# mir-group/allegro

Hardware: NVIDIA H100
Metric: atom-steps/sec (energy+forces) (higher is better)
Workload: dtype f32

## Files before the change

allegro_b200/_lib.py:

```python
from __future__ import annotations

import ctypes as C
import os
from typing import Optional, Sequence, Tuple

import torch

from . import build as _build

AB2_F64, AB2_F32, AB2_BF16 = 0, 1, 2
ACT_NONE, ACT_SILU, ACT_MUL_DSILU = 0, 1, 2
EPI_NONE, EPI_MUL_DSILU = 0, 1
NL_SILU, NL_MISH, NL_GELU = 1, 2, 3
NOT_ELIGIBLE = -1
MAX_SEG = 4

DTYPE_ENUM = {torch.float64: AB2_F64, torch.float32: AB2_F32, torch.bfloat16: AB2_BF16}
ACC_DTYPE = {torch.float64: torch.float64, torch.float32: torch.float32, torch.bfloat16: torch.float32}

_LIB: Optional[C.CDLL] = None

_vp, _i64, _i32, _dbl = C.c_void_p, C.c_int64, C.c_int, C.c_double

_SIGNATURES = {
    "ab2_version": ([], C.c_int),
    "ab2_device_ok": ([], C.c_int),
    "ab2_last_error": ([], C.c_char_p),
    "ab2_set_option": ([C.c_char_p, _i32], C.c_int),
    "ab2_op_scatter_env": ([_i32, _i64, _i64, _dbl, _vp, _vp, _vp, _vp], C.c_int),
    "ab2_op_contract": ([_i32, _i32, _i64, _i32, _i32, _i32, _i32, _i32, _vp, _vp, _vp, _vp, _vp, _vp, _vp], C.c_int),
    "ab2_op_gather_rows": ([_i32, _i64, _i64, _dbl, _vp, _vp, _vp, _vp], C.c_int),
    "ab2_op_contract_wgrad": ([_i32, _i64, _i32, _i32, _i32, _i32, _i32, _vp, _vp, _vp, _vp, _vp, _vp, _vp], C.c_int),
    "ab2_sh_fwd": ([_i32, _i32, _i64, _vp, _vp, _vp], C.c_int),
    "ab2_sh_bwd": ([_i32, _i32, _i64, _vp, _vp, _vp, _i32, _vp], C.c_int),
    "ab2_linear": ([_i32, _i64, _i32, _i32, _i32, _vp, _vp, _vp, _vp, _vp, _i32, _vp, _vp, _i32, _vp, _vp, _vp, _vp, _i32, _vp, _i64, _vp], C.c_int),
    "ab2_linear_nl": ([_i32, _i64, _i32, _i32, _i32, _vp, _vp, _vp, _vp, _vp, _i32, _vp, _vp, _i32, _vp, _vp, _vp, _vp, _i32, _vp, _i64, _vp, _i32], C.c_int),
    "ab2_linear_packed_bytes": ([_i32, _i32, _i32], C.c_int64),
    "ab2_linear_pack": ([_i32, _i32, _i32, _vp, _vp, _vp], C.c_int),
    "ab2_mlp2_readout": ([_i32, _i32, _i64, _i32, _i32, _i32, _i32, _vp, _i64, _vp, _i64, _vp, _i64, _vp, _i64, _vp, _i64, _vp, _i64, _vp, _vp, _vp], C.c_int),
    "ab2_mlp2": ([_i32, _i32, _i64, _i32, _i32, _i32, _i32, _vp, _vp, _vp, _vp, _vp, _vp, _vp, _i64, _i32, _vp, _vp, _vp, _vp, _vp], C.c_int),
    "ab2_mlp2_nl": ([_i32, _i32, _i64, _i32, _i32, _i32, _i32, _vp, _vp, _vp, _vp, _vp, _vp, _vp, _i64, _i32, _vp, _vp, _vp, _vp, _vp, _i32], C.c_int),
    "ab2_mlp2_readout_nl": ([_i32, _i32, _i64, _i32, _i32, _i32, _i32, _vp, _i64, _vp, _i64, _vp, _i64, _vp, _i64, _vp, _i64, _vp, _i64, _vp, _vp, _vp, _i32],
                            C.c_int),
    "ab2_env_sum": ([_i32, _i32, _i64, _i32, _vp, _vp, _vp, _i64, _dbl, _vp, _vp], C.c_int),
    "ab2_env_bwd": ([_i32, _i32, _i64, _i64, _i32, _vp, _vp, _vp, _vp, _i64, _vp, _dbl, _vp, _i64, _vp, _vp], C.c_int),
    "ab2_tp_fwd": ([_i32, _i32, _i64, _i64, _i32, _i32, _i32, _i32, _vp, _vp, _vp, _vp, _vp, _vp, _i32, _vp, _vp, _i64, _vp, _vp], C.c_int),
    "ab2_tp_bwd": ([_i32, _i32, _i64, _i64, _i32, _i32, _i32, _i32, _vp, _vp, _vp, _vp, _vp, _vp, _i32, _vp, _vp, _i64, _vp, _vp, _vp, _i64, _vp, _vp, _vp], C.c_int),
    "ab2_tp_chain_fwd": ([_i32, _i32, _i64, _i64, _i32, _vp, _vp, _vp, _vp, _vp, _vp, _vp, _vp, _vp, _vp], C.c_int),
    "ab2_tp_chain_bwd": ([_i32, _i32, _i64, _i64, _i32, _vp, _vp, _vp, _vp, _vp, _vp, _vp, _vp, _vp, _vp, _vp, _vp, _vp, _vp], C.c_int),
    "ab2_edge_sum": ([_i32, _i64, _vp, _vp, _dbl, _vp, _vp], C.c_int),
    "ab2_edge_sum_bwd": ([_i32, _i64, _vp, _vp, _dbl, _vp, _vp], C.c_int),
    "ab2_force_scatter": ([_i32, _i64, _i64, _i64, _vp, _vp, _vp, _vp, _vp, _vp], C.c_int),
    "ab2_force_virial_scatter": ([_i32, _i64, _i64, _i64, _vp, _vp, _vp, _vp, _vp, _vp, _vp, _vp], C.c_int),
    "ab2_transpose_ui": ([_i32, _i64, _i32, _i32, _vp, _vp, _i32, _vp], C.c_int),
    "ab2_edge_vec": ([_i32, _i32, _i64, _vp, _vp, _vp, _vp, _vp, _vp], C.c_int),
    "ab2_radial_fwd": ([_i32, _i64, _i32, _i32, _dbl, _vp, _vp, _vp, _vp, _vp, _i32, _vp, _vp, _vp, _vp, _vp, _vp], C.c_int),
    "ab2_radial_pq_fwd": ([_i32, _i64, _i32, _i32, _dbl, _vp, _vp, _vp, _vp, _vp, _i32, _vp, _vp, _vp, _vp], C.c_int),
    "ab2_radial_pq_bwd": ([_i32, _i64, _i32, _i32, _dbl, _vp, _vp, _vp, _vp, _vp, _i32, _vp, _vp, _vp, _vp, _vp, _vp], C.c_int),
    "ab2_radial_pq_bwd_nl": ([_i32, _i64, _i32, _i32, _dbl, _vp, _vp, _vp, _vp, _vp, _i32, _vp, _vp, _vp, _vp, _vp, _vp, _i32], C.c_int),
    "ab2_zbl": ([_i32, _i64, _i32, _dbl, _dbl, _vp, _vp, _vp, _vp, _vp, _vp, _vp, _vp, _vp], C.c_int),
    "ab2_p2p_mailbox_bytes": ([_i32, _i32], C.c_int64),
    "ab2_p2p_alloc": ([_i64, C.POINTER(C.c_void_p)], C.c_int),
    "ab2_p2p_free": ([_vp], C.c_int),
    "ab2_p2p_get_handle": ([_vp, _vp], C.c_int),
    "ab2_p2p_open_handle": ([_vp, C.POINTER(C.c_void_p)], C.c_int),
    "ab2_p2p_close_handle": ([_vp], C.c_int),
    "ab2_p2p_error": ([_vp, _i32, _i32, _vp], C.c_int),
    "ab2_p2p_begin": ([_vp, _vp], C.c_int),
    "ab2_p2p_push_rows": ([_i32, _i32, _i32, _vp, _vp, _i32, _dbl, _vp, _i32, _i32, _vp, _vp, _vp], C.c_int),
    "ab2_p2p_push_rows_v": ([_i32, _i32, _i32, _vp, _vp, _i32, _dbl, _dbl, _dbl, _vp, _i32, _i32, _vp, _vp, _vp], C.c_int),
    "ab2_p2p_wait_unpack": ([_i32, _i32, _i32, _vp, _i32, _i32, _vp, _i32, _vp, _vp, _i32, _vp], C.c_int),
    "ab2_p2p_allreduce_energy": ([_vp, _i32, _i32, _i32, _vp, _vp, _vp, _vp, _vp], C.c_int),
    "ab2_p2p_mailbox_bytes_ex": ([_i32, _i32, _i32], C.c_int64),
    "ab2_p2p_push_rows_w": ([_i32, _i32, _vp, _vp, _i32, _vp, _i32, _i32, _vp, _vp, _vp], C.c_int),
    "ab2_p2p_wait_unpack_w": ([_i32, _i32, _vp, _i32, _i32, _vp, _i32, _vp, _vp, _vp, _vp], C.c_int),
    "ab2_p2p_allreduce_vec": ([_vp, _i32, _i32, _i32, _i32, _vp, _vp, _vp, _vp, _vp], C.c_int),
    "ab2_slab_plan_count": ([_i32, _i32, _i64, _vp, _vp, _vp, _i32, _i32, _dbl, _dbl, _dbl, _vp, _vp, _vp], C.c_int),
    "ab2_slab_plan_fill": ([_i64, _vp, _vp, _vp, _vp, _vp, _vp], C.c_int),
    "ab2_slab_plan_count_lattice": ([_i32, _i32, _i64, _vp, _vp, _vp, _i32, _i32, _dbl, _dbl, _vp, _vp, _vp], C.c_int),
    "ab2_nl_bin": ([_i32, _i64, _vp, _vp, _vp, _vp, _vp, _dbl, _vp, _vp], C.c_int),
    "ab2_nl_count": ([_i32, _i64, _vp, _vp, _vp, _vp, _vp, _dbl, _vp, _vp, _vp, _vp], C.c_int),
    "ab2_nl_fill": ([_i32, _i64, _vp, _vp, _vp, _vp, _vp, _dbl, _vp, _vp, _vp, _vp, _vp, _vp], C.c_int),
    "ab2_nl_lattice_bin": ([_i32, _i64, _vp, _vp, _vp, _vp, _vp, _vp, _dbl, _vp, _vp], C.c_int),
    "ab2_nl_lattice_count": ([_i32, _i64, _vp, _vp, _vp, _vp, _vp, _vp, _dbl, _vp, _vp, _vp, _vp], C.c_int),
    "ab2_nl_lattice_fill": ([_i32, _i64, _vp, _vp, _vp, _vp, _vp, _vp, _dbl, _vp, _vp, _vp, _vp, _vp, _vp], C.c_int),
    "ab2_radial_bwd": ([_i32, _i64, _i32, _i32, _dbl, _vp, _vp, _vp, _vp, _vp, _i32, _vp, _vp, _vp, _vp, _vp, _vp, _vp], C.c_int),
    "ab2_nl_frames_count": ([_i32, _i64, _i64, _vp, _vp, _vp, _vp, _vp, _vp, _dbl, _vp, _vp], C.c_int),
    "ab2_nl_frames_fill": ([_i32, _i64, _i64, _vp, _vp, _vp, _vp, _vp, _vp, _dbl, _vp, _vp, _vp, _vp], C.c_int),
    "ab2_nl_prune_count": ([_i32, _i64, _i64, _i32, _vp, _vp, _vp, _vp, _vp, _vp, _vp, _vp], C.c_int),
    "ab2_nl_prune_fill": ([_i32, _i64, _i64, _i32, _vp, _vp, _vp, _vp, _vp, _vp, _vp, _vp, _vp, _vp], C.c_int),
    "ab2_frame_scratch_elems": ([_i64, _i64], C.c_int64),
    "ab2_frame_sum": ([_i32, _i64, _i64, _vp, _vp, _vp, _i64, _vp, _vp], C.c_int),
    "ab2_frame_virial": ([_i32, _i64, _i64, _vp, _vp, _vp, _vp, _vp, _i64, _vp, _vp], C.c_int),
    "ab2_frame_heat_current": ([_i32, _i64, _i64, _vp, _vp, _vp, _vp, _vp, _i64, _vp, _vp], C.c_int),
    "ab2_frame_extrema": ([_i32, _i64, _i64, _vp, _vp, _vp, _i64, _vp, _vp], C.c_int),
    "ab2_committee_moments": ([_i32, _i32, _i64, _i32, C.POINTER(C.c_void_p), _vp, _vp, _vp], C.c_int),
    "ab2_slots_check": ([_i32, _i64, _i64, _vp, _vp, _vp, _dbl, _vp, _vp], C.c_int),
    "ab2_slots_count": ([_i32, _i64, _i64, _vp, _vp, _vp, _vp, _vp, _vp, _dbl, _vp, _vp, _vp], C.c_int),
    "ab2_slots_place": ([_i64, _vp, _vp, _vp, _vp, _vp, _vp, _vp, _vp], C.c_int),
    "ab2_slots_fill": ([_i32, _i64, _i64, _vp, _vp, _vp, _vp, _vp, _vp, _dbl, _vp, _vp, _dbl, _vp, _vp, _vp, _vp, _vp], C.c_int),
    "ab2_slots_transpose": ([_i64, _i32, _vp, _vp, _vp, _vp, _vp, _vp, _vp], C.c_int),
}


def exported_symbols() -> Sequence[str]:
    return tuple(_SIGNATURES)


def lib_path() -> str:
    return _build.LIB


def load() -> C.CDLL:
    global _LIB
    if _LIB is not None:
        return _LIB
    path = lib_path()
    if not os.path.exists(path):
        if os.environ.get("ALLEGRO_B200_AUTOBUILD", "0") == "1":
            _build.build()
        else:
            raise RuntimeError(
                f"allegro_b200: CUDA extension {path} not built. Run `python -m allegro_b200.build` "
                "(or __graft_entry__.build()).  There is no CPU fallback."
            )
    lib = C.CDLL(path)
# ... 33 lines not shown
    _TAG[0] = tag


class _timed:
    __slots__ = ("name", "n", "ev")

    def __init__(self, name: str, n_kernels: int = 1):
        self.name, self.n = name, n_kernels

    def __enter__(self):
        PROF.launches += self.n
        if PROF.enabled:
            self.ev = (torch.cuda.Event(enable_timing=True), torch.cuda.Event(enable_timing=True))
            self.ev[0].record()
        return self

    def __exit__(self, *a):
        if PROF.enabled:
            self.ev[1].record()
            PROF.records.setdefault(self.name + "@" + _TAG[0], []).append(self.ev)
        return False

    def cancel(self):
        PROF.launches -= self.n
        if PROF.enabled:
            key = self.name + "@" + _TAG[0]
            PROF.records[key].pop()
            if not PROF.records[key]:
                del PROF.records[key]


def set_option(key: str, value: int):
    _check(load().ab2_set_option(key.encode(), int(value)))


def _check(rc: int):
    if rc != 0:
        msg = load().ab2_last_error()
        raise RuntimeError(f"allegro_b200 kernel call failed (rc={rc}): {msg.decode() if msg else '?'}")


def _ptr(t: Optional[torch.Tensor]):
    if t is None:
        return None
    if not t.is_cuda:
        raise RuntimeError("allegro_b200: tensor is not on a CUDA device (no CPU fallback on the hot path)")
    return C.c_void_p(t.data_ptr())


def _stream():
    return C.c_void_p(torch.cuda.current_stream().cuda_stream)


def _contig(t: torch.Tensor, name: str):
    if not t.is_contiguous():
        raise RuntimeError(f"allegro_b200: {name} must be contiguous")
    return t


def _row_strided(t: torch.Tensor, name: str):
    if t.dim() != 2 or t.stride(1) != 1:
        raise RuntimeError(f"allegro_b200: {name} must be 2-D with unit inner stride")
    return t, int(t.stride(0))


def sh_fwd(vec: torch.Tensor, lmax: int) -> torch.Tensor:
    E = vec.shape[0]
    Y = torch.empty(E, (lmax + 1) ** 2, dtype=vec.dtype, device=vec.device)
    with _timed("sh_fwd"):
        _check(load().ab2_sh_fwd(DTYPE_ENUM[vec.dtype], lmax, E, _ptr(_contig(vec, "vec")), _ptr(Y), _stream()))
    return Y


def sh_bwd(vec: torch.Tensor, gY: torch.Tensor, lmax: int, out: Optional[torch.Tensor] = None, accumulate: bool = False):
    E = vec.shape[0]
    if out is None:
        out = torch.empty_like(vec)
        accumulate = False
    with _timed("sh_bwd"):
        _check(load().ab2_sh_bwd(DTYPE_ENUM[vec.dtype], lmax, E, _ptr(_contig(vec, "vec")), _ptr(_contig(gY, "gY")), _ptr(out), int(accumulate), _stream()))
    return out


def linear(
    a_segs: Sequence[torch.Tensor],
    W: torch.Tensor,
    o_segs: Sequence[torch.Tensor],
    o_accum: Optional[Sequence[bool]] = None,
    act: int = ACT_NONE,
    epi: int = EPI_NONE,
    aux: Optional[torch.Tensor] = None,
    W_packed: Optional[torch.Tensor] = None,
    a_aux: Optional[Sequence[Optional[torch.Tensor]]] = None,
    nonlin: int = NL_SILU,
):
    M = a_segs[0].shape[0]
    K, N = W.shape
    dt = W.dtype
    na, no = len(a_segs), len(o_segs)
    a_ptr = (C.c_void_p * na)()
    a_ld = (C.c_int64 * na)()
    a_w = (C.c_int32 * na)()
    for s, t in enumerate(a_segs):
        t, ld = _row_strided(t, f"A segment {s}")
        assert t.dtype == dt and t.shape[0] == M
        a_ptr[s], a_ld[s], a_w[s] = t.data_ptr(), ld, t.shape[1]
        _ptr(t)
    x_ptr = x_ld = None
    if a_aux is not None:
        assert act == ACT_MUL_DSILU and len(a_aux) == na
        x_ptr = (C.c_void_p * na)()
        x_ld = (C.c_int64 * na)()
        for s, t in enumerate(a_aux):
            if t is None:
                x_ptr[s], x_ld[s] = None, 0
            else:
                t, ld = _row_strided(t, f"A aux segment {s}")
                assert t.dtype == dt and t.shape == a_segs[s].shape
                x_ptr[s], x_ld[s] = t.data_ptr(), ld
                _ptr(t)
    o_ptr = (C.c_void_p * no)()
    o_ld = (C.c_int64 * no)()
    o_w = (C.c_int32 * no)()
    o_acc = (C.c_int32 * no)()
    for s, t in enumerate(o_segs):
        t, ld = _row_strided(t, f"output segment {s}")
        assert t.dtype == dt and t.shape[0] == M
        o_ptr[s], o_ld[s], o_w[s] = t.data_ptr(), ld, t.shape[1]
        o_acc[s] = int(bool(o_accum[s])) if o_accum is not None else 0
        _ptr(t)
    aux_ld = 0
    if aux is not None:
        aux, aux_ld = _row_strided(aux, "aux")
        assert aux.dtype == dt
    args = (DTYPE_ENUM[dt], M, K, N, na, a_ptr, a_ld, a_w, x_ptr, x_ld, act, _ptr(_contig(W, "W")), _ptr(W_packed), no, o_ptr, o_ld, o_w, o_acc,
            epi, _ptr(aux), aux_ld, _stream())
    with _timed("linear", 1):
        _check(load().ab2_linear(*args) if nonlin == NL_SILU else load().ab2_linear_nl(*args, nonlin))


def mlp2(
    a_segs: Sequence[torch.Tensor],
    W1: torch.Tensor,
    W2: torch.Tensor,
    o_segs: Sequence[torch.Tensor],
    pre: torch.Tensor,
    o_accum: Optional[Sequence[bool]] = None,
    backward: bool = False,
    W1_packed: Optional[torch.Tensor] = None,
    W2_packed: Optional[torch.Tensor] = None,
    nonlin: int = NL_SILU,
) -> bool:
    M = a_segs[0].shape[0]
    K, H = W1.shape
    N = W2.shape[1]
    dt = W1.dtype
    rank1 = backward and K == 1
    if W2_packed is None or (W1_packed is None and not rank1):
        return False
    na, no = len(a_segs), len(o_segs)
    a_ptr = (C.c_void_p * na)()
    a_ld = (C.c_int64 * na)()
    a_w = (C.c_int32 * na)()
    for s, t in enumerate(a_segs):
        t, ld = _row_strided(t, f"A segment {s}") if t.shape[1] > 1 else (t, int(t.stride(0)))
        assert t.dtype == dt and t.shape[0] == M
        a_ptr[s], a_ld[s], a_w[s] = t.data_ptr(), ld, t.shape[1]
        _ptr(t)
    o_ptr = (C.c_void_p * no)()
    o_ld = (C.c_int64 * no)()
    o_w = (C.c_int32 * no)()
    o_acc = (C.c_int32 * no)()
    for s, t in enumerate(o_segs):
        t, ld = _row_strided(t, f"output segment {s}")
        assert t.dtype == dt and t.shape[0] == M
        o_ptr[s], o_ld[s], o_w[s] = t.data_ptr(), ld, t.shape[1]
        o_acc[s] = int(bool(o_accum[s])) if o_accum is not None else 0
        _ptr(t)
    pre, pre_ld = _row_strided(pre, "pre")
    assert pre.dtype == dt and tuple(pre.shape) == (M, H)
    timer = _timed("mlp2", 1)
    args = (DTYPE_ENUM[dt], int(backward), M, K, H, N, na, a_ptr, a_ld, a_w, _ptr(W1_packed), _ptr(W2_packed),
            _ptr(_contig(W1, "W1")) if rank1 else None, _ptr(pre), pre_ld, no, o_ptr, o_ld, o_w, o_acc, _stream())
    with timer:
        rc = load().ab2_mlp2(*args) if nonlin == NL_SILU else load().ab2_mlp2_nl(*args, nonlin)
    if rc == NOT_ELIGIBLE:
        timer.cancel()
        return False
    _check(rc)
    return True


def mlp2_readout(
    backward: bool,
    x: torch.Tensor,
    s: torch.Tensor,
    xl: Optional[torch.Tensor],
    pre_l: torch.Tensor,
    pre_r: torch.Tensor,
    ez: torch.Tensor,
    w2_ro: torch.Tensor,
    W_packed: Sequence[Optional[torch.Tensor]],
    S: int,
    nonlin: int = NL_SILU,
) -> bool:
    if any(w is None for w in W_packed):
        return False
    M, P = x.shape
    U = s.shape[1]
    H = pre_l.shape[1]
    if pre_r.shape[1] != H or w2_ro.numel() != H:
        return False
    if not backward and xl.shape[1] != S:
        raise ValueError(f"mlp2_readout: x_L has {xl.shape[1]} columns, S = {S}")
    kn = [(H, P + S), (S, H), (H, P + U)] if backward else [(P + U, H), (H, S), (P, H), (S, H)]
    if len(W_packed) != len(kn):
        raise ValueError(f"mlp2_readout: {len(W_packed)} packed images, expected {len(kn)}")
    for i, ((k, n), w) in enumerate(zip(kn, W_packed)):
        if w.numel() * w.element_size() != (n + 31) // 32 * 32 * k * 4:
            raise ValueError(f"mlp2_readout: packed image {i} is not that of a [{k}][{n}] matrix")
    dt = x.dtype
    views = {}
    for name, t in (("x", x), ("s", s), ("xl", xl), ("pre_l", pre_l), ("pre_r", pre_r), ("ez", ez)):
        if t is None:
            views[name] = (None, 0)
            continue
        assert t.dtype == dt and t.shape[0] == M
        views[name] = (_ptr(t), int(t.stride(0))) if name == "ez" else (_ptr(_row_strided(t, name)[0]), int(t.stride(0)))
    assert ez.shape[1] == 1
    wp = (C.c_void_p * len(W_packed))(*[w.data_ptr() for w in W_packed])
    for w in W_packed:
        _ptr(w)
    timer = _timed("mlp2_readout", 1)
    args = (DTYPE_ENUM[dt], int(backward), M, P, S, U, H, *views["x"], *views["s"], *views["xl"], *views["pre_l"], *views["pre_r"],
            *views["ez"], wp, _ptr(_contig(w2_ro, "w2_ro")), _stream())
    with timer:
        rc = load().ab2_mlp2_readout(*args) if nonlin == NL_SILU else load().ab2_mlp2_readout_nl(*args, nonlin)
    if rc == NOT_ELIGIBLE:
        timer.cancel()
        return False
    _check(rc)
    return True


def linear_pack(W: torch.Tensor) -> Optional[torch.Tensor]:
    K, N = W.shape
    nbytes = int(load().ab2_linear_packed_bytes(DTYPE_ENUM[W.dtype], K, N))
    if nbytes == 0:
        return None
    packed = torch.empty(nbytes, dtype=torch.uint8, device=W.device)
    _check(load().ab2_linear_pack(DTYPE_ENUM[W.dtype], K, N, _ptr(_contig(W, "W")), _ptr(packed), _stream()))
    return packed


def env_sum(dtype, lmax: int, N: int, U: int, row_ptr, Y, w: torch.Tensor, sf: float, out: Optional[torch.Tensor] = None):
    w, w_ld = _row_strided(w, "w")
    D = (lmax + 1) ** 2
    if out is None:
        out = torch.empty(N, D, U, dtype=ACC_DTYPE[dtype], device=Y.device)
    with _timed("env_sum"):
        _check(load().ab2_env_sum(DTYPE_ENUM[dtype], lmax, N, U, _ptr(row_ptr), _ptr(_contig(Y, "Y")), _ptr(w), w_ld, float(sf), _ptr(out), _stream()))
    return out


def env_bwd(dtype, lmax: int, U: int, ctr, Y, w: torch.Tensor, ggamma, sf: float, gw: torch.Tensor, gY: torch.Tensor, row_ptr=None):
    w, w_ld = _row_strided(w, "w")
    gw, gw_ld = _row_strided(gw, "gw")
    E = Y.shape[0]
    with _timed("env_bwd", 1):
        _check(
            load().ab2_env_bwd(
                DTYPE_ENUM[dtype], lmax, ggamma.shape[0], E, U, _ptr(row_ptr), _ptr(ctr), _ptr(_contig(Y, "Y")), _ptr(w), w_ld,
                _ptr(_contig(ggamma, "ggamma")), float(sf),
                _ptr(gw), gw_ld, _ptr(_contig(gY, "gY")), _stream(),
            )
        )


def tp_fwd(dtype, lmax, N, E, U, d_in, d_out, tab, cgw, row_ptr, ctr, gamma, Vin, Y, w0, Vout):
    implicit = Vin is None
    w0_ld = 0
    if implicit:
        w0, w0_ld = _row_strided(w0, "w0")
    with _timed("tp_fwd", 1):
        _check(
            load().ab2_tp_fwd(
                DTYPE_ENUM[dtype], lmax, N, E, U, d_in, d_out, tab.shape[0], _ptr(tab), _ptr(cgw), _ptr(row_ptr), _ptr(ctr), _ptr(gamma),
                _ptr(Vin), int(implicit), _ptr(Y), _ptr(w0) if implicit else None, w0_ld, _ptr(Vout), _stream(),
            )
        )


def tp_bwd(dtype, lmax, N, E, U, d_in, d_out, tab, cgw, row_ptr, ctr, gamma, Vin, Y, w0, gVout, gVin, gw0, gY, ggamma):
    implicit = Vin is None
    w0_ld = gw0_ld = 0
    if implicit:
        w0, w0_ld = _row_strided(w0, "w0")
        gw0, gw0_ld = _row_strided(gw0, "gw0")
    with _timed("tp_bwd", 2):
        _check(
            load().ab2_tp_bwd(
                DTYPE_ENUM[dtype], lmax, N, E, U, d_in, d_out, tab.shape[0], _ptr(tab), _ptr(cgw), _ptr(row_ptr), _ptr(ctr), _ptr(gamma),
                _ptr(Vin), int(implicit), _ptr(Y), _ptr(w0) if implicit else None, w0_ld, _ptr(gVout), _ptr(gVin),
                _ptr(gw0) if implicit else None, gw0_ld, _ptr(gY) if implicit else None, _ptr(ggamma), _stream(),
            )
        )


def tp_chain_takes(dtype, U: int) -> bool:
    return dtype == torch.float32 and U in (32, 64)


def tp_chain_plan(dtype, U: int, cgw0: torch.Tensor, cgw1: torch.Tensor):
    if not tp_chain_takes(dtype, U) or not cgw0.is_cuda:
        return None
    return {"cgw0": cgw0.to(torch.float32).contiguous(), "cgw1": cgw1.to(torch.float32).contiguous(), "U": U}


def _chain_dense(t: torch.Tensor, shape, name: str):
    if tuple(t.shape) != tuple(shape) or t.dtype != torch.float32:
        raise ValueError(f"tp_chain: {name} is {tuple(t.shape)} {t.dtype}, expected {tuple(shape)} float32")
    return _ptr(_contig(t, name))


def tp_chain_fwd(plan, last: bool, row_ptr, ctr, gamma0, gamma1, Y, w0, s) -> bool:
    if plan is None:
        return False
    E, U = s.shape
    N = gamma0.shape[0]
    args = [_chain_dense(gamma0, (N, 9, U), "gamma0"), _chain_dense(gamma1, (N, 9, U), "gamma1") if last else None,
            _chain_dense(Y, (E, 9), "Y"), _chain_dense(w0, (E, 3 * U), "w0"), _chain_dense(s, (E, U), "s")]
    timer = _timed("tp_chain_fwd", 1)
    with timer:
        rc = load().ab2_tp_chain_fwd(AB2_F32, int(last), N, E, U, _ptr(row_ptr), _ptr(ctr), _ptr(plan["cgw0"]), _ptr(plan["cgw1"]),
                                     *args, _stream())
    if rc == NOT_ELIGIBLE:
        timer.cancel()
        return False
    _check(rc)
    return True


def tp_chain_bwd(plan, first: bool, row_ptr, ctr, gamma0, gamma1, Y, w0, g1, g2, gw0, gY, ggamma) -> bool:
    if plan is None:
        return False
    E, U = g2.shape
    N = gamma0.shape[0]
    args = [_chain_dense(gamma0, (N, 9, U), "gamma0"), _chain_dense(gamma1, (N, 9, U), "gamma1") if first else None,
            _chain_dense(Y, (E, 9), "Y"), _chain_dense(w0, (E, 3 * U), "w0"), _chain_dense(g1, (E, U), "g1") if first else None,
            _chain_dense(g2, (E, U), "g2"), _chain_dense(gw0, (E, 3 * U), "gw0") if first else None,
            _chain_dense(gY, (E, 9), "gY") if first else None, _chain_dense(ggamma, (N, 9, U), "ggamma")]
    timer = _timed("tp_chain_bwd", 1)
# ... 429 lines not shown
```

allegro_b200/csrc/env.cu:

```cuda
#include "common.cuh"

extern int g_ab2_opt_env_split;
int g_ab2_opt_env_unroll = 2;

template <typename TAct, typename TAcc, int LMAX, int SPLIT, int UNR = 2>
__global__ void __launch_bounds__(128) env_sum_kernel(int64_t N, int U, const int32_t* __restrict__ row_ptr,
                                                      const TAcc* __restrict__ Y, const TAct* __restrict__ w, int64_t w_ld,
                                                      TAcc sf, TAcc* __restrict__ gamma) {
    constexpr int D = (LMAX + 1) * (LMAX + 1);
    __shared__ TAcc red[SPLIT > 1 ? 4 : 1][SPLIT > 1 ? D : 1][32];
    const int nchunk = (U + 31) >> 5;
    const int warp = threadIdx.x >> 5, lane = threadIdx.x & 31;
    const int64_t grp = ((int64_t)blockIdx.x * 4 + warp) / SPLIT;
    const int sub = warp % SPLIT;
    const int64_t c = grp / nchunk;
    const bool valid = c < N;
    const int u = (int)(grp % nchunk) * 32 + lane;
    const bool live = valid && u < U;
    const int beg = valid ? row_ptr[c] : 0, end = valid ? row_ptr[c + 1] : 0;
    TAcc acc[D];
#pragma unroll
    for (int j = 0; j < D; ++j) acc[j] = TAcc(0);
#pragma unroll UNR
    for (int z = beg + sub; z < end; z += SPLIT) {
// ... 61 lines not shown
        if (lane == (j & 31)) gY[z * D + j] += s;
    }
}

template <typename TAct, typename TAcc, int LMAX, int SPLIT>
__global__ void __launch_bounds__(128) env_bwd_fast_kernel(int64_t N, int U, const int32_t* __restrict__ row_ptr,
                                                           const TAcc* __restrict__ Y, const TAct* __restrict__ w, int64_t w_ld,
                                                           const TAcc* __restrict__ ggamma, TAcc sf, TAct* __restrict__ gw,
                                                           int64_t gw_ld, TAcc* __restrict__ gY) {
    constexpr int D = (LMAX + 1) * (LMAX + 1);
    const int nchunk = (U + 31) >> 5;
    const int64_t wid = ((int64_t)blockIdx.x * 128 + threadIdx.x) >> 5;
    const int lane = threadIdx.x & 31;
    const int64_t grp = wid / SPLIT;
    const int sub = (int)(wid % SPLIT);
    const int64_t c = grp / nchunk;
    if (c >= N) return;
    const int u = (int)(grp % nchunk) * 32 + lane;
    const bool live = u < U;
    const int beg = row_ptr[c], end = row_ptr[c + 1];
    TAcc gg[D];
#pragma unroll
    for (int j = 0; j < D; ++j) gg[j] = live ? sf * ggamma[(c * D + j) * U + u] : TAcc(0);
#pragma unroll 2
    for (int64_t z = beg + sub; z < end; z += SPLIT) {
        TAcc Yz[D], wl[LMAX + 1];
#pragma unroll
        for (int j = 0; j < D; ++j) Yz[j] = Y[z * D + j];
#pragma unroll
        for (int l = 0; l <= LMAX; ++l) wl[l] = live ? to_acc<TAcc>(w[z * w_ld + l * U + u]) : TAcc(0);
        TAcc part[D];
#pragma unroll
        for (int l = 0; l <= LMAX; ++l) {
            TAcc gwl = TAcc(0);
#pragma unroll
            for (int j = l * l; j < (l + 1) * (l + 1); ++j) {
                gwl += Yz[j] * gg[j];
                part[j] = wl[l] * gg[j];
            }
            if (live) gw[z * gw_ld + l * U + u] = from_acc<TAct>(gwl);
        }
        const TAcc tot = warp_multi_sum<TAcc, D>(part, lane);
        const int j = lane >> 1;
        if (!(lane & 1) && j < D) {
            if (nchunk == 1) gY[z * D + j] += tot;
            else atomicAdd(&gY[z * D + j], tot);
        }
    }
}

extern "C" int ab2_env_sum(int dtype, int lmax, int64_t N, int U, const int32_t* row_ptr, const void* Y, const void* w,
                           int64_t w_ld, double sf, void* gamma, void* stream) {
    if (N == 0) return 0;
    AB2_CHECK_ARG(row_ptr && Y && w && gamma && U > 0, "null pointer / U");
    AB2_CHECK_ARG(w_ld >= (int64_t)(lmax + 1) * U, "w_ld too small");
    cudaStream_t st = (cudaStream_t)stream;
    const int64_t groups = N * ((U + 31) / 32);
    const int split = g_ab2_opt_env_split ? g_ab2_opt_env_split : (U <= 32 ? 4 : 1);
    if (split >= 4 && g_ab2_opt_env_unroll == 4) {
        AB2_DISPATCH_DTYPE(dtype, AB2_DISPATCH_LMAX(lmax, env_sum_kernel<TAct, TAcc, LMAX, 4, 4><<<ab2_blocks(groups * 4 * 32, 128), 128, 0, st>>>(
                                                              N, U, row_ptr, (const TAcc*)Y, (const TAct*)w, w_ld, (TAcc)sf, (TAcc*)gamma)));
    } else if (split >= 4) {
        AB2_DISPATCH_DTYPE(dtype, AB2_DISPATCH_LMAX(lmax, env_sum_kernel<TAct, TAcc, LMAX, 4><<<ab2_blocks(groups * 4 * 32, 128), 128, 0, st>>>(
                                                              N, U, row_ptr, (const TAcc*)Y, (const TAct*)w, w_ld, (TAcc)sf, (TAcc*)gamma)));
    } else if (split >= 2) {
        AB2_DISPATCH_DTYPE(dtype, AB2_DISPATCH_LMAX(lmax, env_sum_kernel<TAct, TAcc, LMAX, 2><<<ab2_blocks(groups * 2 * 32, 128), 128, 0, st>>>(
                                                              N, U, row_ptr, (const TAcc*)Y, (const TAct*)w, w_ld, (TAcc)sf, (TAcc*)gamma)));
    } else {
        AB2_DISPATCH_DTYPE(dtype, AB2_DISPATCH_LMAX(lmax, env_sum_kernel<TAct, TAcc, LMAX, 1><<<ab2_blocks(groups * 32, 128), 128, 0, st>>>(
                                                              N, U, row_ptr, (const TAcc*)Y, (const TAct*)w, w_ld, (TAcc)sf, (TAcc*)gamma)));
    }
    AB2_CUDA_LAUNCH_CHECK();
    return 0;
}

extern int g_ab2_opt_tp_fast;
int ab2_env_bwd_stream(int dtype, int lmax, int64_t N, int64_t E, int U, const int32_t* ctr, const void* Y, const void* w, int64_t w_ld,
                       const void* ggamma, double sf, void* gw, int64_t gw_ld, void* gY, cudaStream_t st);

extern "C" int ab2_env_bwd(int dtype, int lmax, int64_t N, int64_t E, int U, const int32_t* row_ptr, const int32_t* ctr, const void* Y,
                           const void* w, int64_t w_ld, const void* ggamma, double sf, void* gw, int64_t gw_ld, void* gY,
                           void* stream) {
    if (E == 0) return 0;
    AB2_CHECK_ARG(ctr && Y && w && ggamma && gw && gY && U > 0, "null pointer / U");
    cudaStream_t st = (cudaStream_t)stream;
    if (g_ab2_opt_tp_fast && ab2_env_bwd_stream(dtype, lmax, N, E, U, ctr, Y, w, w_ld, ggamma, sf, gw, gw_ld, gY, st) == 0) {
        AB2_CUDA_LAUNCH_CHECK();
        return 0;
    }
    if (g_ab2_opt_tp_fast && row_ptr && lmax <= 3) {
        const int opt = g_ab2_opt_env_split ? g_ab2_opt_env_split : (U > 32 && dtype != AB2_F64 ? 4 : 1);
        const int split = opt >= 4 ? 4 : opt >= 2 ? 2 : 1;
        const int64_t warps = N * ((U + 31) / 32) * split;
#define AB2_ENV_BWD(L, SP)                                                                                              \
    AB2_DISPATCH_DTYPE(dtype, env_bwd_fast_kernel<TAct, TAcc, L, SP><<<ab2_blocks(warps * 32, 128), 128, 0, st>>>(           \
                                  N, U, row_ptr, (const TAcc*)Y, (const TAct*)w, w_ld, (const TAcc*)ggamma, (TAcc)sf, (TAct*)gw, gw_ld, (TAcc*)gY))
#define AB2_ENV_BWD_L(L)                                  \
    do {                                                  \
        if (split == 4) { AB2_ENV_BWD(L, 4); }            \
        else if (split == 2) { AB2_ENV_BWD(L, 2); }       \
        else { AB2_ENV_BWD(L, 1); }                       \
    } while (0)
        if (lmax == 3) AB2_ENV_BWD_L(3);
        else if (lmax == 2) AB2_ENV_BWD_L(2);
        else if (lmax == 1) AB2_ENV_BWD_L(1);
        else AB2_ENV_BWD_L(0);
#undef AB2_ENV_BWD_L
#undef AB2_ENV_BWD
        AB2_CUDA_LAUNCH_CHECK();
        return 0;
    }
    AB2_DISPATCH_DTYPE(dtype, AB2_DISPATCH_LMAX(lmax, env_bwd_kernel<TAct, TAcc, LMAX><<<ab2_blocks(E * 32, 128), 128, 0, st>>>(
                                                          E, U, ctr, (const TAcc*)Y, (const TAct*)w, w_ld, (const TAcc*)ggamma, (TAcc)sf,
                                                          (TAct*)gw, gw_ld, (TAcc*)gY)));
    AB2_CUDA_LAUNCH_CHECK();
    return 0;
}
```

allegro_b200/csrc/env_stream.cu:

```cuda
#include "common.cuh"
#include "stream_common.cuh"

int g_ab2_opt_env_stream = 1;
int g_ab2_opt_env_stream_cps = 0;

namespace {

struct EnvParams {
    int64_t N, E;
    int U;
    const int32_t* ctr;
    const void* Y;
    const void* w;
    const void* ggamma;
    float sf;
    void* gw;
    void* gY;
};

template <typename TAct, int LMAX, int NCH, int UT, int TE, int NS, int NCW>
__global__ void __launch_bounds__((NCW + 1) * 32) env_bwd_stream_kernel(const EnvParams p) {
    constexpr int D = (LMAX + 1) * (LMAX + 1), N_IR = LMAX + 1;
    constexpr int YP = (D + 3) / 4 * 4;
    extern __shared__ __align__(128) uint8_t smem[];
    const int U = UT ? UT : p.U;
    const int row_el = N_IR * U;
    const int offW = 0;
    const int offY = (TE * row_el * (int)sizeof(TAct) + 127) & ~127;
    const int offC = offY + ((TE * YP * 4 + 127) & ~127);
    const int stage_bytes = offC + ((TE * 4 + 127) & ~127);
    uint64_t* bars = reinterpret_cast<uint64_t*>(smem);
    uint8_t* ring = smem + 128;
    const uint32_t bar0 = smem_u32(bars);
    auto full_bar = [&](int s) { return bar0 + 8u * s; };
    auto empty_bar = [&](int s) { return bar0 + 8u * (NS + s); };
    const int warp = threadIdx.x >> 5, lane = threadIdx.x & 31;
    if (threadIdx.x == 0) {
        for (int s = 0; s < NS; ++s) {
            mbar_init(full_bar(s), 33);
            mbar_init(empty_bar(s), NCW);
        }
        asm volatile("fence.mbarrier_init.release.cluster;" ::: "memory");
    }
    __syncthreads();
    const int64_t G = gridDim.x, b = blockIdx.x;
    const int e_lo = (int)(b * p.E / G), e_hi = (int)((b + 1) * p.E / G);

    if (warp == NCW) {
        int stage = 0;
        uint32_t phase = 0;
        for (int za = e_lo; za < e_hi; za += TE) {
            const int n = (e_hi - za) < TE ? (e_hi - za) : TE;
            if (lane == 0) mbar_wait_backoff(empty_bar(stage), phase ^ 1);
            __syncwarp();
            uint8_t* sb = ring + (size_t)stage * stage_bytes;
            if (lane == 0) {
                const uint32_t bytes = (uint32_t)(n * row_el * sizeof(TAct));
                mbar_expect_tx(full_bar(stage), bytes);
                bulk_g2s(smem_u32(sb + offW), (const TAct*)p.w + (int64_t)za * row_el, bytes, full_bar(stage));
            }
            const float* __restrict__ ysrc = (const float*)p.Y + (int64_t)za * D;
            const uint32_t ydst = smem_u32(sb + offY), cdst = smem_u32(sb + offC);
            for (int e = lane; e < n * D; e += 32) {
                const int r = e / D, i = e - r * D;
                cp_async4(ydst + 4u * (r * YP + i), ysrc + e);
            }
            for (int e = lane; e < n; e += 32) cp_async4(cdst + 4u * e, p.ctr + za + e);
            cp_async_arrive_noinc(full_bar(stage));
            if (++stage == NS) { stage = 0; phase ^= 1; }
        }
        asm volatile("cp.async.wait_all;" ::: "memory");
        return;
    }

    float gg[NCH][D];
    int cur = -1;
    int stage = 0;
    uint32_t phase = 0;
    const float sf = p.sf;
    for (int za = e_lo; za < e_hi; za += TE) {
        const int n = (e_hi - za) < TE ? (e_hi - za) : TE;
        mbar_wait(full_bar(stage), phase);
        const uint8_t* sb = ring + (size_t)stage * stage_bytes;
        const TAct* __restrict__ sW = reinterpret_cast<const TAct*>(sb + offW) + lane;
        const float* __restrict__ sY = reinterpret_cast<const float*>(sb + offY);
        const int* __restrict__ sC = reinterpret_cast<const int*>(sb + offC);
#pragma unroll 2
        for (int t = warp; t < n; t += NCW) {
            const int c = sC[t];
            if (c != cur) {
                cur = c;
#pragma unroll
                for (int q = 0; q < NCH; ++q)
#pragma unroll
                    for (int j = 0; j < D; ++j) {
                        const int u = q * 32 + lane;
                        gg[q][j] = (UT || u < U) ? sf * __ldg((const float*)p.ggamma + ((int64_t)c * D + j) * U + u) : 0.f;
                    }
            }
            float Yr[YP];
#pragma unroll
            for (int i4 = 0; i4 < YP / 4; ++i4) {
                const float4 y4 = *reinterpret_cast<const float4*>(sY + t * YP + 4 * i4);
                Yr[4 * i4] = y4.x; Yr[4 * i4 + 1] = y4.y; Yr[4 * i4 + 2] = y4.z; Yr[4 * i4 + 3] = y4.w;
            }
            float part[D];
#pragma unroll
            for (int j = 0; j < D; ++j) part[j] = 0.f;
            TAct* __restrict__ gw_row = (TAct*)p.gw + (int64_t)(za + t) * row_el + lane;
#pragma unroll
            for (int q = 0; q < NCH; ++q) {
                const bool live = UT ? true : (q * 32 + lane < U);
#pragma unroll
                for (int l = 0; l <= LMAX; ++l) {
                    const float wl = live ? to_acc<float>(sW[(t * N_IR + l) * U + q * 32]) : 0.f;
                    float gwl = 0.f;
#pragma unroll
                    for (int j = l * l; j < (l + 1) * (l + 1); ++j) {
                        gwl = fmaf(Yr[j], gg[q][j], gwl);
                        part[j] = fmaf(wl, gg[q][j], part[j]);
                    }
                    if (live) gw_row[l * U + q * 32] = from_acc<TAct>(gwl);
                }
            }
            float* __restrict__ gy = (float*)p.gY + (int64_t)(za + t) * D;
#pragma unroll
            for (int j0 = 0; j0 < D; j0 += 8) {
                constexpr int DD = D;
                const int cnt = (DD - j0) < 8 ? (DD - j0) : 8;
                if (cnt == 8) {
                    float v[8];
#pragma unroll
                    for (int k = 0; k < 8; ++k) v[k] = part[j0 + k];
                    const float tot = MultiSum<8>::run(v, lane);
                    if (MultiSum<8>::is_writer(lane)) atomicAdd(gy + j0 + MultiSum<8>::idx_of(lane), tot);
                } else if (cnt == 4) {
                    float v[4];
#pragma unroll
                    for (int k = 0; k < 4; ++k) v[k] = part[(j0 + k) < DD ? (j0 + k) : 0];
                    const float tot = MultiSum<4>::run(v, lane);
                    if (MultiSum<4>::is_writer(lane)) atomicAdd(gy + j0 + MultiSum<4>::idx_of(lane), tot);
                } else {
                    const float tot = warp_sum(part[j0 < DD ? j0 : 0]);
                    if (lane == 0) atomicAdd(gy + j0, tot);
                }
            }
        }
        __syncwarp();
        if (lane == 0) mbar_arrive(empty_bar(stage));
        if (++stage == NS) { stage = 0; phase ^= 1; }
    }
}

template <typename TAct, int LMAX, int NCH, int UT>
int launch(const EnvParams& p, cudaStream_t st) {
    constexpr int TE = 16, NS = 3, NCW = 4;
    constexpr int D = (LMAX + 1) * (LMAX + 1), N_IR = LMAX + 1, YP = (D + 3) / 4 * 4;
    auto kern = env_bwd_stream_kernel<TAct, LMAX, NCH, UT, TE, NS, NCW>;
    const int offY = (TE * N_IR * p.U * (int)sizeof(TAct) + 127) & ~127;
    const int stage_bytes = offY + ((TE * YP * 4 + 127) & ~127) + ((TE * 4 + 127) & ~127);
    const int smem = 128 + NS * stage_bytes;
    static int num_sms = 0;
    if (num_sms == 0) {
        int dev = 0;
        cudaGetDevice(&dev);
        cudaDeviceGetAttribute(&num_sms, cudaDevAttrMultiProcessorCount, dev);
    }
    if (cudaFuncSetAttribute(kern, cudaFuncAttributeMaxDynamicSharedMemorySize, smem) != cudaSuccess) {
        cudaGetLastError();
        return -1;
    }
    int cps = 0;
    if (cudaOccupancyMaxActiveBlocksPerMultiprocessor(&cps, kern, (NCW + 1) * 32, smem) != cudaSuccess || cps < 1) {
        cudaGetLastError();
        return -1;
    }
    if (cps > 8) cps = 8;
    if (g_ab2_opt_env_stream_cps > 0 && cps > g_ab2_opt_env_stream_cps) cps = g_ab2_opt_env_stream_cps;
    int64_t grid = (int64_t)num_sms * cps;
    const int64_t max_grid = (p.E + TE - 1) / TE;
    if (grid > max_grid) grid = max_grid;
    if (grid < 1) grid = 1;
    kern<<<(unsigned)grid, (NCW + 1) * 32, smem, st>>>(p);
    return 0;
}

template <typename TAct, int LMAX>
int launch_u(const EnvParams& p, cudaStream_t st) {
    if (p.U == 32) return launch<TAct, LMAX, 1, 32>(p, st);
    if (p.U < 32) return launch<TAct, LMAX, 1, 0>(p, st);
    if (p.U == 64) return launch<TAct, LMAX, 2, 64>(p, st);
    return -1;
}

}

int ab2_env_bwd_stream(int dtype, int lmax, int64_t N, int64_t E, int U, const int32_t* ctr, const void* Y, const void* w, int64_t w_ld,
                       const void* ggamma, double sf, void* gw, int64_t gw_ld, void* gY, cudaStream_t st) {
    if (!g_ab2_opt_env_stream || dtype == AB2_F64 || lmax < 1 || lmax > 2 || E <= 0 || E >= ((int64_t)1 << 31)) return -1;
    const int esz = dtype == AB2_F32 ? 4 : 2;
    const int n_ir = lmax + 1;
    if ((U * esz) % 16 != 0 || w_ld != (int64_t)n_ir * U || gw_ld != (int64_t)n_ir * U) return -1;
    if ((reinterpret_cast<uintptr_t>(w) & 15) != 0) return -1;
    EnvParams p;
    p.N = N; p.E = E; p.U = U; p.ctr = ctr; p.Y = Y; p.w = w; p.ggamma = ggamma; p.sf = (float)sf; p.gw = gw; p.gY = gY;
    if (dtype == AB2_F32) return lmax == 2 ? launch_u<float, 2>(p, st) : launch_u<float, 1>(p, st);
    return lmax == 2 ? launch_u<bf16, 2>(p, st) : launch_u<bf16, 1>(p, st);
}
```

allegro_b200/csrc/linear.cu:

```cuda
#include "common.cuh"

struct LinSeg {
    const void* ptr;
    int64_t ld;
    int width;
    int accum;
    const void* aux;
    int64_t aux_ld;
};

struct LinParams {
    int64_t M;
    int K, N;
    int n_a;
    LinSeg a[AB2_MAX_SEG];
    int act;
    const void* W;
    int n_o;
    LinSeg o[AB2_MAX_SEG];
    int epi;
    const void* aux;
    int64_t aux_ld;
};

// ... 15 lines not shown
}

template <typename TAct, typename TAcc, int NL>
__global__ void __launch_bounds__(256) linear_kernel(const LinParams p) {
    constexpr int BM = 64, BN = 64, BK = 16;
    __shared__ TAcc As[BK][BM + 4];
    __shared__ TAcc Ws[BK][BN + 4];
    const int tid = threadIdx.x;
    const int tx = tid & 15, ty = tid >> 4;
    const int64_t m0 = (int64_t)blockIdx.x * BM;
    const int n0 = blockIdx.y * BN;
    TAcc acc[4][4];
#pragma unroll
    for (int i = 0; i < 4; ++i)
#pragma unroll
        for (int j = 0; j < 4; ++j) acc[i][j] = TAcc(0);

    const TAct* __restrict__ W = (const TAct*)p.W;
    for (int k0 = 0; k0 < p.K; k0 += BK) {
#pragma unroll
        for (int t = 0; t < (BM * BK) / 256; ++t) {
            const int e = tid + t * 256;
            const int kk = e & (BK - 1), r = e >> 4;
            const int64_t m = m0 + r;
            TAcc v = TAcc(0);
            if (m < p.M && k0 + kk < p.K) {
                v = lin_load_a<TAct, TAcc, NL>(p, m, k0 + kk);
                if (p.act == AB2_ACT_SILU) v = act_f<NL>(v);
            }
            As[kk][r] = v;
        }
#pragma unroll
        for (int t = 0; t < (BK * BN) / 256; ++t) {
            const int e = tid + t * 256;
            const int n = e & (BN - 1), kk = e >> 6;
            TAcc v = TAcc(0);
            if (k0 + kk < p.K && n0 + n < p.N) v = to_acc<TAcc>(W[(int64_t)(k0 + kk) * p.N + n0 + n]);
            Ws[kk][n] = v;
        }
        __syncthreads();
#pragma unroll
        for (int kk = 0; kk < BK; ++kk) {
            TAcc a[4], b[4];
#pragma unroll
            for (int i = 0; i < 4; ++i) a[i] = As[kk][ty * 4 + i];
#pragma unroll
            for (int j = 0; j < 4; ++j) b[j] = Ws[kk][tx * 4 + j];
#pragma unroll
            for (int i = 0; i < 4; ++i)
#pragma unroll
                for (int j = 0; j < 4; ++j) acc[i][j] += a[i] * b[j];
        }
        __syncthreads();
    }

#pragma unroll
    for (int i = 0; i < 4; ++i) {
        const int64_t m = m0 + ty * 4 + i;
        if (m >= p.M) continue;
#pragma unroll
        for (int j = 0; j < 4; ++j) {
            int n = n0 + tx * 4 + j;
            if (n >= p.N) continue;
            TAcc v = acc[i][j];
            if (p.epi == AB2_EPI_MUL_DSILU) v *= dact_f<NL>(to_acc<TAcc>(((const TAct*)p.aux)[m * p.aux_ld + n]));
#pragma unroll
            for (int s = 0; s < AB2_MAX_SEG; ++s) {
                if (s < p.n_o) {
                    if (n >= 0 && n < p.o[s].width) {
                        TAct* dst = (TAct*)p.o[s].ptr + m * p.o[s].ld + n;
                        if (p.o[s].accum) v += to_acc<TAcc>(*dst);
                        *dst = from_acc<TAct>(v);
                        n = -1 << 20;
                    }
                    n -= p.o[s].width;
                }
            }
        }
    }
}

int ab2_linear_tc_try(int dtype, int64_t M, int K, int N, int n_a, const void* const* a_ptr, const int64_t* a_ld,
                      const int32_t* a_width, const void* const* a_aux, const int64_t* a_aux_ld, int act, const void* Wpacked, int n_o, void* const* o_ptr, const int64_t* o_ld,
                      const int32_t* o_width, const int32_t* o_accum, int epi, const void* aux, int64_t aux_ld, cudaStream_t st, int nonlin);

extern "C" int ab2_linear_nl(int dtype, int64_t M, int K, int N, int n_a, const void* const* a_ptr, const int64_t* a_ld,
                          const int32_t* a_width, const void* const* a_aux, const int64_t* a_aux_ld, int act, const void* W,
                          const void* Wpacked, int n_o, void* const* o_ptr,
                          const int64_t* o_ld, const int32_t* o_width, const int32_t* o_accum, int epi, const void* aux,
                          int64_t aux_ld, void* stream, int nonlin) {
    AB2_CHECK_ARG(nonlin == AB2_NL_SILU || nonlin == AB2_NL_MISH || nonlin == AB2_NL_GELU, "nonlinearity");
    if (M == 0) return 0;
    AB2_CHECK_ARG(n_a >= 1 && n_a <= AB2_MAX_SEG && n_o >= 1 && n_o <= AB2_MAX_SEG, "segment count");
    AB2_CHECK_ARG(K > 0 && N > 0 && W, "shape");
    AB2_CHECK_ARG(epi == AB2_EPI_NONE || aux, "aux required for dsilu epilogue");
    LinParams p;
    memset(&p, 0, sizeof(p));
    p.M = M; p.K = K; p.N = N; p.n_a = n_a; p.act = act; p.W = W; p.n_o = n_o; p.epi = epi; p.aux = aux; p.aux_ld = aux_ld;
    int ks = 0, ns = 0;
    for (int s = 0; s < n_a; ++s) {
        AB2_CHECK_ARG(a_ptr[s] && a_width[s] > 0 && a_ld[s] >= a_width[s], "A segment");
        p.a[s].ptr = a_ptr[s]; p.a[s].ld = a_ld[s]; p.a[s].width = a_width[s]; ks += a_width[s];
        p.a[s].aux = a_aux ? a_aux[s] : nullptr;
        p.a[s].aux_ld = (a_aux && a_aux_ld) ? a_aux_ld[s] : 0;
    }
    for (int s = 0; s < n_o; ++s) {
        AB2_CHECK_ARG(o_ptr[s] && o_width[s] > 0 && o_ld[s] >= o_width[s], "output segment");
        p.o[s].ptr = o_ptr[s]; p.o[s].ld = o_ld[s]; p.o[s].width = o_width[s]; p.o[s].accum = o_accum ? o_accum[s] : 0;
        ns += o_width[s];
    }
    AB2_CHECK_ARG(ks == K, "A segment widths must sum to K");
    AB2_CHECK_ARG(ns == N, "output segment widths must sum to N");
    cudaStream_t st = (cudaStream_t)stream;
    const int tc = Wpacked ? ab2_linear_tc_try(dtype, M, K, N, n_a, a_ptr, a_ld, a_width, a_aux, a_aux_ld, act, Wpacked, n_o, o_ptr, o_ld, o_width,
                                               o_accum, epi, aux, aux_ld, st, nonlin)
                           : -1;
    if (tc == 0) {
        AB2_CUDA_LAUNCH_CHECK();
        return 0;
    }
    if (tc > 0) {
        ab2_set_error("%s:%d: tensor-core linear: a column slice failed to launch (K=%d, N=%d)", __FILE__, __LINE__, K, N);
        return 2;
    }
    dim3 grid(ab2_blocks(M, 64), (unsigned)((N + 63) / 64));
    AB2_DISPATCH_NL(nonlin, AB2_DISPATCH_DTYPE(dtype, linear_kernel<TAct, TAcc, NL><<<grid, 256, 0, st>>>(p)));
    AB2_CUDA_LAUNCH_CHECK();
    return 0;
}

extern "C" int ab2_linear(int dtype, int64_t M, int K, int N, int n_a, const void* const* a_ptr, const int64_t* a_ld,
                          const int32_t* a_width, const void* const* a_aux, const int64_t* a_aux_ld, int act, const void* W,
                          const void* Wpacked, int n_o, void* const* o_ptr,
                          const int64_t* o_ld, const int32_t* o_width, const int32_t* o_accum, int epi, const void* aux,
                          int64_t aux_ld, void* stream) {
    return ab2_linear_nl(dtype, M, K, N, n_a, a_ptr, a_ld, a_width, a_aux, a_aux_ld, act, W, Wpacked, n_o, o_ptr, o_ld, o_width, o_accum, epi, aux,
                         aux_ld, stream, AB2_NL_SILU);
}
```

allegro_b200/csrc/linear_tc.cu:

```cuda
#include <cuda.h>

#include <type_traits>

#include "common.cuh"

extern int g_ab2_opt_linear_tc;
extern int g_ab2_opt_linear_tma;
extern int g_ab2_opt_tc_debug;

namespace {

constexpr int BM = 128;
constexpr int KC = 32;
constexpr int NSTAGE = 4;
constexpr int RAW_STAGE = 256 * 4 * 16;
constexpr int EPI_LD = 40;
constexpr int NCONS = 8;
constexpr int EPI_BYTES = NCONS * 16 * EPI_LD * 4;
constexpr int STAGE_HALF = BM * KC * 2;
constexpr int NPROD = 8;
constexpr int NTHREADS = (NPROD + NCONS) * 32;
constexpr int MAX_W_BYTES = 128 * 1024;
constexpr int MAX_K = 512;
constexpr int MAX_N = 128;
constexpr int MAX_CHUNK = MAX_N / 32;
constexpr int TAIL_BARS = 2 * NSTAGE * 8, TAIL_CHUNK = MAX_CHUNK * 32, TAIL_KMAP = (MAX_K / 8) * 16;
constexpr int TAIL_BYTES = TAIL_BARS + TAIL_CHUNK + 2 * TAIL_KMAP;

struct TcSeg {
    const void* ptr;
    int64_t ld;
    int width;
    int accum;
    const void* aux;
    int64_t aux_ld;
};

struct TcParams {
    int64_t M;
    int K, N, Npad;
    int n_a;
    TcSeg a[AB2_MAX_SEG];
    int act;
    const void* Wpacked;
    const void* Wlo;
    int n_o;
    TcSeg o[AB2_MAX_SEG];
    int epi;
    const void* aux;
    int64_t aux_ld;
    int64_t num_tiles;
    int nstage;
    int debug;
    int raw_depth;
    int has_aux;
};

struct KEnt {
    const void* ptr;
    int64_t ld;
};
struct ChunkInfo {
    float* optr;
    const float* aptr;
    int64_t ld;
    int32_t accum;
    int32_t ok;
};
static_assert(sizeof(KEnt) == 16 && sizeof(ChunkInfo) == 32, "table entry sizes");

__device__ __forceinline__ uint32_t smem_u32(const void* p) { return (uint32_t)__cvta_generic_to_shared(p); }

__device__ __forceinline__ void mbar_init(uint32_t bar, uint32_t count) {
    asm volatile("mbarrier.init.shared::cta.b64 [%0], %1;" ::"r"(bar), "r"(count));
}
__device__ __forceinline__ void mbar_arrive(uint32_t bar) {
    asm volatile("mbarrier.arrive.shared::cta.b64 _, [%0];" ::"r"(bar) : "memory");
}
__device__ __forceinline__ void mbar_wait(uint32_t bar, uint32_t parity) {
    asm volatile(
        "{\n\t"
        ".reg .pred p;\n\t"
        "WAIT_LOOP:\n\t"
        "mbarrier.try_wait.parity.shared::cta.b64 p, [%0], %1;\n\t"
        "@p bra WAIT_DONE;\n\t"
        "bra WAIT_LOOP;\n\t"
        "WAIT_DONE:\n\t"
        "}" ::"r"(bar),
        "r"(parity)
        : "memory");
}
__device__ __forceinline__ void fence_proxy_async() { asm volatile("fence.proxy.async.shared::cta;" ::: "memory"); }
__device__ __forceinline__ void fence_barrier_init() { asm volatile("fence.mbarrier_init.release.cluster;" ::: "memory"); }

__device__ __forceinline__ void wgmma_fence() { asm volatile("wgmma.fence.sync.aligned;" ::: "memory"); }
__device__ __forceinline__ void wgmma_commit() { asm volatile("wgmma.commit_group.sync.aligned;" ::: "memory"); }
template <int N>
__device__ __forceinline__ void wgmma_wait() { asm volatile("wgmma.wait_group.sync.aligned %0;" ::"n"(N) : "memory"); }
template <int NCH>
__device__ __forceinline__ void wgmma_bf16(float (&d)[16 * NCH], uint64_t da, uint64_t db, uint32_t scale_d) {
    if constexpr (NCH == 1) {
        asm volatile(
            "{\n\t.reg .pred p;\n\tsetp.ne.b32 p, %18, 0;\n\t"
            "wgmma.mma_async.sync.aligned.m64n32k16.f32.bf16.bf16 {%0, %1, %2, %3, %4, %5, %6, %7, %8, %9, %10, %11, %12, %13, %14, %15}, %16, %17, p, 1, 1, 0, 0;\n\t}"
            : "+f"(d[0]), "+f"(d[1]), "+f"(d[2]), "+f"(d[3]), "+f"(d[4]), "+f"(d[5]), "+f"(d[6]), "+f"(d[7]), "+f"(d[8]), "+f"(d[9]), "+f"(d[10]), "+f"(d[11]), "+f"(d[12]), "+f"(d[13]), "+f"(d[14]), "+f"(d[15])
            : "l"(da), "l"(db), "r"(scale_d));
    } else if constexpr (NCH == 2) {
        asm volatile(
            "{\n\t.reg .pred p;\n\tsetp.ne.b32 p, %34, 0;\n\t"
            "wgmma.mma_async.sync.aligned.m64n64k16.f32.bf16.bf16 {%0, %1, %2, %3, %4, %5, %6, %7, %8, %9, %10, %11, %12, %13, %14, %15, %16, %17, %18, %19, %20, %21, %22, %23, %24, %25, %26, %27, %28, %29, %30, %31}, %32, %33, p, 1, 1, 0, 0;\n\t}"
            : "+f"(d[0]), "+f"(d[1]), "+f"(d[2]), "+f"(d[3]), "+f"(d[4]), "+f"(d[5]), "+f"(d[6]), "+f"(d[7]), "+f"(d[8]), "+f"(d[9]), "+f"(d[10]), "+f"(d[11]), "+f"(d[12]), "+f"(d[13]), "+f"(d[14]), "+f"(d[15]), "+f"(d[16]), "+f"(d[17]), "+f"(d[18]), "+f"(d[19]), "+f"(d[20]), "+f"(d[21]), "+f"(d[22]), "+f"(d[23]), "+f"(d[24]), "+f"(d[25]), "+f"(d[26]), "+f"(d[27]), "+f"(d[28]), "+f"(d[29]), "+f"(d[30]), "+f"(d[31])
            : "l"(da), "l"(db), "r"(scale_d));
    } else if constexpr (NCH == 3) {
        asm volatile(
            "{\n\t.reg .pred p;\n\tsetp.ne.b32 p, %50, 0;\n\t"
            "wgmma.mma_async.sync.aligned.m64n96k16.f32.bf16.bf16 {%0, %1, %2, %3, %4, %5, %6, %7, %8, %9, %10, %11, %12, %13, %14, %15, %16, %17, %18, %19, %20, %21, %22, %23, %24, %25, %26, %27, %28, %29, %30, %31, %32, %33, %34, %35, %36, %37, %38, %39, %40, %41, %42, %43, %44, %45, %46, %47}, %48, %49, p, 1, 1, 0, 0;\n\t}"
            : "+f"(d[0]), "+f"(d[1]), "+f"(d[2]), "+f"(d[3]), "+f"(d[4]), "+f"(d[5]), "+f"(d[6]), "+f"(d[7]), "+f"(d[8]), "+f"(d[9]), "+f"(d[10]), "+f"(d[11]), "+f"(d[12]), "+f"(d[13]), "+f"(d[14]), "+f"(d[15]), "+f"(d[16]), "+f"(d[17]), "+f"(d[18]), "+f"(d[19]), "+f"(d[20]), "+f"(d[21]), "+f"(d[22]), "+f"(d[23]), "+f"(d[24]), "+f"(d[25]), "+f"(d[26]), "+f"(d[27]), "+f"(d[28]), "+f"(d[29]), "+f"(d[30]), "+f"(d[31]), "+f"(d[32]), "+f"(d[33]), "+f"(d[34]), "+f"(d[35]), "+f"(d[36]), "+f"(d[37]), "+f"(d[38]), "+f"(d[39]), "+f"(d[40]), "+f"(d[41]), "+f"(d[42]), "+f"(d[43]), "+f"(d[44]), "+f"(d[45]), "+f"(d[46]), "+f"(d[47])
            : "l"(da), "l"(db), "r"(scale_d));
    } else if constexpr (NCH == 4) {
        asm volatile(
            "{\n\t.reg .pred p;\n\tsetp.ne.b32 p, %66, 0;\n\t"
            "wgmma.mma_async.sync.aligned.m64n128k16.f32.bf16.bf16 {%0, %1, %2, %3, %4, %5, %6, %7, %8, %9, %10, %11, %12, %13, %14, %15, %16, %17, %18, %19, %20, %21, %22, %23, %24, %25, %26, %27, %28, %29, %30, %31, %32, %33, %34, %35, %36, %37, %38, %39, %40, %41, %42, %43, %44, %45, %46, %47, %48, %49, %50, %51, %52, %53, %54, %55, %56, %57, %58, %59, %60, %61, %62, %63}, %64, %65, p, 1, 1, 0, 0;\n\t}"
            : "+f"(d[0]), "+f"(d[1]), "+f"(d[2]), "+f"(d[3]), "+f"(d[4]), "+f"(d[5]), "+f"(d[6]), "+f"(d[7]), "+f"(d[8]), "+f"(d[9]), "+f"(d[10]), "+f"(d[11]), "+f"(d[12]), "+f"(d[13]), "+f"(d[14]), "+f"(d[15]), "+f"(d[16]), "+f"(d[17]), "+f"(d[18]), "+f"(d[19]), "+f"(d[20]), "+f"(d[21]), "+f"(d[22]), "+f"(d[23]), "+f"(d[24]), "+f"(d[25]), "+f"(d[26]), "+f"(d[27]), "+f"(d[28]), "+f"(d[29]), "+f"(d[30]), "+f"(d[31]), "+f"(d[32]), "+f"(d[33]), "+f"(d[34]), "+f"(d[35]), "+f"(d[36]), "+f"(d[37]), "+f"(d[38]), "+f"(d[39]), "+f"(d[40]), "+f"(d[41]), "+f"(d[42]), "+f"(d[43]), "+f"(d[44]), "+f"(d[45]), "+f"(d[46]), "+f"(d[47]), "+f"(d[48]), "+f"(d[49]), "+f"(d[50]), "+f"(d[51]), "+f"(d[52]), "+f"(d[53]), "+f"(d[54]), "+f"(d[55]), "+f"(d[56]), "+f"(d[57]), "+f"(d[58]), "+f"(d[59]), "+f"(d[60]), "+f"(d[61]), "+f"(d[62]), "+f"(d[63])
            : "l"(da), "l"(db), "r"(scale_d));
    }

}

__device__ __forceinline__ void cp_async16(uint32_t dst_smem, const void* src, uint32_t src_bytes) {
    asm volatile("cp.async.cg.shared.global [%0], [%1], 16, %2;" ::"r"(dst_smem), "l"(src), "r"(src_bytes) : "memory");
}
__device__ __forceinline__ void cp_async4(uint32_t dst_smem, const void* src) {
    asm volatile("cp.async.ca.shared.global [%0], [%1], 4;" ::"r"(dst_smem), "l"(src) : "memory");
}
__device__ __forceinline__ void cp_async_commit() { asm volatile("cp.async.commit_group;" ::: "memory"); }
template <int N>
__device__ __forceinline__ void cp_async_wait() { asm volatile("cp.async.wait_group %0;" ::"n"(N) : "memory"); }

// ... 503 lines not shown
            if (++f_kb == nkb) f_kb = 0;
        };
        auto emit = [&](float (&v)[GPW][8]) {
            mbar_wait(empty_bar(stage), phase ^ 1);
            uint8_t* st_hi = sA + stage * stage_bytes;
#pragma unroll
            for (int i = 0; i < GPW; ++i) {
                if (p.act == AB2_ACT_SILU) {
#pragma unroll
                    for (int t = 0; t < 8; ++t) v[i][t] = act_fast<NL>(v[i][t]);
                }
                const int g = warp * GPW + i;
                const uint32_t off = g * (KC / 8) * 128 + kc * 128 + r8 * 16;
                uint32_t hi[4];
                float lo[8];
#pragma unroll
                for (int t = 0; t < 4; ++t) {
                    const __nv_bfloat16 h0 = __float2bfloat16_rn(v[i][2 * t]), h1 = __float2bfloat16_rn(v[i][2 * t + 1]);
                    lo[2 * t] = v[i][2 * t] - __bfloat162float(h0);
                    lo[2 * t + 1] = v[i][2 * t + 1] - __bfloat162float(h1);
                    __nv_bfloat162 hh;
                    hh.x = h0; hh.y = h1;
                    hi[t] = *reinterpret_cast<uint32_t*>(&hh);
                }
                *reinterpret_cast<uint4*>(st_hi + off) = make_uint4(hi[0], hi[1], hi[2], hi[3]);
                if constexpr (SPLIT) {
                    *reinterpret_cast<uint4*>(st_hi + STAGE_HALF + off) =
                        make_uint4(pack_bf16x2(lo[0], lo[1]), pack_bf16x2(lo[2], lo[3]), pack_bf16x2(lo[4], lo[5]), pack_bf16x2(lo[6], lo[7]));
                }
            }
            fence_proxy_async();
            mbar_arrive(full_bar(stage));
            if (++stage == p.nstage) { stage = 0; phase ^= 1; }
        };
        static_assert(GPW == 2, "raw slot layout assumes 2 row groups per producer warp");
        for (int d = 0; d < p.raw_depth; ++d) issue();
        for (int64_t seq = 0; seq < total; ++seq) {
            if (p.raw_depth == 4) cp_async_wait<3>();
            else cp_async_wait<1>();
            float v[GPW][8];
            fetch(v);
            issue();
            emit(v);
        }
        cp_async_wait<0>();
    } else {
        tc_consumer_role<TSrc, SPLIT, NCH, NL>(p, ctx, warp - NPROD, lane);
    }
}

constexpr int TMA_BOX_BYTES = BM * KC * 4;

struct alignas(64) TmaMaps {
    CUtensorMap a[AB2_MAX_SEG];
    CUtensorMap x[AB2_MAX_SEG];
};

__device__ __forceinline__ void tma_load_2d(uint32_t dst, const CUtensorMap* map, int x, int y, uint32_t bar) {
    asm volatile("cp.async.bulk.tensor.2d.shared::cluster.global.mbarrier::complete_tx::bytes [%0], [%1, {%3, %4}], [%2];" ::"r"(dst),
                 "l"(reinterpret_cast<uint64_t>(map)), "r"(bar), "r"(x), "r"(y)
                 : "memory");
}
__device__ __forceinline__ void mbar_expect_tx(uint32_t bar, uint32_t bytes) {
    asm volatile("mbarrier.arrive.expect_tx.shared::cta.b64 _, [%0], %1;" ::"r"(bar), "r"(bytes) : "memory");
}

__device__ __forceinline__ void split_bf16x2(float a, float b, uint32_t& hi, uint32_t& lo) {
    const __nv_bfloat16 h0 = __float2bfloat16_rn(a), h1 = __float2bfloat16_rn(b);
    __nv_bfloat162 hh;
    hh.x = h0; hh.y = h1;
    hi = *reinterpret_cast<uint32_t*>(&hh);
    lo = pack_bf16x2(a - __bfloat162float(h0), b - __bfloat162float(h1));
}

__device__ __forceinline__ void tma_init_bars(uint32_t bar0, uint32_t rbar0, int wpg) {
    for (int s = 0; s < NSTAGE; ++s) {
        mbar_init(bar0 + 8u * s, wpg * 32);
        mbar_init(bar0 + 8u * (NSTAGE + s), NCONS);
    }
    for (int s = 0; s < 8; ++s) mbar_init(rbar0 + 8u * s, 1);
    fence_barrier_init();
}

__device__ __forceinline__ int4 tma_kseg_entry(const TcParams& p, int i) {
    int kk = i * KC;
    int4 ent = make_int4(-1, 0, 0, 0);
#pragma unroll
    for (int sgi = 0; sgi < AB2_MAX_SEG; ++sgi) {
        if (sgi < p.n_a && ent.x < 0 && kk < p.K) {
            if (kk < p.a[sgi].width) ent = make_int4(sgi, kk, p.a[sgi].aux ? 1 : 0, 0);
            kk -= p.a[sgi].width;
        }
    }
    return ent;
}

__device__ __forceinline__ void stage_w(uint8_t* dst, const void* hi, const void* lo, int w_half) {
    const uint4* src = reinterpret_cast<const uint4*>(hi);
    uint4* d = reinterpret_cast<uint4*>(dst);
    for (int e = threadIdx.x; e < w_half / 16; e += NTHREADS) d[e] = __ldg(src + e);
    const uint4* srcl = reinterpret_cast<const uint4*>(lo);
    uint4* dl = reinterpret_cast<uint4*>(dst + w_half);
    for (int e = threadIdx.x; e < w_half / 16; e += NTHREADS) dl[e] = __ldg(srcl + e);
}

template <int G, int NL>
__device__ __forceinline__ void tma_converter_role(const TcParams& p, const TmaMaps& maps, int NR, const TcCtx& ctx, uint8_t* sRaw,
                                                   const int4* sKseg, uint32_t rbar0, int64_t total, int warp, int lane) {
    constexpr int WPG = NPROD / G;
    constexpr int RGW = 16 / WPG;
    const int nkb = ctx.nkb;
    const int raw_slot = TMA_BOX_BYTES * (p.has_aux ? 2 : 1);
    uint8_t* sA = ctx.sA;
    const int stage_bytes = ctx.stage_bytes;
    auto rfull_bar = [&](int s) { return rbar0 + 8u * s; };

    auto tma_issue = [&](int64_t qs, int rs) {
        const int64_t tile = blockIdx.x + (qs / nkb) * gridDim.x;
        const int4 ent = sKseg[(int)(qs % nkb)];
        const uint32_t dst = smem_u32(sRaw + (size_t)rs * raw_slot);
        const bool ax = p.has_aux && ent.z;
        mbar_expect_tx(rfull_bar(rs), TMA_BOX_BYTES * (ax ? 2u : 1u));
        if (!(p.debug & 2)) {
            tma_load_2d(dst, &maps.a[ent.x], ent.y, (int)(tile * BM), rfull_bar(rs));
            if (ax) tma_load_2d(dst + TMA_BOX_BYTES, &maps.x[ent.x], ent.y, (int)(tile * BM), rfull_bar(rs));
        } else {
            asm volatile("mbarrier.complete_tx.shared::cta.b64 [%0], %1;" ::"r"(rfull_bar(rs)), "r"(TMA_BOX_BYTES * (ax ? 2u : 1u)) : "memory");
        }
    };

    {
        const int grp = warp / WPG, sub = warp % WPG;
        const int r8 = lane & 7, kc = lane >> 3;
        int rs = grp % NR, cs = grp % p.nstage, kb = grp % nkb;
        uint32_t rph = (uint32_t)((grp / NR) & 1), cph = (uint32_t)((grp / p.nstage) & 1);
        const bool leader = sub == 0 && lane == 0;
        if (leader) {
            for (int sgi = 0; sgi < p.n_a; ++sgi) {
                asm volatile("prefetch.tensormap [%0];" ::"l"(reinterpret_cast<uint64_t>(&maps.a[sgi])) : "memory");
                if (p.a[sgi].aux) asm volatile("prefetch.tensormap [%0];" ::"l"(reinterpret_cast<uint64_t>(&maps.x[sgi])) : "memory");
            }
            for (int q = grp; q < NR && q < total; q += G) tma_issue(q, q);
        }
        for (int64_t qs = grp; qs < total; qs += G) {
            mbar_wait(rfull_bar(rs), rph);
            const uint8_t* raw = sRaw + (size_t)rs * raw_slot;
            const bool ax = p.has_aux && sKseg[kb].z;
            float v[RGW][8];
#pragma unroll
            for (int i = 0; i < RGW; ++i) {
                const int row = (sub * RGW + i) * 8 + r8;
                const uint8_t* rp = raw + row * 128;
                const float4 x = *reinterpret_cast<const float4*>(rp + (((2 * kc) ^ r8) << 4));
                const float4 y = *reinterpret_cast<const float4*>(rp + (((2 * kc + 1) ^ r8) << 4));
                v[i][0] = x.x; v[i][1] = x.y; v[i][2] = x.z; v[i][3] = x.w; v[i][4] = y.x; v[i][5] = y.y; v[i][6] = y.z; v[i][7] = y.w;
            }
            if (ax) {
#pragma unroll
                for (int i = 0; i < RGW; ++i) {
                    const int row = (sub * RGW + i) * 8 + r8;
                    const uint8_t* rp = raw + TMA_BOX_BYTES + row * 128;
                    const float4 x = *reinterpret_cast<const float4*>(rp + (((2 * kc) ^ r8) << 4));
                    const float4 y = *reinterpret_cast<const float4*>(rp + (((2 * kc + 1) ^ r8) << 4));
                    v[i][0] *= dact_fast<NL>(x.x); v[i][1] *= dact_fast<NL>(x.y); v[i][2] *= dact_fast<NL>(x.z); v[i][3] *= dact_fast<NL>(x.w);
                    v[i][4] *= dact_fast<NL>(y.x); v[i][5] *= dact_fast<NL>(y.y); v[i][6] *= dact_fast<NL>(y.z); v[i][7] *= dact_fast<NL>(y.w);
                }
            }
            asm volatile("bar.sync %0, %1;" ::"r"(1 + grp), "r"(WPG * 32) : "memory");
            if (leader && qs + NR < total) tma_issue(qs + NR, rs);
            mbar_wait(ctx.empty_bar(cs), cph ^ 1);
            uint8_t* st_hi = sA + cs * stage_bytes;
#pragma unroll
            for (int i = 0; i < RGW; ++i) {
                if (p.act == AB2_ACT_SILU) {
#pragma unroll
                    for (int t = 0; t < 8; ++t) v[i][t] = act_fast<NL>(v[i][t]);
                }
                const int g = sub * RGW + i;
                const uint32_t off = g * (KC / 8) * 128 + kc * 128 + r8 * 16;
                uint32_t hi[4];
                float lo[8];
#pragma unroll
                for (int t = 0; t < 4; ++t) {
                    const __nv_bfloat16 h0 = __float2bfloat16_rn(v[i][2 * t]), h1 = __float2bfloat16_rn(v[i][2 * t + 1]);
                    lo[2 * t] = v[i][2 * t] - __bfloat162float(h0);
                    lo[2 * t + 1] = v[i][2 * t + 1] - __bfloat162float(h1);
                    __nv_bfloat162 hh;
                    hh.x = h0; hh.y = h1;
                    hi[t] = *reinterpret_cast<uint32_t*>(&hh);
                }
                *reinterpret_cast<uint4*>(st_hi + off) = make_uint4(hi[0], hi[1], hi[2], hi[3]);
                *reinterpret_cast<uint4*>(st_hi + STAGE_HALF + off) =
                    make_uint4(pack_bf16x2(lo[0], lo[1]), pack_bf16x2(lo[2], lo[3]), pack_bf16x2(lo[4], lo[5]), pack_bf16x2(lo[6], lo[7]));
            }
            fence_proxy_async();
            mbar_arrive(ctx.full_bar(cs));
            rs += G; if (rs >= NR) { rs -= NR; rph ^= 1; }
            cs += G; if (cs >= p.nstage) { cs -= p.nstage; cph ^= 1; }
            kb += G; while (kb >= nkb) kb -= nkb;
        }
    }
}

template <int G, int NCH, int NL>
__global__ void __launch_bounds__(NTHREADS, 1) linear_tma_kernel(const TcParams p, const __grid_constant__ TmaMaps maps, int NR) {
    constexpr int WPG = NPROD / G;
    using TSrc = float;
    constexpr bool SPLIT = true;
    extern __shared__ __align__(1024) uint8_t smem[];
    const int warp = __shfl_sync(0xffffffffu, threadIdx.x >> 5, 0), lane = threadIdx.x & 31;
    const int w_half = p.Npad * p.K * 2;
    const int w_bytes = 2 * w_half;
    const int stage_bytes = 2 * STAGE_HALF;
    const int raw_slot = TMA_BOX_BYTES * (p.has_aux ? 2 : 1);
    uint8_t* sRaw = smem + ((1024u - (smem_u32(smem) & 1023u)) & 1023u);
    uint8_t* sW = sRaw + (size_t)NR * raw_slot;
    uint8_t* sA = sW + ((w_bytes + 127) & ~127);
    float* sEpi = reinterpret_cast<float*>(sA + p.nstage * stage_bytes);
    uint64_t* bars = reinterpret_cast<uint64_t*>(reinterpret_cast<uint8_t*>(sEpi) + EPI_BYTES);
    ChunkInfo* sChunk = reinterpret_cast<ChunkInfo*>(reinterpret_cast<uint8_t*>(bars) + TAIL_BARS);
    int4* sKseg = reinterpret_cast<int4*>(reinterpret_cast<uint8_t*>(sChunk) + TAIL_CHUNK);
    uint64_t* rbars = reinterpret_cast<uint64_t*>(reinterpret_cast<uint8_t*>(sKseg) + (MAX_K / 32) * 16);
    const uint32_t bar0 = smem_u32(bars), rbar0 = smem_u32(rbars);
    const int nkb = p.K / KC;

    if (threadIdx.x == 0) tma_init_bars(bar0, rbar0, WPG);
    if (threadIdx.x < MAX_K / 32) {
        sKseg[threadIdx.x] = tma_kseg_entry(p, threadIdx.x);
    } else if (threadIdx.x >= 64 && threadIdx.x < 64 + MAX_CHUNK) {
        sChunk[threadIdx.x - 64] = tc_chunk_info<TSrc>(p, (threadIdx.x - 64) * 32);
    }
    stage_w(sW, p.Wpacked, p.Wlo, w_half);
    fence_proxy_async();
    __syncthreads();
    TcCtx ctx;
    ctx.sW = sW; ctx.sA = sA; ctx.sEpi = sEpi; ctx.sChunk = sChunk; ctx.bar0 = bar0;
    ctx.nkb = nkb; ctx.stage_bytes = stage_bytes; ctx.w_half = w_half;
    const int64_t my_tiles = (p.num_tiles > blockIdx.x) ? (p.num_tiles - blockIdx.x + gridDim.x - 1) / gridDim.x : 0;
    const int64_t total = my_tiles * nkb;

    if (warp >= NPROD) {
        tc_consumer_role<TSrc, SPLIT, NCH, NL>(p, ctx, warp - NPROD, lane);
    } else {
        tma_converter_role<G, NL>(p, maps, NR, ctx, sRaw, sKseg, rbar0, total, warp, lane);
    }
}

constexpr int MLP2_MAX_H = 64;
constexpr int MLP2_CHUNK = 64;
constexpr int MLP2_MAX_CHUNKS = 4;
constexpr int MLP2_TAIL = TAIL_BARS + (1 + MLP2_MAX_CHUNKS) * TAIL_CHUNK + (MAX_K / 32) * 16 + 8 * 8;

struct Mlp2Params {
    TcParams s1;
    TcParams s2[MLP2_MAX_CHUNKS];
    int n0[MLP2_MAX_CHUNKS];
    int n2;
    int w2_npad;
    int backward;
    const float* pre;
    int64_t pre_ld;
    const float* gout1;
    int64_t gout1_ld;
    const float* w1row;
};

template <int NCH>
__device__ __forceinline__ void mlp2_stage2(const TcParams& p2, const ChunkInfo* chunks, float* stg, uint32_t h_u, uint32_t h_half, int H, uint32_t w_u,
                                            uint32_t w_half, int64_t tile, int wg, int w4, int lane) {
    float acc[16 * NCH];
    tc_mma_resident<NCH>(acc, h_u, h_half, H, w_u, w_half);
    tc_epilogue<float, NCH, false>(p2, chunks, stg, acc, tile, wg, w4, lane);
}

template <int NCH1, int NL>
__global__ void __launch_bounds__(NTHREADS, 1) mlp2_kernel(const __grid_constant__ Mlp2Params q, const __grid_constant__ TmaMaps maps, int NR) {
    constexpr int G = 2, WPG = NPROD / G;
    constexpr int H = 32 * NCH1;
    const TcParams& p = q.s1;
    extern __shared__ __align__(1024) uint8_t smem[];
    const int warp = __shfl_sync(0xffffffffu, threadIdx.x >> 5, 0), lane = threadIdx.x & 31;
    const bool rank1 = q.gout1 != nullptr;
    const int w1_half = rank1 ? 0 : H * p.K * 2;
    const int w2_half = q.w2_npad * H * 2;
    const int stage_bytes = 2 * STAGE_HALF;
    constexpr int h_half = 64 * H * 2;
    uint8_t* sRaw = smem + ((1024u - (smem_u32(smem) & 1023u)) & 1023u);
    uint8_t* sW1 = sRaw + (size_t)NR * TMA_BOX_BYTES;
    uint8_t* sW2 = sW1 + 2 * w1_half;
    uint8_t* sA = sW2 + 2 * w2_half;
    uint8_t* sH = sA + p.nstage * stage_bytes;
    float* sEpi = reinterpret_cast<float*>(sH + 4 * h_half);
    uint64_t* bars = reinterpret_cast<uint64_t*>(reinterpret_cast<uint8_t*>(sEpi) + EPI_BYTES);
    ChunkInfo* sChunk = reinterpret_cast<ChunkInfo*>(reinterpret_cast<uint8_t*>(bars) + TAIL_BARS);
    int4* sKseg = reinterpret_cast<int4*>(reinterpret_cast<uint8_t*>(sChunk) + (1 + MLP2_MAX_CHUNKS) * TAIL_CHUNK);
    uint64_t* rbars = reinterpret_cast<uint64_t*>(reinterpret_cast<uint8_t*>(sKseg) + (MAX_K / 32) * 16);
    const uint32_t bar0 = smem_u32(bars), rbar0 = smem_u32(rbars);
    const int nkb = p.K / KC;

    if (threadIdx.x == 0) tma_init_bars(bar0, rbar0, WPG);
    if (threadIdx.x < MAX_K / 32) {
        sKseg[threadIdx.x] = tma_kseg_entry(p, threadIdx.x);
    } else if (threadIdx.x >= 64 && threadIdx.x < 64 + (1 + MLP2_MAX_CHUNKS) * MAX_CHUNK) {
        const int i = threadIdx.x - 64, t = i / MAX_CHUNK, c0 = (i % MAX_CHUNK) * 32;
        ChunkInfo ci{nullptr, nullptr, 0, 0, 0};
        if (t == 0) ci = tc_chunk_info<float>(p, c0);
        else if (t - 1 < q.n2) ci = tc_chunk_info<float>(q.s2[t - 1], c0);
        sChunk[i] = ci;
    }
    if (!rank1) stage_w(sW1, p.Wpacked, p.Wlo, w1_half);
    stage_w(sW2, q.s2[0].Wpacked, q.s2[0].Wlo, w2_half);
    fence_proxy_async();
    __syncthreads();
    TcCtx ctx;
    ctx.sW = sW1; ctx.sA = sA; ctx.sEpi = sEpi; ctx.sChunk = sChunk; ctx.bar0 = bar0;
    ctx.nkb = nkb; ctx.stage_bytes = stage_bytes; ctx.w_half = w1_half;

    if (warp < NPROD) {
        if (!rank1) {
            const int64_t my_tiles = (p.num_tiles > blockIdx.x) ? (p.num_tiles - blockIdx.x + gridDim.x - 1) / gridDim.x : 0;
            tma_converter_role<G, AB2_NL_SILU>(p, maps, NR, ctx, sRaw, sKseg, rbar0, my_tiles * nkb, warp, lane);
        }
        return;
    }
    const int cw = warp - NPROD, wg = cw >> 2, w4 = cw & 3;
    float* stg = sEpi + cw * 16 * EPI_LD;
    uint8_t* hid = sH + wg * 2 * h_half;
    const uint32_t hid_u = smem_u32(hid);
    const int r8 = lane >> 2, cq = 2 * (lane & 3);
    const uint32_t wg_bar = 8 + wg;
    int stage = 0;
    uint32_t phase = 0;
    for (int64_t tile = blockIdx.x; tile < p.num_tiles; tile += gridDim.x) {
        const uint32_t off_a = (uint32_t)(threadIdx.x & 96) * (H / 8) * 8 + r8 * 16 + cq * 2, off_b = off_a + (H / 8) * 128;
        const int64_t m0 = tile * BM + wg * 64 + w4 * 16 + r8;
        const int64_t ma = m0 < p.M ? m0 : p.M - 1, mb = m0 + 8 < p.M ? m0 + 8 : p.M - 1;
        asm volatile("bar.sync %0, %1;" ::"r"(wg_bar), "r"(128) : "memory");
        if (q.backward) {
            const float* ra = q.pre + ma * q.pre_ld + cq;
            const float* rb = q.pre + mb * q.pre_ld + cq;
#pragma unroll
            for (int j = 0; j < 4 * NCH1; ++j) {
                cp_async4(hid_u + off_a + j * 128, ra + 8 * j);
                cp_async4(hid_u + h_half + off_a + j * 128, ra + 8 * j + 1);
                cp_async4(hid_u + off_b + j * 128, rb + 8 * j);
                cp_async4(hid_u + h_half + off_b + j * 128, rb + 8 * j + 1);
            }
            cp_async_commit();
        }
        auto slot = [&](int i) { return hid + ((i & 2) ? off_b : off_a) + (i >> 2) * 128 + ((i & 1) ? h_half : 0); };
        auto pre_at = [&](int i) { return *reinterpret_cast<const float*>(slot(i)); };
        auto store_hidden = [&](auto&& h) {
#pragma unroll
            for (int j = 0; j < 4 * NCH1; ++j) {
                const float h0 = h(4 * j), h1 = h(4 * j + 1), h2 = h(4 * j + 2), h3 = h(4 * j + 3);
                uint32_t hi, lo;
                split_bf16x2(h0, h1, hi, lo);
                *reinterpret_cast<uint32_t*>(slot(4 * j)) = hi;
                *reinterpret_cast<uint32_t*>(slot(4 * j + 1)) = lo;
                split_bf16x2(h2, h3, hi, lo);
                *reinterpret_cast<uint32_t*>(slot(4 * j + 2)) = hi;
                *reinterpret_cast<uint32_t*>(slot(4 * j + 3)) = lo;
            }
        };
        if (rank1) {
            const float ga = __ldg(q.gout1 + ma * q.gout1_ld), gb = __ldg(q.gout1 + mb * q.gout1_ld);
            cp_async_wait<0>();
            store_hidden([&](int i) {
                const float w = __ldg(q.w1row + 8 * (i >> 2) + cq + (i & 1));
                return ((i & 2) ? gb : ga) * w * dact_fast<NL>(pre_at(i));
            });
        } else {
            float acc[16 * NCH1];
            tc_mma_ring<true, NCH1>(acc, p, ctx, wg, lane, stage, phase);
            if (!q.backward) {
                tc_epilogue<float, NCH1, false>(p, sChunk, stg, acc, tile, wg, w4, lane);
                store_hidden([&](int i) { return act_fast<NL>(acc[i]); });
            } else {
                cp_async_wait<0>();
                store_hidden([&](int i) { return acc[i] * dact_fast<NL>(pre_at(i)); });
            }
        }
        fence_proxy_async();
        asm volatile("bar.sync %0, %1;" ::"r"(wg_bar), "r"(128) : "memory");
#pragma unroll 1
        for (int c = 0; c < q.n2; ++c) {
            const TcParams& p2 = q.s2[c];
            const ChunkInfo* ch = sChunk + (1 + c) * MAX_CHUNK;
            const uint32_t w_u = smem_u32(sW2) + (uint32_t)q.n0[c] * H * 2;
            if (p2.Npad == 32) mlp2_stage2<1>(p2, ch, stg, hid_u, h_half, H, w_u, w2_half, tile, wg, w4, lane);
            else mlp2_stage2<2>(p2, ch, stg, hid_u, h_half, H, w_u, w2_half, tile, wg, w4, lane);
        }
    }
}

constexpr int RO_H = 64;
constexpr int RO_TILE = 64 * RO_H * 2;
constexpr int RO_MAX_CHUNKS = 4;
constexpr int RO_TAIL = TAIL_BARS + RO_MAX_CHUNKS * TAIL_CHUNK + (MAX_K / 32) * 16 + 8 * 8 + RO_H * 4;

struct Mlp2RoParams {
    TcParams s1;
    TcParams o[RO_MAX_CHUNKS];
    int n0[RO_MAX_CHUNKS];
// ... 193 lines not shown
    uint8_t* sT = sWi[2] + 2 * q.w_half[2];
    float* sEpi = reinterpret_cast<float*>(sT + 3 * 4 * RO_TILE);
    ChunkInfo* sChunk = reinterpret_cast<ChunkInfo*>(reinterpret_cast<uint8_t*>(sEpi) + EPI_BYTES + TAIL_BARS);
    if (threadIdx.x < RO_MAX_CHUNKS * MAX_CHUNK) {
        const int t = threadIdx.x / MAX_CHUNK;
        ChunkInfo ci{nullptr, nullptr, 0, 0, 0};
        if (t < q.n_chunks) ci = tc_chunk_info<float>(q.o[t], (threadIdx.x % MAX_CHUNK) * 32);
        sChunk[threadIdx.x] = ci;
    }
    for (int i = 0; i < 3; ++i) stage_w(sWi[i], q.w[i], reinterpret_cast<const uint8_t*>(q.w[i]) + q.w_half[i], q.w_half[i]);
    fence_proxy_async();
    __syncthreads();
    if (warp < NPROD) return;
    const int cw = warp - NPROD, wg = cw >> 2, w4 = cw & 3;
    float* stg = sEpi + cw * 16 * EPI_LD;
    uint8_t* t_r = sT + wg * 2 * RO_TILE;
    uint8_t* t_x = t_r + 4 * RO_TILE;
    uint8_t* t_h = t_x + 4 * RO_TILE;
    const uint32_t tr_u = smem_u32(t_r), tx_u = smem_u32(t_x), th_u = smem_u32(t_h);
    const uint32_t wr_u = smem_u32(sWi[0]), wl_u = smem_u32(sWi[2]);
    const int r8 = lane >> 2, cq = 2 * (lane & 3);
    const uint32_t wg_bar = 8 + wg;
    const uint32_t off_a = (uint32_t)(threadIdx.x & 96) * (RO_H / 8) * 8 + r8 * 16 + cq * 2, off_b = off_a + (RO_H / 8) * 128;
    auto wg_sync = [&]() { asm volatile("bar.sync %0, %1;" ::"r"(wg_bar), "r"(128) : "memory"); };
    for (int64_t tile = blockIdx.x; tile < p.num_tiles; tile += gridDim.x) {
        const int64_t m0 = tile * BM + wg * 64 + w4 * 16 + r8;
        const int64_t ma = m0 < p.M ? m0 : p.M - 1, mb = m0 + 8 < p.M ? m0 + 8 : p.M - 1;
        wg_sync();
        ro_fetch_pre(tr_u, off_a, off_b, q.pre_r + ma * q.pre_r_ld + cq, q.pre_r + mb * q.pre_r_ld + cq);
        ro_fetch_pre(th_u, off_a, off_b, q.pre_l + ma * q.pre_l_ld + cq, q.pre_l + mb * q.pre_l_ld + cq);
        const float ga = __ldg(q.ez + ma * q.ez_ld), gb = __ldg(q.ez + mb * q.ez_ld);
        cp_async_wait<1>();
        ro_store_tile(t_r, off_a, off_b, [&](int i) {
            const float w = __ldg(q.w2ro + 8 * (i >> 2) + cq + (i & 1));
            return ((i & 2) ? gb : ga) * w * dact_fast<NL>(ro_pre_at(t_r, off_a, off_b, i));
        });
        fence_proxy_async();
        wg_sync();
        {
            float gx[32];
            tc_mma_resident<2>(gx, tr_u, RO_TILE, RO_H, wr_u + (uint32_t)q.P * RO_H * 2, q.w_half[0]);
            ro_store_tile(t_x, off_a, off_b, [&](int i) { return gx[i]; });
        }
        fence_proxy_async();
        wg_sync();
        {
            float gh[32];
            tc_mma_resident<2>(gh, tx_u, RO_TILE, RO_H, smem_u32(sWi[1]), q.w_half[1]);
            cp_async_wait<0>();
            ro_store_tile(t_h, off_a, off_b, [&](int i) { return gh[i] * dact_fast<NL>(ro_pre_at(t_h, off_a, off_b, i)); });
        }
        fence_proxy_async();
        wg_sync();
#pragma unroll 1
        for (int c = 0; c < q.n_chunks; ++c) {
            const TcParams& pc = q.o[c];
            const uint32_t n0 = (uint32_t)q.n0[c];
            const bool with_ro = (int)n0 < q.P;
            if (pc.Npad == 32)
                ro_bwd_chunk<1>(pc, sChunk + c * MAX_CHUNK, stg, th_u, wl_u + n0 * RO_H * 2, q.w_half[2], tr_u, wr_u + n0 * RO_H * 2, q.w_half[0],
                                with_ro, tile, wg, w4, lane);
            else
                ro_bwd_chunk<2>(pc, sChunk + c * MAX_CHUNK, stg, th_u, wl_u + n0 * RO_H * 2, q.w_half[2], tr_u, wr_u + n0 * RO_H * 2, q.w_half[0],
                                with_ro, tile, wg, w4, lane);
        }
    }
}

template <typename TSrc>
__global__ void pack_w_kernel(int K, int N, int Npad, const TSrc* __restrict__ W, bf16* __restrict__ out) {
    const int e = blockIdx.x * blockDim.x + threadIdx.x;
    if (e >= Npad * K) return;
    const int n = e / K, k = e % K;
    const float w = (n < N) ? to_acc<float>(W[(int64_t)k * N + n]) : 0.f;
    const bf16 h = __float2bfloat16_rn(w);
    const bf16 l = __float2bfloat16_rn(w - __bfloat162float(h));
    const int64_t off = ((int64_t)(n / 8) * (K / 8) + k / 8) * 64 + (n % 8) * 8 + (k % 8);
    out[off] = h;
    out[(int64_t)Npad * K + off] = l;
}

}

static int tc_npad(int N) { return (N + 31) / 32 * 32; }

extern "C" int64_t ab2_linear_packed_bytes(int dtype, int K, int N) {
    if (dtype == AB2_F64 || K % 16 != 0 || K <= 0 || K > MAX_K || N <= 0) return 0;
    const int Npad = tc_npad(N);
    return (int64_t)Npad * K * 2 * 2;
}

static int tc_slice_cap(int dtype, int K) {
    const int per_col = K * 2 * (dtype == AB2_F32 ? 2 : 1);
    int cap = (MAX_W_BYTES / per_col) / 32 * 32;
    if (cap > MAX_N) cap = MAX_N;
    return cap;
}

extern "C" int ab2_linear_pack(int dtype, int K, int N, const void* W, void* packed, void* stream) {
    AB2_CHECK_ARG(ab2_linear_packed_bytes(dtype, K, N) > 0, "shape not supported by the tensor-core path");
    AB2_CHECK_ARG(W && packed, "null pointer");
    const int Npad = tc_npad(N);
    cudaStream_t st = (cudaStream_t)stream;
    const int total = Npad * K;
    if (dtype == AB2_F32)
        pack_w_kernel<float><<<(total + 255) / 256, 256, 0, st>>>(K, N, Npad, (const float*)W, (bf16*)packed);
    else
        pack_w_kernel<bf16><<<(total + 255) / 256, 256, 0, st>>>(K, N, Npad, (const bf16*)W, (bf16*)packed);
    AB2_CUDA_LAUNCH_CHECK();
    return 0;
}

typedef CUresult (*EncodeTiledFn)(CUtensorMap*, CUtensorMapDataType, cuuint32_t, void*, const cuuint64_t*, const cuuint64_t*, const cuuint32_t*,
                                  const cuuint32_t*, CUtensorMapInterleave, CUtensorMapSwizzle, CUtensorMapL2promotion, CUtensorMapFloatOOBfill);

static EncodeTiledFn tc_encode_fn() {
    static EncodeTiledFn fn = nullptr;
    static bool tried = false;
    if (!tried) {
        tried = true;
        void* ptr = nullptr;
        cudaDriverEntryPointQueryResult qres;
        if (cudaGetDriverEntryPoint("cuTensorMapEncodeTiled", &ptr, cudaEnableDefault, &qres) == cudaSuccess && qres == cudaDriverEntryPointSuccess)
            fn = reinterpret_cast<EncodeTiledFn>(ptr);
        else
            cudaGetLastError();
    }
    return fn;
}

static bool tc_make_map(CUtensorMap* map, const void* ptr, int64_t ld, int width, int64_t M) {
    EncodeTiledFn fn = tc_encode_fn();
    if (!fn) return false;
    const cuuint64_t dims[2] = {(cuuint64_t)width, (cuuint64_t)M};
    const cuuint64_t strides[1] = {(cuuint64_t)ld * 4};
    const cuuint32_t box[2] = {(cuuint32_t)KC, (cuuint32_t)BM};
    const cuuint32_t estr[2] = {1, 1};
    return fn(map, CU_TENSOR_MAP_DATA_TYPE_FLOAT32, 2, const_cast<void*>(ptr), dims, strides, box, estr, CU_TENSOR_MAP_INTERLEAVE_NONE,
              CU_TENSOR_MAP_SWIZZLE_128B, CU_TENSOR_MAP_L2_PROMOTION_L2_128B, CU_TENSOR_MAP_FLOAT_OOB_FILL_NONE) == CUDA_SUCCESS;
}

template <typename F>
static int tc_with_nl(int nonlin, F&& f) {
    switch (nonlin) {
        case AB2_NL_MISH: return f(std::integral_constant<int, AB2_NL_MISH>{});
        case AB2_NL_GELU: return f(std::integral_constant<int, AB2_NL_GELU>{});
        default: return f(std::integral_constant<int, AB2_NL_SILU>{});
    }
}

static int tc_launch_tma(TcParams& p, int w_bytes, int stage_bytes, int max_smem, unsigned grid, cudaStream_t st, bool dry, int nonlin) {
    TmaMaps maps;
    memset(&maps, 0, sizeof(maps));
    if (!tc_encode_fn()) return -1;
    for (int s = 0; s < p.n_a && !dry; ++s) {
        if (!tc_make_map(&maps.a[s], p.a[s].ptr, p.a[s].ld, p.a[s].width, p.M)) return -1;
        if (p.a[s].aux && !tc_make_map(&maps.x[s], p.a[s].aux, p.a[s].aux_ld, p.a[s].width, p.M)) return -1;
    }
    const int raw_slot = TMA_BOX_BYTES * (p.has_aux ? 2 : 1);
    const int plans[6][3] = {{4, 8, 4}, {4, 4, 4}, {2, 4, 4}, {2, 2, 4}, {2, 4, 2}, {2, 2, 2}};
    int G = 0, NR = 0, nstage = 0;
    size_t smem = 0;
    for (int q = 0; q < 6 && !G; ++q) {
        const size_t need = 1024 + ((w_bytes + 127) & ~127) + (size_t)plans[q][2] * stage_bytes + EPI_BYTES + TAIL_BYTES +
                            (size_t)plans[q][1] * raw_slot;
        if (need <= (size_t)max_smem) { G = plans[q][0]; NR = plans[q][1]; nstage = plans[q][2]; smem = need; }
    }
    if (!G) return -1;
    if (dry) return 0;
    p.nstage = nstage;
    auto go = [&](auto kern) -> int {
        if (cudaFuncSetAttribute(kern, cudaFuncAttributeMaxDynamicSharedMemorySize, (int)smem) != cudaSuccess) {
            cudaGetLastError();
            return -1;
        }
        kern<<<grid, NTHREADS, smem, st>>>(p, maps, NR);
        return 0;
    };
    return tc_with_nl(nonlin, [&](auto nl) -> int {
        constexpr int NL = decltype(nl)::value;
        switch ((G == 4 ? 4 : 0) + p.Npad / 32) {
            case 1: return go(linear_tma_kernel<2, 1, NL>);
            case 2: return go(linear_tma_kernel<2, 2, NL>);
            case 3: return go(linear_tma_kernel<2, 3, NL>);
            case 4: return go(linear_tma_kernel<2, 4, NL>);
            case 5: return go(linear_tma_kernel<4, 1, NL>);
            case 6: return go(linear_tma_kernel<4, 2, NL>);
            case 7: return go(linear_tma_kernel<4, 3, NL>);
            case 8: return go(linear_tma_kernel<4, 4, NL>);
        }
        return -1;
    });
}

static void tc_device_limits(int& num_sms, int& max_smem) {
    static int sms = 0, smem = 0;
    if (sms == 0) {
        int dev = 0;
        cudaGetDevice(&dev);
        cudaDeviceGetAttribute(&smem, cudaDevAttrMaxSharedMemoryPerBlockOptin, dev);
        cudaDeviceGetAttribute(&sms, cudaDevAttrMultiProcessorCount, dev);
    }
    num_sms = sms;
    max_smem = smem;
}

static int tc_launch_slice(int dtype, int64_t M, int K, int N, int n_a, const void* const* a_ptr, const int64_t* a_ld,
                           const int32_t* a_width, const void* const* a_aux, const int64_t* a_aux_ld, int act, const void* Whi, const void* Wlo,
                           int n_o, void* const* o_ptr, const int64_t* o_ld, const int32_t* o_width, const int32_t* o_accum, int epi,
                           const void* aux, int64_t aux_ld, cudaStream_t st, int nonlin, bool dry = false) {
    const int has_aux = (act == AB2_ACT_MUL_DSILU && a_aux) ? 1 : 0;
    if (tc_npad(N) > MAX_N) return -1;
    int num_sms = 0, max_smem = 0;
    tc_device_limits(num_sms, max_smem);
    TcParams p;
    memset(&p, 0, sizeof(p));
    p.M = M; p.K = K; p.N = N; p.Npad = tc_npad(N); p.n_a = n_a; p.act = act; p.Wpacked = Whi; p.Wlo = Wlo; p.n_o = n_o;
    p.epi = epi; p.aux = aux; p.aux_ld = aux_ld; p.num_tiles = (M + BM - 1) / BM;
    for (int s = 0; s < n_a; ++s) {
        p.a[s].ptr = a_ptr[s]; p.a[s].ld = a_ld[s]; p.a[s].width = a_width[s];
        p.a[s].aux = has_aux ? a_aux[s] : nullptr; p.a[s].aux_ld = has_aux ? a_aux_ld[s] : 0;
    }
    p.has_aux = has_aux;
    for (int s = 0; s < n_o; ++s) { p.o[s].ptr = o_ptr[s]; p.o[s].ld = o_ld[s]; p.o[s].width = o_width[s]; p.o[s].accum = o_accum ? o_accum[s] : 0; }
    const bool split = dtype == AB2_F32;
    const int w_bytes = p.Npad * K * 2 * (split ? 2 : 1);
    const int stage_bytes = STAGE_HALF * (split ? 2 : 1);
    int nstage = 0, raw_depth = 0;
    size_t smem = 0;
    const int raw_stage = RAW_STAGE * (has_aux ? 2 : 1);
    const int plans[4][2] = {{4, NSTAGE}, {4, 2}, {2, NSTAGE}, {2, 2}};
    for (int q = 0; q < 4 && !nstage; ++q) {
        const size_t need = ((w_bytes + 127) & ~127) + (size_t)plans[q][1] * stage_bytes + (size_t)plans[q][0] * raw_stage + EPI_BYTES +
                            TAIL_BYTES;
        if ((int)need <= max_smem) { raw_depth = plans[q][0]; nstage = plans[q][1]; smem = need; }
    }
    if (!nstage) return -1;
    if (dry) return 0;
    p.nstage = nstage;
    p.raw_depth = raw_depth;
    p.debug = g_ab2_opt_tc_debug;
    const unsigned grid = (unsigned)((p.num_tiles < num_sms) ? p.num_tiles : num_sms);
    bool tma_ok = g_ab2_opt_linear_tma && split && K % KC == 0 && M < ((int64_t)1 << 31);
    for (int s = 0; s < n_a && tma_ok; ++s) tma_ok = a_width[s] % KC == 0;
    if (tma_ok) {
        const int rc = tc_launch_tma(p, w_bytes, stage_bytes, max_smem, grid, st, dry, nonlin);
        if (rc == 0) return 0;
    }
    auto go = [&](auto kern) -> int {
        if (cudaFuncSetAttribute(kern, cudaFuncAttributeMaxDynamicSharedMemorySize, (int)smem) != cudaSuccess) {
            cudaGetLastError();
            return -1;
        }
        kern<<<grid, NTHREADS, smem, st>>>(p);
        return 0;
    };
    return tc_with_nl(nonlin, [&](auto nl) -> int {
        constexpr int NL = decltype(nl)::value;
        switch ((split ? 4 : 0) + p.Npad / 32) {
            case 1: return go(linear_tc_kernel<bf16, false, 1, NL>);
            case 2: return go(linear_tc_kernel<bf16, false, 2, NL>);
            case 3: return go(linear_tc_kernel<bf16, false, 3, NL>);
            case 4: return go(linear_tc_kernel<bf16, false, 4, NL>);
            case 5: return go(linear_tc_kernel<float, true, 1, NL>);
            case 6: return go(linear_tc_kernel<float, true, 2, NL>);
            case 7: return go(linear_tc_kernel<float, true, 3, NL>);
            case 8: return go(linear_tc_kernel<float, true, 4, NL>);
        }
        return -1;
    });
}

int ab2_linear_tc_try(int dtype, int64_t M, int K, int N, int n_a, const void* const* a_ptr, const int64_t* a_ld,
                      const int32_t* a_width, const void* const* a_aux, const int64_t* a_aux_ld, int act, const void* Wpacked, int n_o, void* const* o_ptr, const int64_t* o_ld,
                      const int32_t* o_width, const int32_t* o_accum, int epi, const void* aux, int64_t aux_ld, cudaStream_t st, int nonlin) {
    if (!g_ab2_opt_linear_tc || !Wpacked || dtype == AB2_F64) return -1;
    if (ab2_linear_packed_bytes(dtype, K, N) == 0) return -1;
    const int esz = (dtype == AB2_F32) ? 4 : 2;
    for (int s = 0; s < n_a; ++s) {
        if (a_width[s] % 8 != 0) return -1;
        if ((reinterpret_cast<uintptr_t>(a_ptr[s]) % 16) != 0 || (a_ld[s] * esz) % 16 != 0) return -1;
        if (act == AB2_ACT_MUL_DSILU && a_aux && a_aux[s] &&
            ((reinterpret_cast<uintptr_t>(a_aux[s]) % 16) != 0 || (a_aux_ld[s] * esz) % 16 != 0)) return -1;
    }
    const int cap = tc_slice_cap(dtype, K);
    if (cap < 32) return -1;
    const int Npad_full = tc_npad(N);
    const int nslices = (N + cap - 1) / cap;
    int width = ((N + nslices - 1) / nslices + 31) / 32 * 32;
    if (width > cap) width = cap;
    int32_t any_accum = 0;
    for (int s = 0; s < n_o && o_accum; ++s) any_accum |= o_accum[s];
    while (true) {
        const int probe = width < N ? width : N;
        if (tc_launch_slice(dtype, M, K, probe, n_a, a_ptr, a_ld, a_width, a_aux, a_aux_ld, act, Wpacked, Wpacked, 1, o_ptr, o_ld, &probe, &any_accum, epi,
                            aux, aux_ld, st, nonlin, true) == 0)
            break;
        if (width <= 32) return -1;
        width = (width / 2 + 31) / 32 * 32;
    }
    const uint8_t* hi = reinterpret_cast<const uint8_t*>(Wpacked);
    const uint8_t* lo = hi + (size_t)Npad_full * K * 2;
    for (int n0 = 0; n0 < N; n0 += width) {
        const int ns = (N - n0 < width) ? (N - n0) : width;
        void* so_ptr[AB2_MAX_SEG];
        int64_t so_ld[AB2_MAX_SEG];
        int32_t so_w[AB2_MAX_SEG], so_acc[AB2_MAX_SEG];
        int cnt = 0, seg_lo = 0;
        for (int s = 0; s < n_o; ++s) {
            const int seg_hi = seg_lo + o_width[s];
            const int a = n0 > seg_lo ? n0 : seg_lo, b = (n0 + ns) < seg_hi ? (n0 + ns) : seg_hi;
            if (a < b) {
                so_ptr[cnt] = reinterpret_cast<uint8_t*>(o_ptr[s]) + (size_t)(a - seg_lo) * esz;
                so_ld[cnt] = o_ld[s];
                so_w[cnt] = b - a;
                so_acc[cnt] = o_accum ? o_accum[s] : 0;
                ++cnt;
            }
            seg_lo = seg_hi;
        }
        const void* aux_s = aux ? reinterpret_cast<const uint8_t*>(aux) + (size_t)n0 * esz : nullptr;
        const int rc = tc_launch_slice(dtype, M, K, ns, n_a, a_ptr, a_ld, a_width, a_aux, a_aux_ld, act, hi + (size_t)n0 * K * 2,
                                       lo + (size_t)n0 * K * 2, cnt, so_ptr, so_ld, so_w, so_acc, epi, aux_s, aux_ld, st, nonlin);
        if (rc != 0) return n0 == 0 ? -1 : 1;
    }
    return 0;
}

extern "C" int ab2_mlp2_nl(int dtype, int backward, int64_t M, int K, int H, int N, int n_a, const void* const* a_ptr, const int64_t* a_ld,
                           const int32_t* a_width, const void* W1_packed, const void* W2_packed, const void* w1_row, void* pre, int64_t pre_ld,
                           int n_o, void* const* o_ptr, const int64_t* o_ld, const int32_t* o_width, const int32_t* o_accum, void* stream,
                           int nonlin) {
    AB2_CHECK_ARG(nonlin == AB2_NL_SILU || nonlin == AB2_NL_MISH || nonlin == AB2_NL_GELU, "nonlinearity");
    AB2_CHECK_ARG(n_a >= 1 && n_a <= AB2_MAX_SEG && n_o >= 1 && n_o <= AB2_MAX_SEG, "segment count");
    AB2_CHECK_ARG(K > 0 && H > 0 && N > 0 && pre && pre_ld >= H, "shape");
    int ks = 0, ns = 0;
    for (int s = 0; s < n_a; ++s) {
        AB2_CHECK_ARG(a_ptr[s] && a_width[s] > 0 && a_ld[s] >= a_width[s], "A segment");
        ks += a_width[s];
    }
    for (int s = 0; s < n_o; ++s) {
        AB2_CHECK_ARG(o_ptr[s] && o_width[s] > 0 && o_ld[s] >= o_width[s], "output segment");
        ns += o_width[s];
    }
    AB2_CHECK_ARG(ks == K, "A segment widths must sum to K");
    AB2_CHECK_ARG(ns == N, "output segment widths must sum to N");
    const bool rank1 = w1_row != nullptr;
    AB2_CHECK_ARG(!rank1 || (backward && K == 1 && n_a == 1), "rank-1 mode is the backward of a single output column");
    if (M == 0) return 0;
    auto al16 = [](const void* ptr, int64_t ld) { return (reinterpret_cast<uintptr_t>(ptr) % 16) == 0 && (ld * 4) % 16 == 0; };
    if (dtype != AB2_F32 || !g_ab2_opt_linear_tc || !g_ab2_opt_linear_tma || !tc_encode_fn()) return AB2_NOT_ELIGIBLE;
    if (H % 32 != 0 || H > MLP2_MAX_H || !W2_packed || M >= ((int64_t)1 << 31) || !al16(pre, pre_ld)) return AB2_NOT_ELIGIBLE;
    if (rank1) {
        if (reinterpret_cast<uintptr_t>(w1_row) % 16 != 0) return AB2_NOT_ELIGIBLE;
    } else {
        if (!W1_packed || K % KC != 0 || K > MAX_K) return AB2_NOT_ELIGIBLE;
        for (int s = 0; s < n_a; ++s)
            if (a_width[s] % KC != 0 || !al16(a_ptr[s], a_ld[s])) return AB2_NOT_ELIGIBLE;
    }
    const int nchunks = (N + MLP2_CHUNK - 1) / MLP2_CHUNK;
    if (nchunks > MLP2_MAX_CHUNKS) return AB2_NOT_ELIGIBLE;
    const int cwidth = ((N + nchunks - 1) / nchunks + 31) / 32 * 32;
    const int w2_npad = tc_npad(N);
    int num_sms = 0, max_smem = 0;
    tc_device_limits(num_sms, max_smem);
    const size_t fixed = 1024 + (rank1 ? 0 : (size_t)2 * H * K * 2) + (size_t)2 * w2_npad * H * 2 + (size_t)4 * 64 * H * 2 + EPI_BYTES + MLP2_TAIL;
    const int plans[4][2] = {{4, 4}, {2, 4}, {4, 2}, {2, 2}};
    int NR = 0, nstage = 0;
    size_t smem = rank1 ? fixed : 0;
    for (int q = 0; q < 4 && !rank1 && !NR; ++q) {
        const size_t need = fixed + (size_t)(plans[q][0] * TMA_BOX_BYTES + plans[q][1] * 2 * STAGE_HALF);
        if (need <= (size_t)max_smem) { NR = plans[q][0]; nstage = plans[q][1]; smem = need; }
    }
    if (smem == 0 || smem > (size_t)max_smem) return AB2_NOT_ELIGIBLE;

    Mlp2Params q;
    memset(&q, 0, sizeof(q));
    TmaMaps maps;
    memset(&maps, 0, sizeof(maps));
    const int64_t num_tiles = (M + BM - 1) / BM;
    TcParams& p = q.s1;
    p.M = M; p.K = K; p.N = H; p.Npad = H; p.n_a = n_a; p.act = AB2_ACT_NONE; p.epi = AB2_EPI_NONE;
    p.num_tiles = num_tiles; p.nstage = nstage;
    for (int s = 0; s < n_a; ++s) { p.a[s].ptr = a_ptr[s]; p.a[s].ld = a_ld[s]; p.a[s].width = a_width[s]; }
    if (rank1) {
        q.gout1 = reinterpret_cast<const float*>(a_ptr[0]);
        q.gout1_ld = a_ld[0];
        q.w1row = reinterpret_cast<const float*>(w1_row);
    } else {
        p.Wpacked = W1_packed;
        p.Wlo = reinterpret_cast<const uint8_t*>(W1_packed) + (size_t)H * K * 2;
        for (int s = 0; s < n_a; ++s)
            if (!tc_make_map(&maps.a[s], a_ptr[s], a_ld[s], a_width[s], M)) return AB2_NOT_ELIGIBLE;
    }
    if (backward) {
        q.backward = 1;
        q.pre = reinterpret_cast<const float*>(pre);
        q.pre_ld = pre_ld;
    } else {
        p.n_o = 1;
        p.o[0].ptr = pre; p.o[0].ld = pre_ld; p.o[0].width = H;
    }
    q.w2_npad = w2_npad;
    q.n2 = 0;
    for (int n0 = 0; n0 < N; n0 += cwidth, ++q.n2) {
        const int nc = (N - n0 < cwidth) ? (N - n0) : cwidth;
        TcParams& p2 = q.s2[q.n2];
        p2.M = M; p2.K = H; p2.N = nc; p2.Npad = tc_npad(nc); p2.epi = AB2_EPI_NONE; p2.num_tiles = num_tiles;
        q.n0[q.n2] = n0;
        int seg_lo = 0;
        for (int s = 0; s < n_o; ++s) {
            const int seg_hi = seg_lo + o_width[s];
            const int a = n0 > seg_lo ? n0 : seg_lo, b = (n0 + nc) < seg_hi ? (n0 + nc) : seg_hi;
            if (a < b) {
                TcSeg& o = p2.o[p2.n_o++];
                o.ptr = reinterpret_cast<float*>(o_ptr[s]) + (a - seg_lo);
                o.ld = o_ld[s];
                o.width = b - a;
                o.accum = o_accum ? o_accum[s] : 0;
            }
            seg_lo = seg_hi;
        }
    }
    q.s2[0].Wpacked = W2_packed;
    q.s2[0].Wlo = reinterpret_cast<const uint8_t*>(W2_packed) + (size_t)w2_npad * H * 2;

    const unsigned grid = (unsigned)((num_tiles < num_sms) ? num_tiles : num_sms);
    cudaStream_t st = (cudaStream_t)stream;
    auto go = [&](auto kern) -> int {
        if (cudaFuncSetAttribute(kern, cudaFuncAttributeMaxDynamicSharedMemorySize, (int)smem) != cudaSuccess) {
            cudaGetLastError();
            return AB2_NOT_ELIGIBLE;
        }
        kern<<<grid, NTHREADS, smem, st>>>(q, maps, NR);
        AB2_CUDA_LAUNCH_CHECK();
        return 0;
    };
    return tc_with_nl(nonlin, [&](auto nl) -> int {
        constexpr int NL = decltype(nl)::value;
        switch (H / 32) {
            case 1: return go(mlp2_kernel<1, NL>);
            case 2: return go(mlp2_kernel<2, NL>);
        }
        return AB2_NOT_ELIGIBLE;
    });
}

extern "C" int ab2_mlp2(int dtype, int backward, int64_t M, int K, int H, int N, int n_a, const void* const* a_ptr, const int64_t* a_ld,
                        const int32_t* a_width, const void* W1_packed, const void* W2_packed, const void* w1_row, void* pre, int64_t pre_ld, int n_o,
                        void* const* o_ptr, const int64_t* o_ld, const int32_t* o_width, const int32_t* o_accum, void* stream) {
    return ab2_mlp2_nl(dtype, backward, M, K, H, N, n_a, a_ptr, a_ld, a_width, W1_packed, W2_packed, w1_row, pre, pre_ld, n_o, o_ptr, o_ld, o_width,
                       o_accum, stream, AB2_NL_SILU);
}

extern "C" int ab2_mlp2_readout_nl(int dtype, int backward, int64_t M, int P, int S, int U, int H, void* x, int64_t x_ld, void* s, int64_t s_ld,
                                   void* xl, int64_t xl_ld, void* pre_l, int64_t pre_l_ld, void* pre_r, int64_t pre_r_ld, void* ez, int64_t ez_ld,
                                   const void* const* w_packed, const void* w2_ro, void* stream, int nonlin) {
    AB2_CHECK_ARG(nonlin == AB2_NL_SILU || nonlin == AB2_NL_MISH || nonlin == AB2_NL_GELU, "nonlinearity");
    AB2_CHECK_ARG(P > 0 && S > 0 && U > 0 && H > 0 && M >= 0, "shape");
    AB2_CHECK_ARG(x && s && pre_l && pre_r && ez && w2_ro && w_packed && (backward || xl), "null pointer");
    AB2_CHECK_ARG(x_ld >= P && s_ld >= U && (backward || xl_ld >= S) && pre_l_ld >= H && pre_r_ld >= H && ez_ld >= 1, "leading dimension");
    if (M == 0) return 0;
    const int n_w = backward ? 3 : 4;
    auto al16 = [](const void* ptr, int64_t ld) { return (reinterpret_cast<uintptr_t>(ptr) % 16) == 0 && (ld * 4) % 16 == 0; };
    if (dtype != AB2_F32 || !g_ab2_opt_linear_tc || !g_ab2_opt_linear_tma || (!backward && !tc_encode_fn())) return AB2_NOT_ELIGIBLE;
    if (H != RO_H || S != RO_H || P % KC != 0 || U % KC != 0 || P + U > MAX_K || M >= ((int64_t)1 << 31)) return AB2_NOT_ELIGIBLE;
    if (!al16(x, x_ld) || !al16(s, s_ld) || (!backward && !al16(xl, xl_ld)) || !al16(pre_l, pre_l_ld) || !al16(pre_r, pre_r_ld) ||
        reinterpret_cast<uintptr_t>(w2_ro) % 16 != 0)
        return AB2_NOT_ELIGIBLE;
    for (int i = 0; i < n_w; ++i)
        if (!w_packed[i]) return AB2_NOT_ELIGIBLE;

    Mlp2RoParams q;
    memset(&q, 0, sizeof(q));
    const int64_t num_tiles = (M + BM - 1) / BM;
    q.P = P;
    q.w2ro = reinterpret_cast<const float*>(w2_ro);
    q.ez = reinterpret_cast<float*>(ez);
    q.ez_ld = ez_ld;
    for (int i = 0; i < n_w; ++i) q.w[i] = w_packed[i];
    TcParams& p = q.s1;
    p.M = M; p.num_tiles = num_tiles;
    auto out1 = [&](TcParams& o, void* ptr, int64_t ld, int n) {
        o.M = M; o.K = H; o.N = n; o.Npad = n; o.epi = AB2_EPI_NONE; o.num_tiles = num_tiles;
        o.n_o = 1; o.o[0].ptr = ptr; o.o[0].ld = ld; o.o[0].width = n;
    };
    int num_sms = 0, max_smem = 0;
    tc_device_limits(num_sms, max_smem);
    const unsigned grid = (unsigned)((num_tiles < num_sms) ? num_tiles : num_sms);
    cudaStream_t st = (cudaStream_t)stream;
    auto go = [&](auto kern, size_t smem, auto... args) -> int {
        if (cudaFuncSetAttribute(kern, cudaFuncAttributeMaxDynamicSharedMemorySize, (int)smem) != cudaSuccess) {
            cudaGetLastError();
            return AB2_NOT_ELIGIBLE;
        }
        kern<<<grid, NTHREADS, smem, st>>>(q, args...);
        AB2_CUDA_LAUNCH_CHECK();
        return 0;
    };

    if (backward) {
        for (int seg = 0; seg < 2; ++seg) {
            const int lo = seg ? P : 0, hi = seg ? P + U : P;
            for (int n0 = lo; n0 < hi; n0 += 64) {
                if (q.n_chunks == RO_MAX_CHUNKS) return AB2_NOT_ELIGIBLE;
                const int nc = hi - n0 < 64 ? hi - n0 : 64;
                float* base = seg ? reinterpret_cast<float*>(s) + (n0 - P) : reinterpret_cast<float*>(x) + n0;
                out1(q.o[q.n_chunks], base, seg ? s_ld : x_ld, nc);
                q.n0[q.n_chunks++] = n0;
            }
        }
        q.w_half[0] = (P + S) * H * 2;
        q.w_half[1] = H * S * 2;
        q.w_half[2] = (P + U) * H * 2;
        q.pre_l = reinterpret_cast<const float*>(pre_l); q.pre_l_ld = pre_l_ld;
        q.pre_r = reinterpret_cast<const float*>(pre_r); q.pre_r_ld = pre_r_ld;
        const size_t smem = (size_t)2 * (q.w_half[0] + q.w_half[1] + q.w_half[2]) + (size_t)12 * RO_TILE + EPI_BYTES + RO_TAIL;
        if (smem > (size_t)max_smem) return AB2_NOT_ELIGIBLE;
        return tc_with_nl(nonlin, [&](auto nl) { return go(mlp2_readout_bwd_kernel<decltype(nl)::value>, smem); });
    }

    p.K = P + U; p.N = H; p.Npad = H; p.n_a = 2; p.act = AB2_ACT_NONE; p.epi = AB2_EPI_NONE;
    p.a[0].ptr = x; p.a[0].ld = x_ld; p.a[0].width = P;
    p.a[1].ptr = s; p.a[1].ld = s_ld; p.a[1].width = U;
    p.Wpacked = w_packed[0];
    p.n_o = 1; p.o[0].ptr = pre_l; p.o[0].ld = pre_l_ld; p.o[0].width = H;
    out1(q.o[0], xl, xl_ld, S);
    out1(q.o[1], pre_r, pre_r_ld, H);
// ... 27 lines not shown
```

allegro_b200/nn/_pipeline.py:

```python
from __future__ import annotations

import math
from typing import Dict, List, Optional

import torch

from .. import _lib
from ..data import EdgeCSR
from ._mlp import PackedMLP


def _env_perm(U: int, n_ir: int, individual: bool = True) -> torch.Tensor:
    r = torch.arange(n_ir).view(-1, 1)
    u = torch.arange(U).view(1, -1)
    if not individual:
        return (u + 0 * r).reshape(-1)
    return (u * n_ir + r).reshape(-1)


class _Saved:
    __slots__ = ("csr", "vec", "Y", "w0", "omega", "V", "gamma", "pre_lat", "pre_read", "X", "fold", "chain")


_BAKED_TABLES = {}


def _baked_table(d_out: int) -> torch.Tensor:
    if d_out not in _BAKED_TABLES:
        from ._contract import Contracter

        ir = "1x0e+1x1o+1x2e"
        _BAKED_TABLES[d_out] = Contracter(ir, ir, ir if d_out == 9 else "1x0e", mul=1).sparse_table()[0].cpu()
    return _BAKED_TABLES[d_out]


class AllegroCore:

    def __init__(self, tensor_embed, allegro, edge_readout, avg_num_neighbors: float, dtype: torch.dtype, device):
        self.dtype = dtype
        self.acc = _lib.ACC_DTYPE[dtype]
        self.device = torch.device(device)
        self.lmax = tensor_embed.lmax
        self.D = (self.lmax + 1) ** 2
        self.n_ir = self.lmax + 1
        self.U = allegro.num_tensor_features
        self.S = allegro.num_scalar_features
        self.L = allegro.num_layers
        self.S_in = tensor_embed.env_embed_linear.input_dim
        self.sf = 1.0 / math.sqrt(avg_num_neighbors)
        self.factor = 1.0 / math.sqrt(2.0 * avg_num_neighbors)
        U, n_ir, S = self.U, self.n_ir, self.S
        perm = _env_perm(U, n_ir, allegro._env_weighter.weight_individual_irreps)
        perm_w0 = _env_perm(U, n_ir, tensor_embed._edge_weighter.weight_individual_irreps)
        nw = n_ir * U
        nw0_ref = tensor_embed._edge_weighter.weight_numel
        proj = allegro.first_layer_env_embed_projection.folded_weights()[0]
        proj_perm = torch.cat([torch.arange(S), S + perm])
        self.embed = PackedMLP(
            tensor_embed.env_embed_linear, dtype, device, out_perm=torch.cat([perm_w0, nw0_ref + proj_perm]),
            extra_first=[proj],
        )
        self.layers = []
        for l, (tp, lat) in enumerate(zip(allegro.tps, allegro.latents)):
            last = l == self.L - 1
            ijk, _, _ = tp.sparse_table()
            out_perm = None if last else torch.cat([torch.arange(S), S + perm])
            self.layers.append(
                dict(
                    d_in=tp.base_dim1,
                    d_out=tp.base_dim_out,
                    tab=ijk.to(device),
                    cgw=tp.cgw(self.acc, device),
                    mlp=PackedMLP(lat, dtype, device, out_perm=out_perm),
                    last=last,
                )
            )
            assert tp.base_dim2 == self.D
        self.readout = PackedMLP(edge_readout, dtype, device)
        self.nw = nw
        last = self.layers[-1]["mlp"]
        self.ro_fused = (last.is_two_layer_nonlinear and self.readout.is_two_layer_nonlinear and last.dims[1] == self.readout.dims[1]
                         and last.nonlinearity == self.readout.nonlinearity)
        if self.ro_fused:
            P = S * self.L
            W1r = self.readout.W[0]
            self.ro_fwd_p = [last.Wp[0], last.Wp[1], _lib.linear_pack(W1r[:P].contiguous()), _lib.linear_pack(W1r[P:].contiguous())]
            self.ro_bwd_p = [self.readout.WTp[0], last.WTp[1], last.WTp[0]]
        import os as _os

        self.plain_ok = (_os.environ.get("ALLEGRO_B200_PLAIN_BWD", "0") == "1" and self.readout.is_two_layer_nonlinear
                         and all(ly["mlp"].is_two_layer_nonlinear and ly["mlp"].nonlinearity == self.readout.nonlinearity
                                 for ly in self.layers))
        if self.plain_ok:
            L = self.L
            self.gxW, self.gxWp, self.gsW, self.gsWp = [], [], [], []
            for b in range(L + 1):
                blocks = [self.readout.WT[0][:, S * b : S * (b + 1)]]
                blocks += [self.layers[mm]["mlp"].WT[0][:, S * b : S * (b + 1)] for mm in range(L - 1, b - 1, -1) if mm >= b]
                Wg = torch.cat(blocks, dim=0).contiguous()
                self.gxW.append(Wg)
                self.gxWp.append(_lib.linear_pack(Wg))
            for l in range(L):
                Ws = self.layers[l]["mlp"].WT[0][:, S * (l + 1) : S * (l + 1) + U].contiguous()
                self.gsW.append(Ws)
                self.gsWp.append(_lib.linear_pack(Ws))
        self.chain = None
        l0, l1 = (self.layers + [None, None])[:2]
        if (self.L == 2 and not self.plain_ok and self.D == 9
                and (l0["d_in"], l0["d_out"], l1["d_in"], l1["d_out"]) == (9, 9, 9, 1)
                and torch.equal(l0["tab"].cpu(), _baked_table(9)) and torch.equal(l1["tab"].cpu(), _baked_table(1))):
            self.chain = _lib.tp_chain_plan(dtype, U, l0["cgw"], l1["cgw"])

    def forward(self, csr: EdgeCSR, vec: torch.Tensor, x_emb: Optional[torch.Tensor], keep: bool = True, fill_embed=None):
        E, N, U, S, L, D = csr.num_edges, csr.num_atoms, self.U, self.S, self.L, self.D
        dt, dev = self.dtype, self.device
        assert vec.dtype == self.acc and (fill_embed is not None or x_emb.dtype == dt)
        sv = _Saved()
        sv.fold = fill_embed is not None
        sv.csr, sv.vec = csr, vec
        _lib.set_tag("fwd.embed")
        Y = _lib.sh_fwd(vec, self.lmax)
        X = torch.empty(E, S * (L + 1), dtype=dt, device=dev)
        w0 = torch.empty(E, self.nw, dtype=dt, device=dev)
        omega = [torch.empty(E, self.nw, dtype=dt, device=dev)]
        if fill_embed is not None:
            fill_embed(w0, X[:, :S], omega[0])
        else:
            self.embed.forward([x_emb], [w0, X[:, :S], omega[0]])
        V: List[Optional[torch.Tensor]] = [None]
        gammas, pre_lat = [], []
        Ez = torch.empty(E, 1, dtype=dt, device=dev)
        pre_read = None
        chain = self.chain
        for l, ly in enumerate(self.layers):
            _lib.set_tag(f"fwd.L{l}")
            gamma = _lib.env_sum(dt, self.lmax, N, U, csr.row_ptr, Y, omega[l], self.sf)
            Vn = None
            if chain is not None:
                s = torch.empty(E, U, dtype=dt, device=dev)
                if not _lib.tp_chain_fwd(chain, ly["last"], csr.row_ptr, csr.ctr, gammas[0] if l else gamma, gamma if l else None, Y, w0, s):
                    if l:
                        raise RuntimeError("tp_chain_fwd declined the last layer after taking the first")
                    chain = None
            if chain is None:
                Vn = torch.empty(E, ly["d_out"], U, dtype=dt, device=dev)
                _lib.tp_fwd(dt, self.lmax, N, E, U, ly["d_in"], ly["d_out"], ly["tab"], ly["cgw"], csr.row_ptr, csr.ctr, gamma,
                            V[l], Y, w0 if l == 0 else None, Vn)
                s = Vn.view(E, ly["d_out"] * U)[:, :U]
            outs = [X[:, S * (l + 1) : S * (l + 2)]]
            if not ly["last"]:
                omega.append(torch.empty(E, self.nw, dtype=dt, device=dev))
                outs.append(omega[l + 1])
            if ly["last"] and self.ro_fused:
                P = S * L
                pre_l = torch.empty(E, ly["mlp"].dims[1], dtype=dt, device=dev)
                pre_r = torch.empty(E, self.readout.dims[1], dtype=dt, device=dev)
                if _lib.mlp2_readout(False, X[:, :P], s, X[:, P:], pre_l, pre_r, Ez, self.readout.W[1], self.ro_fwd_p, S, **self.readout.nl_kw):
                    pre_lat.append([pre_l])
                    pre_read = [pre_r]
            if pre_read is None:
                pre_lat.append(ly["mlp"].forward([X[:, : S * (l + 1)], s], outs))
            V.append(Vn)
            gammas.append(gamma)
        if pre_read is None:
            _lib.set_tag("fwd.readout")
            pre_read = self.readout.forward([X], [Ez])
        Ei = _lib.edge_sum(Ez.view(E).to(self.acc), csr.row_ptr, self.factor)
        sv.Y, sv.w0, sv.omega, sv.V, sv.gamma, sv.pre_lat, sv.pre_read, sv.X = Y, w0, omega, V, gammas, pre_lat, pre_read, X
        sv.chain = chain
        return Ei, X, Ez, sv

    def backward(self, sv: _Saved, gEi: torch.Tensor):
        if self.plain_ok:
            return self._backward_plain(sv, gEi)
        return self._backward_legacy(sv, gEi)

    def _backward_plain(self, sv: _Saved, gEi: torch.Tensor):
        csr = sv.csr
        E, N, U, S, L, D = csr.num_edges, csr.num_atoms, self.U, self.S, self.L, self.D
        dt, dev = self.dtype, self.device
        _lib.set_tag("bwd.readout")
        gEz = _lib.edge_sum_bwd(gEi.contiguous(), csr.ctr, self.factor).to(dt).view(E, 1)
        g_h = {"r": self.readout.hidden_grad([gEz])}
        pre = {"r": sv.pre_read[0]}
        for l in range(L):
            pre[l] = sv.pre_lat[l][0]
        gY = torch.zeros(E, D, dtype=self.acc, device=dev)
        gV_next: Optional[torch.Tensor] = None
# ... 23 lines not shown
                gs_acc = True
            gs = gV_next.view(E, ly["d_out"] * U)[:, :U]
            _lib.linear([g_h[l]], self.gsW[l], [gs], o_accum=[gs_acc], act=_lib.ACT_MUL_DSILU, a_aux=[pre[l]], W_packed=self.gsWp[l],
                        **self.readout.nl_kw)
            ggamma = torch.empty(N, D, U, dtype=self.acc, device=dev)
            if l == 0:
                gw0 = torch.empty(E, self.nw, dtype=dt, device=dev)
                _lib.tp_bwd(dt, self.lmax, N, E, U, ly["d_in"], ly["d_out"], ly["tab"], ly["cgw"], csr.row_ptr, csr.ctr,
                            sv.gamma[l], None, sv.Y, sv.w0, gV_next, None, gw0, gY, ggamma)
                gV_in = None
            else:
                gV_in = torch.empty(E, ly["d_in"], U, dtype=dt, device=dev)
                _lib.tp_bwd(dt, self.lmax, N, E, U, ly["d_in"], ly["d_out"], ly["tab"], ly["cgw"], csr.row_ptr, csr.ctr,
                            sv.gamma[l], sv.V[l], None, None, gV_next, gV_in, None, None, ggamma)
            gomega = torch.empty(E, self.nw, dtype=dt, device=dev)
            _lib.env_bwd(dt, self.lmax, U, csr.ctr, sv.Y, sv.omega[l], ggamma, self.sf, gomega, gY, row_ptr=csr.row_ptr)
            gV_next, gomega_next = gV_in, gomega
        _lib.set_tag("bwd.embed")
        g_x0 = block_grad(0)
        gvec = _lib.sh_bwd(sv.vec, gY, self.lmax)
        if sv.fold:
            return gvec, [gw0, g_x0, gomega_next]
        gx_emb = torch.empty(E, self.S_in, dtype=dt, device=dev)
        self.embed.backward([gw0, g_x0, gomega_next], [], [gx_emb], [False])
        return gvec, gx_emb

    def _backward_legacy(self, sv: _Saved, gEi: torch.Tensor):
        csr = sv.csr
        E, N, U, S, L, D = csr.num_edges, csr.num_atoms, self.U, self.S, self.L, self.D
        dt, dev = self.dtype, self.device
        _lib.set_tag("bwd.readout")
        gEz = _lib.edge_sum_bwd(gEi.contiguous(), csr.ctr, self.factor).to(dt).view(E, 1)
        gX = torch.empty(E, S * (L + 1), dtype=dt, device=dev)
        last = self.layers[-1]
        gV_last = torch.empty(E, last["d_out"], U, dtype=dt, device=dev)
        if last["d_out"] > 1:
            gV_last.zero_()
        fused = self.ro_fused and _lib.mlp2_readout(True, gX[:, : S * L], gV_last.view(E, -1)[:, :U], None, sv.pre_lat[-1][0],
                                                     sv.pre_read[0], gEz, self.readout.W[1], self.ro_bwd_p, S, **self.readout.nl_kw)
        if not fused:
            self.readout.backward([gEz], sv.pre_read, [gX], [False])
        gY = torch.zeros(E, D, dtype=self.acc, device=dev)
        gV_next: Optional[torch.Tensor] = None
        gomega_next: Optional[torch.Tensor] = None
        gw0 = None
        chain = sv.chain
        g1 = None
        for l in range(L - 1, -1, -1):
            ly = self.layers[l]
            _lib.set_tag(f"bwd.L{l}")
            if ly["last"]:
                gV_next = gV_last
                gs_acc = False
            else:
                gs_acc = True
            if chain is not None and not ly["last"]:
                g1 = torch.empty(E, U, dtype=dt, device=dev)
                gs, gs_acc = g1, False
            else:
                gs = gV_next.view(E, ly["d_out"] * U)[:, :U]
            gouts = [gX[:, S * (l + 1) : S * (l + 2)]]
            if not ly["last"]:
                gouts.append(gomega_next)
            if not (ly["last"] and fused):
                ly["mlp"].backward(gouts, sv.pre_lat[l], [gX[:, : S * (l + 1)], gs], [True, gs_acc])
            ggamma = torch.empty(N, D, U, dtype=self.acc, device=dev)
            if chain is not None:
                if l == 0:
                    gw0 = torch.empty(E, self.nw, dtype=dt, device=dev)
                ok = _lib.tp_chain_bwd(chain, l == 0, csr.row_ptr, csr.ctr, sv.gamma[0], sv.gamma[1] if l == 0 else None, sv.Y, sv.w0, g1,
                                       gV_last.view(E, U), gw0, gY if l == 0 else None, ggamma)
                if not ok:
                    raise RuntimeError("tp_chain_bwd declined a case its forward took")
                gV_in = None
            elif l == 0:
                gw0 = torch.empty(E, self.nw, dtype=dt, device=dev)
                _lib.tp_bwd(dt, self.lmax, N, E, U, ly["d_in"], ly["d_out"], ly["tab"], ly["cgw"], csr.row_ptr, csr.ctr,
                            sv.gamma[l], None, sv.Y, sv.w0, gV_next, None, gw0, gY, ggamma)
                gV_in = None
            else:
                gV_in = torch.empty(E, ly["d_in"], U, dtype=dt, device=dev)
                _lib.tp_bwd(dt, self.lmax, N, E, U, ly["d_in"], ly["d_out"], ly["tab"], ly["cgw"], csr.row_ptr, csr.ctr,
                            sv.gamma[l], sv.V[l], None, None, gV_next, gV_in, None, None, ggamma)
            gomega = torch.empty(E, self.nw, dtype=dt, device=dev)
            _lib.env_bwd(dt, self.lmax, U, csr.ctr, sv.Y, sv.omega[l], ggamma, self.sf, gomega, gY, row_ptr=csr.row_ptr)
            gV_next, gomega_next = gV_in, gomega
        _lib.set_tag("bwd.embed")
        gvec = _lib.sh_bwd(sv.vec, gY, self.lmax)
        if sv.fold:
            return gvec, [gw0, gX[:, :S], gomega_next]
        gx_emb = torch.empty(E, self.S_in, dtype=dt, device=dev)
        self.embed.backward([gw0, gX[:, :S], gomega_next], [], [gx_emb], [False])
        return gvec, gx_emb


class UpstreamPack:

    def __init__(self, edge_norm, radial, scalar_embed_mlp, dtype, device, fold_embed_of: Optional["AllegroCore"] = None):
        acc = _lib.ACC_DTYPE[dtype]
        self.fold = fold_embed_of is not None
        self.mlp = PackedMLP(scalar_embed_mlp, dtype, device, post=fold_embed_of.embed.W64[0] if self.fold else None)
        self.dtype = dtype
        self.S_rc = radial.out_dim
        self.kind = "spline" if hasattr(radial, "spline") else "bessel"
        if self.kind == "spline":
            sp = radial.spline
            self.num_types = radial.num_types
            self.rmax64 = edge_norm.rmax_table.detach().to(device=device, dtype=torch.float64).contiguous()
            self.sp_lower = sp.lower.detach().to(device=device, dtype=torch.float64)
            self.sp_upper = sp.upper.detach().to(device=device, dtype=torch.float64)
            self.sp_const = float(sp._const)
            self.sp_w = sp.flat_weights().to(device=device, dtype=torch.float64)
            return
        te = radial.type_embed
        self.p = float(radial.bessel_encode.p)
        self.S_rc = radial.out_dim
        self.rmax_table = edge_norm.rmax_table.detach().to(device=device, dtype=acc).contiguous()
        self.bessel_w = radial.bessel_encode.bessel_weights.detach().reshape(-1).to(device=device, dtype=acc).contiguous()
        self.Wb = te.basis_linear.folded_weights()[0].to(device=device, dtype=acc).contiguous()
        self.cemb = te.center_embed.weight.detach().to(device=device, dtype=acc).contiguous()
        self.nemb = te.neighbor_embed.weight.detach().to(device=device, dtype=acc).contiguous()
        self.PQ, self.S_pq, self.fold_radial = None, 0, False
        nb = int(self.bessel_w.numel())
        import os as _os

        if nb == 8 and _os.environ.get("ALLEGRO_B200_RADIAL_PQ", "1") == "1":
            Wb64 = te.basis_linear.folded_weights()[0].detach().double().cpu()
            ce, ne = te.center_embed.weight.detach().double().cpu(), te.neighbor_embed.weight.detach().double().cpu()
            T = ce.shape[0]
            temb = torch.cat([ce.unsqueeze(1).expand(T, T, -1), ne.unsqueeze(0).expand(T, T, -1)], dim=-1)
            PQ0 = temb.reshape(T * T, 1, -1) * Wb64.unsqueeze(0)
            if self.mlp.is_two_layer_nonlinear and self.mlp.dims[1] <= 128 and _os.environ.get("ALLEGRO_B200_FOLD_RADIAL", "1") == "1":
                self.fold_radial = True
                PQ0 = PQ0 @ self.mlp.W64[0]
            if PQ0.shape[-1] <= 128:
                self.PQ = PQ0.to(device=device, dtype=acc).contiguous()
                self.S_pq = int(PQ0.shape[-1])
            else:
                self.fold_radial = False

    def forward(self, vec, csr: EdgeCSR, types_i32, outs):
        dt = self.dtype
        if self.kind == "spline":
            from ._spline import spline_forward

            t64 = types_i32.long()
            e0, sp_saved = spline_forward(vec, t64[csr.ctr.long()], t64[csr.nbr.long()], self.rmax64, self.sp_lower, self.sp_upper, self.sp_const,
                                          self.sp_w, self.num_types, dt)
            return ("spline", sp_saved, self.mlp.forward([e0], outs))
        if self.fold_radial:
            h = _lib.radial_pq_fwd(dt, self.S_pq, self.p, vec, csr.ctr, csr.nbr, types_i32, self.rmax_table, self.bessel_w, self.PQ)
            _lib.linear([h], self.mlp.W[1], outs, act=_lib.ACT_SILU, W_packed=self.mlp.Wp[1], **self.mlp.nl_kw)
            return ("pq_fold", None, [h])
        if self.PQ is not None:
            e0 = _lib.radial_pq_fwd(dt, self.S_pq, self.p, vec, csr.ctr, csr.nbr, types_i32, self.rmax_table, self.bessel_w, self.PQ)
        else:
            e0 = _lib.radial_fwd(dt, self.S_rc, self.p, vec, csr.ctr, csr.nbr, types_i32, self.rmax_table, self.bessel_w, self.Wb, self.cemb, self.nemb)
        return ("bessel", None, self.mlp.forward([e0], outs))

    def backward(self, saved, gouts, vec, csr: EdgeCSR, types_i32, gvec):
        kind, sp_saved, pre = saved
        dt = self.dtype
        E = vec.shape[0]
        if kind == "pq_fold":
            g_h = self.mlp.hidden_grad(gouts)
            _lib.radial_pq_bwd(dt, self.S_pq, self.p, vec, csr.ctr, csr.nbr, types_i32, self.rmax_table, self.bessel_w, self.PQ, g_h, pre[0], gvec,
                               **self.mlp.nl_kw)
            return
# ... 84 lines not shown
```

include/allegro_b200.h:

```cpp
#ifndef ALLEGRO_B200_H
#define ALLEGRO_B200_H
#include <stdint.h>

#ifdef __cplusplus
extern "C" {
#endif

enum { AB2_F64 = 0, AB2_F32 = 1, AB2_BF16 = 2 };
enum { AB2_ACT_NONE = 0, AB2_ACT_SILU = 1, AB2_ACT_MUL_DSILU = 2 };
enum { AB2_EPI_NONE = 0, AB2_EPI_MUL_DSILU = 1 };
enum { AB2_NL_SILU = 1, AB2_NL_MISH = 2, AB2_NL_GELU = 3 };

#define AB2_MAX_SEG 4
#define AB2_MAX_LMAX 4

const char* ab2_last_error(void);
int ab2_version(void);
int ab2_device_ok(void);
int ab2_set_option(const char* key, int value);


int ab2_op_scatter_env(int dtype, int64_t E, int64_t row , double sf,
                       const void* x2, const int64_t* idxs, void* gamma, void* stream);

int ab2_op_contract(int dtype, int mode, int64_t E, int U, int d1, int d2, int dout, int nnz,
                    const int32_t* tab_ijk, const void* cgw, const void* a, const void* b,
                    const int64_t* idxs, void* out, void* stream);

int ab2_op_contract_wgrad(int dtype, int64_t E, int U, int d1, int d2, int dout, int nnz,
                          const int32_t* tab_ijk, const void* x1, const void* gamma, const void* gout,
                          const int64_t* idxs, void* gcgw, void* stream);

int ab2_op_gather_rows(int dtype, int64_t E, int64_t row, double sf, const void* src,
                       const int64_t* idxs, void* out, void* stream);


int ab2_sh_fwd(int acc_dtype, int lmax, int64_t E, const void* vec, void* Y, void* stream);
int ab2_sh_bwd(int acc_dtype, int lmax, int64_t E, const void* vec, const void* gY, void* gvec,
               int accumulate, void* stream);

int ab2_linear(int dtype, int64_t M, int K, int N, int n_a, const void* const* a_ptr_host,
               const int64_t* a_ld_host, const int32_t* a_width_host,
               const void* const* a_aux_ptr_host , const int64_t* a_aux_ld_host,
               int act, const void* W,
               const void* W_packed ,
               int n_o, void* const* o_ptr_host, const int64_t* o_ld_host,
               const int32_t* o_width_host, const int32_t* o_accum_host, int epi, const void* aux,
               int64_t aux_ld, void* stream);
int ab2_linear_nl(int dtype, int64_t M, int K, int N, int n_a, const void* const* a_ptr_host,
                  const int64_t* a_ld_host, const int32_t* a_width_host,
                  const void* const* a_aux_ptr_host , const int64_t* a_aux_ld_host,
                  int act, const void* W, const void* W_packed ,
                  int n_o, void* const* o_ptr_host, const int64_t* o_ld_host,
                  const int32_t* o_width_host, const int32_t* o_accum_host, int epi, const void* aux,
                  int64_t aux_ld, void* stream, int nonlin);

int64_t ab2_linear_packed_bytes(int dtype, int K, int N);
int ab2_linear_pack(int dtype, int K, int N, const void* W, void* packed, void* stream);

#define AB2_NOT_ELIGIBLE (-1)
int ab2_mlp2(int dtype, int backward, int64_t M, int K, int H, int N, int n_a, const void* const* a_ptr_host,
             const int64_t* a_ld_host, const int32_t* a_width_host, const void* W1_packed, const void* W2_packed,
             const void* w1_row , void* pre, int64_t pre_ld, int n_o,
             void* const* o_ptr_host, const int64_t* o_ld_host, const int32_t* o_width_host,
             const int32_t* o_accum_host, void* stream);
int ab2_mlp2_nl(int dtype, int backward, int64_t M, int K, int H, int N, int n_a, const void* const* a_ptr_host,
                const int64_t* a_ld_host, const int32_t* a_width_host, const void* W1_packed, const void* W2_packed,
                const void* w1_row , void* pre, int64_t pre_ld, int n_o,
                void* const* o_ptr_host, const int64_t* o_ld_host, const int32_t* o_width_host,
                const int32_t* o_accum_host, void* stream, int nonlin);

int ab2_mlp2_readout(int dtype, int backward, int64_t M, int P, int S, int U, int H, void* x, int64_t x_ld, void* s, int64_t s_ld,
                     void* xl, int64_t xl_ld, void* pre_l, int64_t pre_l_ld, void* pre_r, int64_t pre_r_ld, void* ez, int64_t ez_ld,
                     const void* const* w_packed_host, const void* w2_ro, void* stream);
int ab2_mlp2_readout_nl(int dtype, int backward, int64_t M, int P, int S, int U, int H, void* x, int64_t x_ld, void* s, int64_t s_ld,
                        void* xl, int64_t xl_ld, void* pre_l, int64_t pre_l_ld, void* pre_r, int64_t pre_r_ld, void* ez, int64_t ez_ld,
                        const void* const* w_packed_host, const void* w2_ro, void* stream, int nonlin);

int ab2_env_sum(int dtype, int lmax, int64_t N, int U, const int32_t* row_ptr, const void* Y,
                const void* w, int64_t w_ld, double sf, void* gamma, void* stream);

int ab2_env_bwd(int dtype, int lmax, int64_t N, int64_t E, int U, const int32_t* row_ptr,
                const int32_t* ctr, const void* Y, const void* w, int64_t w_ld, const void* ggamma,
                double sf, void* gw, int64_t gw_ld, void* gY, void* stream);

int ab2_tp_fwd(int dtype, int lmax, int64_t N, int64_t E, int U, int d_in, int d_out, int nnz,
               const int32_t* tab_ijk, const void* cgw, const int32_t* row_ptr, const int32_t* ctr,
               const void* gamma, const void* Vin, int implicit_v0, const void* Y, const void* w0,
               int64_t w0_ld, void* Vout, void* stream);

int ab2_tp_bwd(int dtype, int lmax, int64_t N, int64_t E, int U, int d_in, int d_out, int nnz,
               const int32_t* tab_ijk, const void* cgw, const int32_t* row_ptr, const int32_t* ctr,
               const void* gamma, const void* Vin, int implicit_v0, const void* Y, const void* w0,
               int64_t w0_ld, const void* gVout, void* gVin, void* gw0, int64_t gw0_ld, void* gY,
               void* ggamma, void* stream);

int ab2_tp_chain_fwd(int dtype, int last, int64_t N, int64_t E, int U, const int32_t* row_ptr, const int32_t* ctr,
                     const void* cgw0, const void* cgw1, const void* gamma0, const void* gamma1, const void* Y,
                     const void* w0, void* s, void* stream);
int ab2_tp_chain_bwd(int dtype, int first, int64_t N, int64_t E, int U, const int32_t* row_ptr, const int32_t* ctr,
                     const void* cgw0, const void* cgw1, const void* gamma0, const void* gamma1, const void* Y,
                     const void* w0, const void* g1, const void* g2, void* gw0, void* gY, void* ggamma, void* stream);

int ab2_edge_sum(int acc_dtype, int64_t N, const int32_t* row_ptr, const void* Ez, double factor,
                 void* Ei, void* stream);
int ab2_edge_sum_bwd(int acc_dtype, int64_t E, const int32_t* ctr, const void* gEi, double factor,
                     void* gEz, void* stream);

int ab2_force_scatter(int acc_dtype, int64_t N, int64_t n_total, int64_t E, const int32_t* row_ptr,
                      const int32_t* col_ptr, const int32_t* col_perm, const void* gvec, void* F,
                      void* stream);
int ab2_force_virial_scatter(int acc_dtype, int64_t N, int64_t n_total, int64_t E, const int32_t* row_ptr,
                             const int32_t* col_ptr, const int32_t* col_perm, const void* vec, const void* gvec,
                             void* F, void* W, void* stream);


int ab2_edge_vec(int pos_dtype, int acc_dtype, int64_t E, const void* pos, const int32_t* ctr,
                 const int32_t* nbr, const void* shift, void* vec, void* stream);

int ab2_radial_fwd(int dtype, int64_t E, int S_rc, int num_bessels, double p_cut, const void* vec,
                   const int32_t* ctr, const int32_t* nbr, const int32_t* types,
                   const void* rmax_table, int num_types, const void* bessel_w, const void* Wb,
                   const void* center_embed, const void* neighbor_embed, void* e0, void* stream);
int ab2_radial_bwd(int dtype, int64_t E, int S_rc, int num_bessels, double p_cut, const void* vec,
                   const int32_t* ctr, const int32_t* nbr, const int32_t* types,
                   const void* rmax_table, int num_types, const void* bessel_w, const void* Wb,
                   const void* center_embed, const void* neighbor_embed, const void* g_e0,
                   void* gvec, void* stream);


int ab2_nl_bin(int pos_dtype, int64_t n, const void* pos, const double* box_host, const double* origin_host,
               const int32_t* pbc_host, const int32_t* ncell_host, double r_max, int32_t* cell_id, void* stream);
int ab2_nl_count(int pos_dtype, int64_t n_centres, const void* pos, const double* box_host,
                 const double* origin_host, const int32_t* pbc_host, const int32_t* ncell_host, double r_max,
                 const int32_t* cell_start, const int32_t* order, int32_t* counts, void* stream);
int ab2_nl_fill(int pos_dtype, int64_t n_centres, const void* pos, const double* box_host,
                const double* origin_host, const int32_t* pbc_host, const int32_t* ncell_host, double r_max,
                const int32_t* cell_start, const int32_t* order, const int32_t* row_ptr, int32_t* nbr,
                void* shift, void* stream);

int ab2_nl_lattice_bin(int pos_dtype, int64_t n, const void* pos, const double* rows_host, const double* origin_host,
                       const int32_t* pbc_host, const int32_t* ncell_host, const int32_t* reach_host, double r_max,
                       int32_t* cell_id, void* stream);
int ab2_nl_lattice_count(int pos_dtype, int64_t n_centres, const void* pos, const double* rows_host,
                         const double* origin_host, const int32_t* pbc_host, const int32_t* ncell_host,
                         const int32_t* reach_host, double r_max, const int32_t* cell_start, const int32_t* order,
                         int32_t* counts, void* stream);
int ab2_nl_lattice_fill(int pos_dtype, int64_t n_centres, const void* pos, const double* rows_host,
                        const double* origin_host, const int32_t* pbc_host, const int32_t* ncell_host,
                        const int32_t* reach_host, double r_max, const int32_t* cell_start, const int32_t* order,
                        const int32_t* row_ptr, int32_t* nbr, void* shift, void* stream);


// ... 106 lines not shown
```

Before: 3.487 million.

## Compute env-adjoint weight gradient inside tensor-core GEMM instead of materializing it

The backward pass no longer writes the gomega tensor (E x nw) for layers after the first. The env backward kernel now produces only gY, and the downstream MLP/linear GEMM rebuilds that A-segment on the fly from Y, ctr and ggamma staged into shared memory. This removes a full write and reread of an edge-sized tensor. In exchange the GEMM producer does extra per-tile arithmetic and loads, and the code gains new template variants and eligibility checks.

```diff
diff --git a/allegro_b200/_lib.py b/allegro_b200/_lib.py
--- a/allegro_b200/_lib.py
+++ b/allegro_b200/_lib.py
@@ -42,6 +42,10 @@
     "ab2_mlp2_nl": ([_i32, _i32, _i64, _i32, _i32, _i32, _i32, _vp, _vp, _vp, _vp, _vp, _vp, _vp, _i64, _i32, _vp, _vp, _vp, _vp, _vp, _i32], C.c_int),
     "ab2_mlp2_readout_nl": ([_i32, _i32, _i64, _i32, _i32, _i32, _i32, _vp, _i64, _vp, _i64, _vp, _i64, _vp, _i64, _vp, _i64, _vp, _i64, _vp, _vp, _vp, _i32],
                             C.c_int),
+    "ab2_linear_env": ([_i32, _i64, _i32, _i32, _i32, _vp, _vp, _vp, _vp, _vp, _i32, _vp, _vp, _i32, _vp, _vp, _vp, _vp, _i32, _vp, _i64, _vp, _i32, _vp],
+                       C.c_int),
+    "ab2_mlp2_env": ([_i32, _i32, _i64, _i32, _i32, _i32, _i32, _vp, _vp, _vp, _vp, _vp, _vp, _vp, _i64, _i32, _vp, _vp, _vp, _vp, _vp, _i32, _vp], C.c_int),
+    "ab2_env_seg_available": ([_i32, _i32, _i32], C.c_int),
     "ab2_env_sum": ([_i32, _i32, _i64, _i32, _vp, _vp, _vp, _i64, _dbl, _vp, _vp], C.c_int),
     "ab2_env_bwd": ([_i32, _i32, _i64, _i64, _i32, _vp, _vp, _vp, _vp, _i64, _vp, _dbl, _vp, _i64, _vp, _vp], C.c_int),
     "ab2_tp_fwd": ([_i32, _i32, _i64, _i64, _i32, _i32, _i32, _i32, _vp, _vp, _vp, _vp, _vp, _vp, _i32, _vp, _vp, _i64, _vp, _vp], C.c_int),
@@ -241,6 +245,46 @@
     return out
 
 
+class EnvAdjSeg:
+
+    __slots__ = ("Y", "ctr", "ggamma", "sf")
+
+    def __init__(self, Y: torch.Tensor, ctr: torch.Tensor, ggamma: torch.Tensor, sf: float):
+        self.Y, self.ctr, self.ggamma, self.sf = Y, ctr, ggamma, float(sf)
+
+    @property
+    def lmax(self) -> int:
+        return int(round(self.Y.shape[1] ** 0.5)) - 1
+
+    @property
+    def shape(self) -> Tuple[int, int]:
+        return (self.Y.shape[0], (self.lmax + 1) * self.ggamma.shape[2])
+
+    @property
+    def dtype(self) -> torch.dtype:
+        return self.ggamma.dtype
+
+
+class _AB2EnvSeg(C.Structure):
+    _fields_ = [("seg", C.c_int), ("lmax", C.c_int), ("U", C.c_int), ("Y", C.c_void_p), ("ctr", C.c_void_p), ("ggamma", C.c_void_p), ("sf", C.c_double)]
+
+
+def _env_desc(a_segs) -> Optional[_AB2EnvSeg]:
+    idx = [s for s, t in enumerate(a_segs) if isinstance(t, EnvAdjSeg)]
+    if not idx:
+        return None
+    if len(idx) > 1:
+        raise ValueError("allegro_b200: at most one computed env-adjoint segment per GEMM")
+    e = a_segs[idx[0]]
+    _ptr(e.ggamma)
+    return _AB2EnvSeg(idx[0], e.lmax, int(e.ggamma.shape[2]), _contig(e.Y, "Y").data_ptr(), _contig(e.ctr, "ctr").data_ptr(),
+                      _contig(e.ggamma, "ggamma").data_ptr(), e.sf)
+
+
+def env_seg_available(dtype: torch.dtype, lmax: int, U: int) -> bool:
+    return bool(load().ab2_env_seg_available(DTYPE_ENUM[dtype], lmax, U))
+
+
 def linear(
     a_segs: Sequence[torch.Tensor],
     W: torch.Tensor,
@@ -257,10 +301,15 @@
     K, N = W.shape
     dt = W.dtype
     na, no = len(a_segs), len(o_segs)
+    env = _env_desc(a_segs)
     a_ptr = (C.c_void_p * na)()
     a_ld = (C.c_int64 * na)()
     a_w = (C.c_int32 * na)()
     for s, t in enumerate(a_segs):
+        if isinstance(t, EnvAdjSeg):
+            assert t.dtype == dt and t.shape[0] == M
+            a_ptr[s], a_ld[s], a_w[s] = None, t.shape[1], t.shape[1]
+            continue
         t, ld = _row_strided(t, f"A segment {s}")
         assert t.dtype == dt and t.shape[0] == M
         a_ptr[s], a_ld[s], a_w[s] = t.data_ptr(), ld, t.shape[1]
@@ -294,6 +343,13 @@
         assert aux.dtype == dt
     args = (DTYPE_ENUM[dt], M, K, N, na, a_ptr, a_ld, a_w, x_ptr, x_ld, act, _ptr(_contig(W, "W")), _ptr(W_packed), no, o_ptr, o_ld, o_w, o_acc,
             epi, _ptr(aux), aux_ld, _stream())
+    if env is not None:
+        with _timed("linear", 1):
+            rc = load().ab2_linear_env(*args, nonlin, C.byref(env))
+        if rc == NOT_ELIGIBLE:
+            raise RuntimeError("allegro_b200: the tensor-core linear declined a computed env-adjoint segment (M=%d, K=%d, N=%d)" % (M, K, N))
+        _check(rc)
+        return
     with _timed("linear", 1):
         _check(load().ab2_linear(*args) if nonlin == NL_SILU else load().ab2_linear_nl(*args, nonlin))
 
@@ -318,10 +374,15 @@
     if W2_packed is None or (W1_packed is None and not rank1):
         return False
     na, no = len(a_segs), len(o_segs)
+    env = _env_desc(a_segs)
     a_ptr = (C.c_void_p * na)()
     a_ld = (C.c_int64 * na)()
     a_w = (C.c_int32 * na)()
     for s, t in enumerate(a_segs):
+        if isinstance(t, EnvAdjSeg):
+            assert t.dtype == dt and t.shape[0] == M
+            a_ptr[s], a_ld[s], a_w[s] = None, t.shape[1], t.shape[1]
+            continue
         t, ld = _row_strided(t, f"A segment {s}") if t.shape[1] > 1 else (t, int(t.stride(0)))
         assert t.dtype == dt and t.shape[0] == M
         a_ptr[s], a_ld[s], a_w[s] = t.data_ptr(), ld, t.shape[1]
@@ -342,7 +403,10 @@
     args = (DTYPE_ENUM[dt], int(backward), M, K, H, N, na, a_ptr, a_ld, a_w, _ptr(W1_packed), _ptr(W2_packed),
             _ptr(_contig(W1, "W1")) if rank1 else None, _ptr(pre), pre_ld, no, o_ptr, o_ld, o_w, o_acc, _stream())
     with timer:
-        rc = load().ab2_mlp2(*args) if nonlin == NL_SILU else load().ab2_mlp2_nl(*args, nonlin)
+        if env is not None:
+            rc = load().ab2_mlp2_env(*args, nonlin, C.byref(env))
+        else:
+            rc = load().ab2_mlp2(*args) if nonlin == NL_SILU else load().ab2_mlp2_nl(*args, nonlin)
     if rc == NOT_ELIGIBLE:
         timer.cancel()
         return False
@@ -422,11 +486,11 @@
     return out
 
 
-def env_bwd(dtype, lmax: int, U: int, ctr, Y, w: torch.Tensor, ggamma, sf: float, gw: torch.Tensor, gY: torch.Tensor, row_ptr=None):
+def env_bwd(dtype, lmax: int, U: int, ctr, Y, w: torch.Tensor, ggamma, sf: float, gw: Optional[torch.Tensor], gY: torch.Tensor, row_ptr=None):
     w, w_ld = _row_strided(w, "w")
-    gw, gw_ld = _row_strided(gw, "gw")
+    gw, gw_ld = _row_strided(gw, "gw") if gw is not None else (None, 0)
     E = Y.shape[0]
-    with _timed("env_bwd", 1):
+    with _timed("env_bwd" if gw is not None else "env_bwd_gy", 1):
         _check(
             load().ab2_env_bwd(
                 DTYPE_ENUM[dtype], lmax, ggamma.shape[0], E, U, _ptr(row_ptr), _ptr(ctr), _ptr(_contig(Y, "Y")), _ptr(w), w_ld,
diff --git a/allegro_b200/csrc/env.cu b/allegro_b200/csrc/env.cu
--- a/allegro_b200/csrc/env.cu
+++ b/allegro_b200/csrc/env.cu
@@ -167,12 +167,13 @@
                            const void* w, int64_t w_ld, const void* ggamma, double sf, void* gw, int64_t gw_ld, void* gY,
                            void* stream) {
     if (E == 0) return 0;
-    AB2_CHECK_ARG(ctr && Y && w && ggamma && gw && gY && U > 0, "null pointer / U");
+    AB2_CHECK_ARG(ctr && Y && w && ggamma && gY && U > 0, "null pointer / U");
     cudaStream_t st = (cudaStream_t)stream;
     if (g_ab2_opt_tp_fast && ab2_env_bwd_stream(dtype, lmax, N, E, U, ctr, Y, w, w_ld, ggamma, sf, gw, gw_ld, gY, st) == 0) {
         AB2_CUDA_LAUNCH_CHECK();
         return 0;
     }
+    AB2_CHECK_ARG(gw, "gw == NULL needs the streaming env adjoint (fp32 / bf16, lmax 1-2, U <= 32 or 64, w and gw dense)");
     if (g_ab2_opt_tp_fast && row_ptr && lmax <= 3) {
         const int opt = g_ab2_opt_env_split ? g_ab2_opt_env_split : (U > 32 && dtype != AB2_F64 ? 4 : 1);
         const int split = opt >= 4 ? 4 : opt >= 2 ? 2 : 1;
diff --git a/allegro_b200/csrc/env_stream.cu b/allegro_b200/csrc/env_stream.cu
--- a/allegro_b200/csrc/env_stream.cu
+++ b/allegro_b200/csrc/env_stream.cu
@@ -18,7 +18,7 @@
     void* gY;
 };
 
-template <typename TAct, int LMAX, int NCH, int UT, int TE, int NS, int NCW>
+template <typename TAct, int LMAX, int NCH, int UT, int TE, int NS, int NCW, bool GW>
 __global__ void __launch_bounds__((NCW + 1) * 32) env_bwd_stream_kernel(const EnvParams p) {
     constexpr int D = (LMAX + 1) * (LMAX + 1), N_IR = LMAX + 1;
     constexpr int YP = (D + 3) / 4 * 4;
@@ -120,7 +120,7 @@
                         gwl = fmaf(Yr[j], gg[q][j], gwl);
                         part[j] = fmaf(wl, gg[q][j], part[j]);
                     }
-                    if (live) gw_row[l * U + q * 32] = from_acc<TAct>(gwl);
+                    if (GW && live) gw_row[l * U + q * 32] = from_acc<TAct>(gwl);
                 }
             }
             float* __restrict__ gy = (float*)p.gY + (int64_t)(za + t) * D;
@@ -152,11 +152,11 @@
     }
 }
 
-template <typename TAct, int LMAX, int NCH, int UT>
+template <typename TAct, int LMAX, int NCH, int UT, bool GW>
 int launch(const EnvParams& p, cudaStream_t st) {
     constexpr int TE = 16, NS = 3, NCW = 4;
     constexpr int D = (LMAX + 1) * (LMAX + 1), N_IR = LMAX + 1, YP = (D + 3) / 4 * 4;
-    auto kern = env_bwd_stream_kernel<TAct, LMAX, NCH, UT, TE, NS, NCW>;
+    auto kern = env_bwd_stream_kernel<TAct, LMAX, NCH, UT, TE, NS, NCW, GW>;
     const int offY = (TE * N_IR * p.U * (int)sizeof(TAct) + 127) & ~127;
     const int stage_bytes = offY + ((TE * YP * 4 + 127) & ~127) + ((TE * 4 + 127) & ~127);
     const int smem = 128 + NS * stage_bytes;
@@ -185,12 +185,17 @@
     return 0;
 }
 
+template <typename TAct, int LMAX, bool GW>
+int launch_u(const EnvParams& p, cudaStream_t st) {
+    if (p.U == 32) return launch<TAct, LMAX, 1, 32, GW>(p, st);
+    if (p.U < 32) return launch<TAct, LMAX, 1, 0, GW>(p, st);
+    if (p.U == 64) return launch<TAct, LMAX, 2, 64, GW>(p, st);
+    return -1;
+}
+
 template <typename TAct, int LMAX>
-int launch_u(const EnvParams& p, cudaStream_t st) {
-    if (p.U == 32) return launch<TAct, LMAX, 1, 32>(p, st);
-    if (p.U < 32) return launch<TAct, LMAX, 1, 0>(p, st);
-    if (p.U == 64) return launch<TAct, LMAX, 2, 64>(p, st);
-    return -1;
+int launch_gw(const EnvParams& p, cudaStream_t st) {
+    return p.gw ? launch_u<TAct, LMAX, true>(p, st) : launch_u<TAct, LMAX, false>(p, st);
 }
 
 }
@@ -200,10 +205,10 @@
     if (!g_ab2_opt_env_stream || dtype == AB2_F64 || lmax < 1 || lmax > 2 || E <= 0 || E >= ((int64_t)1 << 31)) return -1;
     const int esz = dtype == AB2_F32 ? 4 : 2;
     const int n_ir = lmax + 1;
-    if ((U * esz) % 16 != 0 || w_ld != (int64_t)n_ir * U || gw_ld != (int64_t)n_ir * U) return -1;
+    if ((U * esz) % 16 != 0 || w_ld != (int64_t)n_ir * U || (gw && gw_ld != (int64_t)n_ir * U)) return -1;
     if ((reinterpret_cast<uintptr_t>(w) & 15) != 0) return -1;
     EnvParams p;
     p.N = N; p.E = E; p.U = U; p.ctr = ctr; p.Y = Y; p.w = w; p.ggamma = ggamma; p.sf = (float)sf; p.gw = gw; p.gY = gY;
-    if (dtype == AB2_F32) return lmax == 2 ? launch_u<float, 2>(p, st) : launch_u<float, 1>(p, st);
-    return lmax == 2 ? launch_u<bf16, 2>(p, st) : launch_u<bf16, 1>(p, st);
-}
+    if (dtype == AB2_F32) return lmax == 2 ? launch_gw<float, 2>(p, st) : launch_gw<float, 1>(p, st);
+    return lmax == 2 ? launch_gw<bf16, 2>(p, st) : launch_gw<bf16, 1>(p, st);
+}
diff --git a/allegro_b200/csrc/linear.cu b/allegro_b200/csrc/linear.cu
--- a/allegro_b200/csrc/linear.cu
+++ b/allegro_b200/csrc/linear.cu
@@ -121,13 +121,14 @@
 
 int ab2_linear_tc_try(int dtype, int64_t M, int K, int N, int n_a, const void* const* a_ptr, const int64_t* a_ld,
                       const int32_t* a_width, const void* const* a_aux, const int64_t* a_aux_ld, int act, const void* Wpacked, int n_o, void* const* o_ptr, const int64_t* o_ld,
-                      const int32_t* o_width, const int32_t* o_accum, int epi, const void* aux, int64_t aux_ld, cudaStream_t st, int nonlin);
+                      const int32_t* o_width, const int32_t* o_accum, int epi, const void* aux, int64_t aux_ld, cudaStream_t st, int nonlin,
+                      const AB2EnvSeg* env);
 
-extern "C" int ab2_linear_nl(int dtype, int64_t M, int K, int N, int n_a, const void* const* a_ptr, const int64_t* a_ld,
-                          const int32_t* a_width, const void* const* a_aux, const int64_t* a_aux_ld, int act, const void* W,
-                          const void* Wpacked, int n_o, void* const* o_ptr,
-                          const int64_t* o_ld, const int32_t* o_width, const int32_t* o_accum, int epi, const void* aux,
-                          int64_t aux_ld, void* stream, int nonlin) {
+extern "C" int ab2_linear_env(int dtype, int64_t M, int K, int N, int n_a, const void* const* a_ptr, const int64_t* a_ld,
+                              const int32_t* a_width, const void* const* a_aux, const int64_t* a_aux_ld, int act, const void* W,
+                              const void* Wpacked, int n_o, void* const* o_ptr,
+                              const int64_t* o_ld, const int32_t* o_width, const int32_t* o_accum, int epi, const void* aux,
+                              int64_t aux_ld, void* stream, int nonlin, const AB2EnvSeg* env) {
     AB2_CHECK_ARG(nonlin == AB2_NL_SILU || nonlin == AB2_NL_MISH || nonlin == AB2_NL_GELU, "nonlinearity");
     if (M == 0) return 0;
     AB2_CHECK_ARG(n_a >= 1 && n_a <= AB2_MAX_SEG && n_o >= 1 && n_o <= AB2_MAX_SEG, "segment count");
@@ -138,7 +139,8 @@
     p.M = M; p.K = K; p.N = N; p.n_a = n_a; p.act = act; p.W = W; p.n_o = n_o; p.epi = epi; p.aux = aux; p.aux_ld = aux_ld;
     int ks = 0, ns = 0;
     for (int s = 0; s < n_a; ++s) {
-        AB2_CHECK_ARG(a_ptr[s] && a_width[s] > 0 && a_ld[s] >= a_width[s], "A segment");
+        const bool computed = env && s == env->seg;
+        AB2_CHECK_ARG((a_ptr[s] || computed) && a_width[s] > 0 && (a_ld[s] >= a_width[s] || computed), "A segment");
         p.a[s].ptr = a_ptr[s]; p.a[s].ld = a_ld[s]; p.a[s].width = a_width[s]; ks += a_width[s];
         p.a[s].aux = a_aux ? a_aux[s] : nullptr;
         p.a[s].aux_ld = (a_aux && a_aux_ld) ? a_aux_ld[s] : 0;
@@ -152,12 +154,13 @@
     AB2_CHECK_ARG(ns == N, "output segment widths must sum to N");
     cudaStream_t st = (cudaStream_t)stream;
     const int tc = Wpacked ? ab2_linear_tc_try(dtype, M, K, N, n_a, a_ptr, a_ld, a_width, a_aux, a_aux_ld, act, Wpacked, n_o, o_ptr, o_ld, o_width,
-                                               o_accum, epi, aux, aux_ld, st, nonlin)
+                                               o_accum, epi, aux, aux_ld, st, nonlin, env)
                            : -1;
     if (tc == 0) {
         AB2_CUDA_LAUNCH_CHECK();
         return 0;
     }
+    if (tc < 0 && env) return AB2_NOT_ELIGIBLE;
     if (tc > 0) {
         ab2_set_error("%s:%d: tensor-core linear: a column slice failed to launch (K=%d, N=%d)", __FILE__, __LINE__, K, N);
         return 2;
@@ -168,6 +171,15 @@
     return 0;
 }
 
+extern "C" int ab2_linear_nl(int dtype, int64_t M, int K, int N, int n_a, const void* const* a_ptr, const int64_t* a_ld,
+                             const int32_t* a_width, const void* const* a_aux, const int64_t* a_aux_ld, int act, const void* W,
+                             const void* Wpacked, int n_o, void* const* o_ptr,
+                             const int64_t* o_ld, const int32_t* o_width, const int32_t* o_accum, int epi, const void* aux,
+                             int64_t aux_ld, void* stream, int nonlin) {
+    return ab2_linear_env(dtype, M, K, N, n_a, a_ptr, a_ld, a_width, a_aux, a_aux_ld, act, W, Wpacked, n_o, o_ptr, o_ld, o_width, o_accum, epi, aux,
+                          aux_ld, stream, nonlin, nullptr);
+}
+
 extern "C" int ab2_linear(int dtype, int64_t M, int K, int N, int n_a, const void* const* a_ptr, const int64_t* a_ld,
                           const int32_t* a_width, const void* const* a_aux, const int64_t* a_aux_ld, int act, const void* W,
                           const void* Wpacked, int n_o, void* const* o_ptr,
diff --git a/allegro_b200/csrc/linear_tc.cu b/allegro_b200/csrc/linear_tc.cu
--- a/allegro_b200/csrc/linear_tc.cu
+++ b/allegro_b200/csrc/linear_tc.cu
@@ -7,6 +7,7 @@
 extern int g_ab2_opt_linear_tc;
 extern int g_ab2_opt_linear_tma;
 extern int g_ab2_opt_tc_debug;
+extern int g_ab2_opt_tp_fast, g_ab2_opt_env_stream;
 
 namespace {
 
@@ -34,6 +35,15 @@
     int accum;
     const void* aux;
     int64_t aux_ld;
+};
+
+struct TcEnv {
+    const float* Y;
+    const int32_t* ctr;
+    const float* gg;
+    float sf;
+    int D, U;
+    int seg;
 };
 
 struct TcParams {
@@ -54,6 +64,7 @@
     int debug;
     int raw_depth;
     int has_aux;
+    TcEnv env;
 };
 
 struct KEnt {
@@ -723,13 +734,14 @@
     fence_barrier_init();
 }
 
+template <bool ENV = false>
 __device__ __forceinline__ int4 tma_kseg_entry(const TcParams& p, int i) {
     int kk = i * KC;
     int4 ent = make_int4(-1, 0, 0, 0);
 #pragma unroll
     for (int sgi = 0; sgi < AB2_MAX_SEG; ++sgi) {
         if (sgi < p.n_a && ent.x < 0 && kk < p.K) {
-            if (kk < p.a[sgi].width) ent = make_int4(sgi, kk, p.a[sgi].aux ? 1 : 0, 0);
+            if (kk < p.a[sgi].width) ent = make_int4(sgi, kk, p.a[sgi].aux ? 1 : 0, (ENV && sgi == p.env.seg) ? 1 : 0);
             kk -= p.a[sgi].width;
         }
     }
@@ -745,7 +757,61 @@
     for (int e = threadIdx.x; e < w_half / 16; e += NTHREADS) dl[e] = __ldg(srcl + e);
 }
 
-template <int G, int NL>
+constexpr int ENV_Y_OFF = BM * 4;
+__device__ __forceinline__ void env_stage_rows(const TcEnv& e, int64_t M, int64_t row0, uint32_t dst, uint32_t bar, int t, int nt) {
+    const int rows = (M - row0) < BM ? (int)(M - row0) : BM;
+    for (int r = t; r < rows; r += nt) cp_async4(dst + 4u * r, e.ctr + row0 + r);
+    const float* ys = e.Y + row0 * e.D;
+    for (int k = t; k < rows * e.D; k += nt) cp_async4(dst + ENV_Y_OFF + 4u * k, ys + k);
+    asm volatile("cp.async.mbarrier.arrive.shared::cta.b64 [%0];" ::"r"(bar) : "memory");
+}
+
+template <int RGW>
+__device__ __forceinline__ void env_chunk_values(const TcEnv& e, const uint8_t* raw, int64_t M, int l, int u0, int64_t row0, int lrow0,
+                                                 float (&v)[RGW][8]) {
+    const int j0 = l * l, nj = 2 * l + 1;
+    const int* sc = reinterpret_cast<const int*>(raw);
+    const float* sy = reinterpret_cast<const float*>(raw + ENV_Y_OFF);
+    int c[RGW];
+#pragma unroll
+    for (int i = 0; i < RGW; ++i) c[i] = row0 + lrow0 + 8 * i < M ? sc[lrow0 + 8 * i] : -1;
+    float gg[5][8];
+    int cur = -1;
+#pragma unroll
+    for (int i = 0; i < RGW; ++i) {
+        if (c[i] >= 0 && c[i] != cur) {
+            cur = c[i];
+            const float* g = e.gg + ((int64_t)cur * e.D + j0) * e.U + u0;
+#pragma unroll
+            for (int jj = 0; jj < 5; ++jj) {
+                if (jj < nj) {
+                    const float4 g0 = __ldg(reinterpret_cast<const float4*>(g + jj * e.U));
+                    const float4 g1 = __ldg(reinterpret_cast<const float4*>(g + jj * e.U) + 1);
+                    gg[jj][0] = e.sf * g0.x; gg[jj][1] = e.sf * g0.y; gg[jj][2] = e.sf * g0.z; gg[jj][3] = e.sf * g0.w;
+                    gg[jj][4] = e.sf * g1.x; gg[jj][5] = e.sf * g1.y; gg[jj][6] = e.sf * g1.z; gg[jj][7] = e.sf * g1.w;
+                }
+            }
+        }
+        float a[8];
+#pragma unroll
+        for (int t = 0; t < 8; ++t) a[t] = 0.f;
+        if (c[i] >= 0) {
+            const float* y = sy + (lrow0 + 8 * i) * e.D + j0;
+#pragma unroll
+            for (int jj = 0; jj < 5; ++jj) {
+                if (jj < nj) {
+                    const float yj = y[jj];
+#pragma unroll
+                    for (int t = 0; t < 8; ++t) a[t] = fmaf(yj, gg[jj][t], a[t]);
+                }
+            }
+        }
+#pragma unroll
+        for (int t = 0; t < 8; ++t) v[i][t] = a[t];
+    }
+}
+
+template <int G, int NL, bool ENV = false>
 __device__ __forceinline__ void tma_converter_role(const TcParams& p, const TmaMaps& maps, int NR, const TcCtx& ctx, uint8_t* sRaw,
                                                    const int4* sKseg, uint32_t rbar0, int64_t total, int warp, int lane) {
     constexpr int WPG = NPROD / G;
@@ -778,23 +844,43 @@
         const bool leader = sub == 0 && lane == 0;
         if (leader) {
             for (int sgi = 0; sgi < p.n_a; ++sgi) {
+                if (ENV && sgi == p.env.seg) continue;
                 asm volatile("prefetch.tensormap [%0];" ::"l"(reinterpret_cast<uint64_t>(&maps.a[sgi])) : "memory");
                 if (p.a[sgi].aux) asm volatile("prefetch.tensormap [%0];" ::"l"(reinterpret_cast<uint64_t>(&maps.x[sgi])) : "memory");
             }
-            for (int q = grp; q < NR && q < total; q += G) tma_issue(q, q);
-        }
+            if (!ENV)
+                for (int q = grp; q < NR && q < total; q += G) tma_issue(q, q);
+        }
+        auto issue = [&](int64_t qs, int rs) {
+            if (sKseg[(int)(qs % nkb)].w) {
+                const int64_t tile = blockIdx.x + (qs / nkb) * gridDim.x;
+                env_stage_rows(p.env, p.M, tile * BM, smem_u32(sRaw + (size_t)rs * raw_slot), rfull_bar(rs), sub * 32 + lane, WPG * 32);
+                asm volatile("bar.sync %0, %1;" ::"r"(1 + grp), "r"(WPG * 32) : "memory");
+                if (leader) mbar_expect_tx(rfull_bar(rs), 0u);
+            } else if (leader) {
+                tma_issue(qs, rs);
+            }
+        };
+        if (ENV)
+            for (int q = grp; q < NR && q < total; q += G) issue(q, q);
         for (int64_t qs = grp; qs < total; qs += G) {
             mbar_wait(rfull_bar(rs), rph);
             const uint8_t* raw = sRaw + (size_t)rs * raw_slot;
             const bool ax = p.has_aux && sKseg[kb].z;
             float v[RGW][8];
-#pragma unroll
-            for (int i = 0; i < RGW; ++i) {
-                const int row = (sub * RGW + i) * 8 + r8;
-                const uint8_t* rp = raw + row * 128;
-                const float4 x = *reinterpret_cast<const float4*>(rp + (((2 * kc) ^ r8) << 4));
-                const float4 y = *reinterpret_cast<const float4*>(rp + (((2 * kc + 1) ^ r8) << 4));
-                v[i][0] = x.x; v[i][1] = x.y; v[i][2] = x.z; v[i][3] = x.w; v[i][4] = y.x; v[i][5] = y.y; v[i][6] = y.z; v[i][7] = y.w;
+            if (ENV && sKseg[kb].w) {
+                const int col = sKseg[kb].y, l = col / p.env.U;
+                const int64_t tile = blockIdx.x + (int64_t)((int)qs / nkb) * gridDim.x;
+                env_chunk_values<RGW>(p.env, raw, p.M, l, col - l * p.env.U + kc * 8, tile * BM, sub * RGW * 8 + r8, v);
+            } else {
+#pragma unroll
+                for (int i = 0; i < RGW; ++i) {
+                    const int row = (sub * RGW + i) * 8 + r8;
+                    const uint8_t* rp = raw + row * 128;
+                    const float4 x = *reinterpret_cast<const float4*>(rp + (((2 * kc) ^ r8) << 4));
+                    const float4 y = *reinterpret_cast<const float4*>(rp + (((2 * kc + 1) ^ r8) << 4));
+                    v[i][0] = x.x; v[i][1] = x.y; v[i][2] = x.z; v[i][3] = x.w; v[i][4] = y.x; v[i][5] = y.y; v[i][6] = y.z; v[i][7] = y.w;
+                }
             }
             if (ax) {
 #pragma unroll
@@ -808,7 +894,11 @@
                 }
             }
             asm volatile("bar.sync %0, %1;" ::"r"(1 + grp), "r"(WPG * 32) : "memory");
-            if (leader && qs + NR < total) tma_issue(qs + NR, rs);
+            if (ENV) {
+                if (qs + NR < total) issue(qs + NR, rs);
+            } else if (leader && qs + NR < total) {
+                tma_issue(qs + NR, rs);
+            }
             mbar_wait(ctx.empty_bar(cs), cph ^ 1);
             uint8_t* st_hi = sA + cs * stage_bytes;
 #pragma unroll
@@ -843,7 +933,7 @@
     }
 }
 
-template <int G, int NCH, int NL>
+template <int G, int NCH, int NL, bool ENV>
 __global__ void __launch_bounds__(NTHREADS, 1) linear_tma_kernel(const TcParams p, const __grid_constant__ TmaMaps maps, int NR) {
     constexpr int WPG = NPROD / G;
     using TSrc = float;
@@ -867,7 +957,7 @@
 
     if (threadIdx.x == 0) tma_init_bars(bar0, rbar0, WPG);
     if (threadIdx.x < MAX_K / 32) {
-        sKseg[threadIdx.x] = tma_kseg_entry(p, threadIdx.x);
+        sKseg[threadIdx.x] = tma_kseg_entry<ENV>(p, threadIdx.x);
     } else if (threadIdx.x >= 64 && threadIdx.x < 64 + MAX_CHUNK) {
         sChunk[threadIdx.x - 64] = tc_chunk_info<TSrc>(p, (threadIdx.x - 64) * 32);
     }
@@ -883,7 +973,7 @@
     if (warp >= NPROD) {
         tc_consumer_role<TSrc, SPLIT, NCH, NL>(p, ctx, warp - NPROD, lane);
     } else {
-        tma_converter_role<G, NL>(p, maps, NR, ctx, sRaw, sKseg, rbar0, total, warp, lane);
+        tma_converter_role<G, NL, ENV>(p, maps, NR, ctx, sRaw, sKseg, rbar0, total, warp, lane);
     }
 }
 
@@ -914,7 +1004,7 @@
     tc_epilogue<float, NCH, false>(p2, chunks, stg, acc, tile, wg, w4, lane);
 }
 
-template <int NCH1, int NL>
+template <int NCH1, int NL, bool ENV>
 __global__ void __launch_bounds__(NTHREADS, 1) mlp2_kernel(const __grid_constant__ Mlp2Params q, const __grid_constant__ TmaMaps maps, int NR) {
     constexpr int G = 2, WPG = NPROD / G;
     constexpr int H = 32 * NCH1;
@@ -941,7 +1031,7 @@
 
     if (threadIdx.x == 0) tma_init_bars(bar0, rbar0, WPG);
     if (threadIdx.x < MAX_K / 32) {
-        sKseg[threadIdx.x] = tma_kseg_entry(p, threadIdx.x);
+        sKseg[threadIdx.x] = tma_kseg_entry<ENV>(p, threadIdx.x);
     } else if (threadIdx.x >= 64 && threadIdx.x < 64 + (1 + MLP2_MAX_CHUNKS) * MAX_CHUNK) {
         const int i = threadIdx.x - 64, t = i / MAX_CHUNK, c0 = (i % MAX_CHUNK) * 32;
         ChunkInfo ci{nullptr, nullptr, 0, 0, 0};
@@ -960,7 +1050,7 @@
     if (warp < NPROD) {
         if (!rank1) {
             const int64_t my_tiles = (p.num_tiles > blockIdx.x) ? (p.num_tiles - blockIdx.x + gridDim.x - 1) / gridDim.x : 0;
-            tma_converter_role<G, AB2_NL_SILU>(p, maps, NR, ctx, sRaw, sKseg, rbar0, my_tiles * nkb, warp, lane);
+            tma_converter_role<G, AB2_NL_SILU, ENV>(p, maps, NR, ctx, sRaw, sKseg, rbar0, my_tiles * nkb, warp, lane);
         }
         return;
     }
@@ -1320,6 +1410,28 @@
 
 }
 
+extern "C" int ab2_env_seg_available(int dtype, int lmax, int U) {
+    return (dtype == AB2_F32 && (lmax == 1 || lmax == 2) && (U == 32 || U == 64) && g_ab2_opt_linear_tc && g_ab2_opt_linear_tma && g_ab2_opt_tp_fast &&
+            g_ab2_opt_env_stream) ? 1 : 0;
+}
+
+static bool tc_env_ok(int dtype, const AB2EnvSeg* e, int n_a, const int32_t* a_width) {
+    return ab2_env_seg_available(dtype, e->lmax, e->U) && e->seg >= 0 && e->seg < n_a && a_width[e->seg] == (e->lmax + 1) * e->U && e->Y &&
+           e->ctr && e->ggamma && (reinterpret_cast<uintptr_t>(e->ggamma) % 16) == 0;
+}
+
+static TcEnv tc_env_of(const AB2EnvSeg* e) {
+    TcEnv t;
+    t.Y = reinterpret_cast<const float*>(e->Y);
+    t.ctr = e->ctr;
+    t.gg = reinterpret_cast<const float*>(e->ggamma);
+    t.sf = (float)e->sf;
+    t.D = (e->lmax + 1) * (e->lmax + 1);
+    t.U = e->U;
+    t.seg = e->seg;
+    return t;
+}
+
 static int tc_npad(int N) { return (N + 31) / 32 * 32; }
 
 extern "C" int64_t ab2_linear_packed_bytes(int dtype, int K, int N) {
@@ -1391,7 +1503,9 @@
     TmaMaps maps;
     memset(&maps, 0, sizeof(maps));
     if (!tc_encode_fn()) return -1;
+    const bool env = p.env.Y != nullptr;
     for (int s = 0; s < p.n_a && !dry; ++s) {
+        if (env && s == p.env.seg) continue;
         if (!tc_make_map(&maps.a[s], p.a[s].ptr, p.a[s].ld, p.a[s].width, p.M)) return -1;
         if (p.a[s].aux && !tc_make_map(&maps.x[s], p.a[s].aux, p.a[s].aux_ld, p.a[s].width, p.M)) return -1;
     }
@@ -1400,6 +1514,7 @@
     int G = 0, NR = 0, nstage = 0;
     size_t smem = 0;
     for (int q = 0; q < 6 && !G; ++q) {
+        if (env && plans[q][0] != 2) continue;
         const size_t need = 1024 + ((w_bytes + 127) & ~127) + (size_t)plans[q][2] * stage_bytes + EPI_BYTES + TAIL_BYTES +
                             (size_t)plans[q][1] * raw_slot;
         if (need <= (size_t)max_smem) { G = plans[q][0]; NR = plans[q][1]; nstage = plans[q][2]; smem = need; }
@@ -1417,17 +1532,21 @@
     };
     return tc_with_nl(nonlin, [&](auto nl) -> int {
         constexpr int NL = decltype(nl)::value;
-        switch ((G == 4 ? 4 : 0) + p.Npad / 32) {
-            case 1: return go(linear_tma_kernel<2, 1, NL>);
-            case 2: return go(linear_tma_kernel<2, 2, NL>);
-            case 3: return go(linear_tma_kernel<2, 3, NL>);
-            case 4: return go(linear_tma_kernel<2, 4, NL>);
-            case 5: return go(linear_tma_kernel<4, 1, NL>);
-            case 6: return go(linear_tma_kernel<4, 2, NL>);
-            case 7: return go(linear_tma_kernel<4, 3, NL>);
-            case 8: return go(linear_tma_kernel<4, 4, NL>);
-        }
-        return -1;
+        auto pick = [&](auto env_c) -> int {
+            constexpr bool ENV = decltype(env_c)::value;
+            switch ((G == 4 ? 4 : 0) + p.Npad / 32) {
+                case 1: return go(linear_tma_kernel<2, 1, NL, ENV>);
+                case 2: return go(linear_tma_kernel<2, 2, NL, ENV>);
+                case 3: return go(linear_tma_kernel<2, 3, NL, ENV>);
+                case 4: return go(linear_tma_kernel<2, 4, NL, ENV>);
+                case 5: return go(linear_tma_kernel<4, 1, NL, ENV>);
+                case 6: return go(linear_tma_kernel<4, 2, NL, ENV>);
+                case 7: return go(linear_tma_kernel<4, 3, NL, ENV>);
+                case 8: return go(linear_tma_kernel<4, 4, NL, ENV>);
+            }
+            return -1;
+        };
+        return env ? pick(std::true_type{}) : pick(std::false_type{});
     });
 }
 
@@ -1446,7 +1565,7 @@
 static int tc_launch_slice(int dtype, int64_t M, int K, int N, int n_a, const void* const* a_ptr, const int64_t* a_ld,
                            const int32_t* a_width, const void* const* a_aux, const int64_t* a_aux_ld, int act, const void* Whi, const void* Wlo,
                            int n_o, void* const* o_ptr, const int64_t* o_ld, const int32_t* o_width, const int32_t* o_accum, int epi,
-                           const void* aux, int64_t aux_ld, cudaStream_t st, int nonlin, bool dry = false) {
+                           const void* aux, int64_t aux_ld, cudaStream_t st, int nonlin, const TcEnv* env, bool dry = false) {
     const int has_aux = (act == AB2_ACT_MUL_DSILU && a_aux) ? 1 : 0;
     if (tc_npad(N) > MAX_N) return -1;
     int num_sms = 0, max_smem = 0;
@@ -1460,6 +1579,7 @@
         p.a[s].aux = has_aux ? a_aux[s] : nullptr; p.a[s].aux_ld = has_aux ? a_aux_ld[s] : 0;
     }
     p.has_aux = has_aux;
+    if (env) p.env = *env;
     for (int s = 0; s < n_o; ++s) { p.o[s].ptr = o_ptr[s]; p.o[s].ld = o_ld[s]; p.o[s].width = o_width[s]; p.o[s].accum = o_accum ? o_accum[s] : 0; }
     const bool split = dtype == AB2_F32;
     const int w_bytes = p.Npad * K * 2 * (split ? 2 : 1);
@@ -1485,6 +1605,7 @@
         const int rc = tc_launch_tma(p, w_bytes, stage_bytes, max_smem, grid, st, dry, nonlin);
         if (rc == 0) return 0;
     }
+    if (env) return -1;
     auto go = [&](auto kern) -> int {
         if (cudaFuncSetAttribute(kern, cudaFuncAttributeMaxDynamicSharedMemorySize, (int)smem) != cudaSuccess) {
             cudaGetLastError();
@@ -1511,12 +1632,21 @@
 
 int ab2_linear_tc_try(int dtype, int64_t M, int K, int N, int n_a, const void* const* a_ptr, const int64_t* a_ld,
                       const int32_t* a_width, const void* const* a_aux, const int64_t* a_aux_ld, int act, const void* Wpacked, int n_o, void* const* o_ptr, const int64_t* o_ld,
-                      const int32_t* o_width, const int32_t* o_accum, int epi, const void* aux, int64_t aux_ld, cudaStream_t st, int nonlin) {
+                      const int32_t* o_width, const int32_t* o_accum, int epi, const void* aux, int64_t aux_ld, cudaStream_t st, int nonlin,
+                      const AB2EnvSeg* env_seg) {
     if (!g_ab2_opt_linear_tc || !Wpacked || dtype == AB2_F64) return -1;
     if (ab2_linear_packed_bytes(dtype, K, N) == 0) return -1;
+    TcEnv env_v;
+    const TcEnv* env = nullptr;
+    if (env_seg) {
+        if (!tc_env_ok(dtype, env_seg, n_a, a_width) || (act == AB2_ACT_MUL_DSILU && a_aux && a_aux[env_seg->seg])) return -1;
+        env_v = tc_env_of(env_seg);
+        env = &env_v;
+    }
     const int esz = (dtype == AB2_F32) ? 4 : 2;
     for (int s = 0; s < n_a; ++s) {
         if (a_width[s] % 8 != 0) return -1;
+        if (env && s == env->seg) continue;
         if ((reinterpret_cast<uintptr_t>(a_ptr[s]) % 16) != 0 || (a_ld[s] * esz) % 16 != 0) return -1;
         if (act == AB2_ACT_MUL_DSILU && a_aux && a_aux[s] &&
             ((reinterpret_cast<uintptr_t>(a_aux[s]) % 16) != 0 || (a_aux_ld[s] * esz) % 16 != 0)) return -1;
@@ -1532,7 +1662,7 @@
     while (true) {
         const int probe = width < N ? width : N;
         if (tc_launch_slice(dtype, M, K, probe, n_a, a_ptr, a_ld, a_width, a_aux, a_aux_ld, act, Wpacked, Wpacked, 1, o_ptr, o_ld, &probe, &any_accum, epi,
-                            aux, aux_ld, st, nonlin, true) == 0)
+                            aux, aux_ld, st, nonlin, env, true) == 0)
             break;
         if (width <= 32) return -1;
         width = (width / 2 + 31) / 32 * 32;
@@ -1559,22 +1689,23 @@
         }
         const void* aux_s = aux ? reinterpret_cast<const uint8_t*>(aux) + (size_t)n0 * esz : nullptr;
         const int rc = tc_launch_slice(dtype, M, K, ns, n_a, a_ptr, a_ld, a_width, a_aux, a_aux_ld, act, hi + (size_t)n0 * K * 2,
-                                       lo + (size_t)n0 * K * 2, cnt, so_ptr, so_ld, so_w, so_acc, epi, aux_s, aux_ld, st, nonlin);
+                                       lo + (size_t)n0 * K * 2, cnt, so_ptr, so_ld, so_w, so_acc, epi, aux_s, aux_ld, st, nonlin, env);
         if (rc != 0) return n0 == 0 ? -1 : 1;
     }
     return 0;
 }
 
-extern "C" int ab2_mlp2_nl(int dtype, int backward, int64_t M, int K, int H, int N, int n_a, const void* const* a_ptr, const int64_t* a_ld,
-                           const int32_t* a_width, const void* W1_packed, const void* W2_packed, const void* w1_row, void* pre, int64_t pre_ld,
-                           int n_o, void* const* o_ptr, const int64_t* o_ld, const int32_t* o_width, const int32_t* o_accum, void* stream,
-                           int nonlin) {
+extern "C" int ab2_mlp2_env(int dtype, int backward, int64_t M, int K, int H, int N, int n_a, const void* const* a_ptr, const int64_t* a_ld,
+                            const int32_t* a_width, const void* W1_packed, const void* W2_packed, const void* w1_row, void* pre, int64_t pre_ld,
+                            int n_o, void* const* o_ptr, const int64_t* o_ld, const int32_t* o_width, const int32_t* o_accum, void* stream,
+                            int nonlin, const AB2EnvSeg* env) {
     AB2_CHECK_ARG(nonlin == AB2_NL_SILU || nonlin == AB2_NL_MISH || nonlin == AB2_NL_GELU, "nonlinearity");
     AB2_CHECK_ARG(n_a >= 1 && n_a <= AB2_MAX_SEG && n_o >= 1 && n_o <= AB2_MAX_SEG, "segment count");
     AB2_CHECK_ARG(K > 0 && H > 0 && N > 0 && pre && pre_ld >= H, "shape");
     int ks = 0, ns = 0;
     for (int s = 0; s < n_a; ++s) {
-        AB2_CHECK_ARG(a_ptr[s] && a_width[s] > 0 && a_ld[s] >= a_width[s], "A segment");
+        const bool computed = env && s == env->seg;
+        AB2_CHECK_ARG((a_ptr[s] || computed) && a_width[s] > 0 && (a_ld[s] >= a_width[s] || computed), "A segment");
         ks += a_width[s];
     }
     for (int s = 0; s < n_o; ++s) {
@@ -1584,6 +1715,7 @@
     AB2_CHECK_ARG(ks == K, "A segment widths must sum to K");
     AB2_CHECK_ARG(ns == N, "output segment widths must sum to N");
     const bool rank1 = w1_row != nullptr;
+    if (env && (rank1 || !tc_env_ok(dtype, env, n_a, a_width))) return AB2_NOT_ELIGIBLE;
     AB2_CHECK_ARG(!rank1 || (backward && K == 1 && n_a == 1), "rank-1 mode is the backward of a single output column");
     if (M == 0) return 0;
     auto al16 = [](const void* ptr, int64_t ld) { return (reinterpret_cast<uintptr_t>(ptr) % 16) == 0 && (ld * 4) % 16 == 0; };
@@ -1594,7 +1726,7 @@
     } else {
         if (!W1_packed || K % KC != 0 || K > MAX_K) return AB2_NOT_ELIGIBLE;
         for (int s = 0; s < n_a; ++s)
-            if (a_width[s] % KC != 0 || !al16(a_ptr[s], a_ld[s])) return AB2_NOT_ELIGIBLE;
+            if (a_width[s] % KC != 0 || (!(env && s == env->seg) && !al16(a_ptr[s], a_ld[s]))) return AB2_NOT_ELIGIBLE;
     }
     const int nchunks = (N + MLP2_CHUNK - 1) / MLP2_CHUNK;
     if (nchunks > MLP2_MAX_CHUNKS) return AB2_NOT_ELIGIBLE;
@@ -1629,7 +1761,8 @@
         p.Wpacked = W1_packed;
         p.Wlo = reinterpret_cast<const uint8_t*>(W1_packed) + (size_t)H * K * 2;
         for (int s = 0; s < n_a; ++s)
-            if (!tc_make_map(&maps.a[s], a_ptr[s], a_ld[s], a_width[s], M)) return AB2_NOT_ELIGIBLE;
+            if (!(env && s == env->seg) && !tc_make_map(&maps.a[s], a_ptr[s], a_ld[s], a_width[s], M)) return AB2_NOT_ELIGIBLE;
+        if (env) p.env = tc_env_of(env);
     }
     if (backward) {
         q.backward = 1;
@@ -1676,12 +1809,24 @@
     };
     return tc_with_nl(nonlin, [&](auto nl) -> int {
         constexpr int NL = decltype(nl)::value;
-        switch (H / 32) {
-            case 1: return go(mlp2_kernel<1, NL>);
-            case 2: return go(mlp2_kernel<2, NL>);
-        }
-        return AB2_NOT_ELIGIBLE;
+        auto pick = [&](auto env_c) -> int {
+            constexpr bool ENV = decltype(env_c)::value;
+            switch (H / 32) {
+                case 1: return go(mlp2_kernel<1, NL, ENV>);
+                case 2: return go(mlp2_kernel<2, NL, ENV>);
+            }
+            return AB2_NOT_ELIGIBLE;
+        };
+        return env ? pick(std::true_type{}) : pick(std::false_type{});
     });
+}
+
+extern "C" int ab2_mlp2_nl(int dtype, int backward, int64_t M, int K, int H, int N, int n_a, const void* const* a_ptr, const int64_t* a_ld,
+                           const int32_t* a_width, const void* W1_packed, const void* W2_packed, const void* w1_row, void* pre, int64_t pre_ld,
+                           int n_o, void* const* o_ptr, const int64_t* o_ld, const int32_t* o_width, const int32_t* o_accum, void* stream,
+                           int nonlin) {
+    return ab2_mlp2_env(dtype, backward, M, K, H, N, n_a, a_ptr, a_ld, a_width, W1_packed, W2_packed, w1_row, pre, pre_ld, n_o, o_ptr, o_ld, o_width,
+                        o_accum, stream, nonlin, nullptr);
 }
 
 extern "C" int ab2_mlp2(int dtype, int backward, int64_t M, int K, int H, int N, int n_a, const void* const* a_ptr, const int64_t* a_ld,
diff --git a/allegro_b200/nn/_pipeline.py b/allegro_b200/nn/_pipeline.py
--- a/allegro_b200/nn/_pipeline.py
+++ b/allegro_b200/nn/_pipeline.py
@@ -104,6 +104,10 @@
                 Ws = self.layers[l]["mlp"].WT[0][:, S * (l + 1) : S * (l + 1) + U].contiguous()
                 self.gsW.append(Ws)
                 self.gsWp.append(_lib.linear_pack(Ws))
+        self.env_seg = (not self.plain_ok and self.L >= 2 and dtype == torch.float32 and S % 32 == 0
+                        and all(ly["mlp"].is_two_layer_nonlinear and ly["mlp"].dims[1] <= 64 and ly["mlp"].WTp[-1] is not None
+                                for ly in self.layers[:-1])
+                        and _lib.env_seg_available(dtype, self.lmax, U))
         self.chain = None
         l0, l1 = (self.layers + [None, None])[:2]
         if (self.L == 2 and not self.plain_ok and self.D == 9
@@ -293,8 +297,12 @@
                 gV_in = torch.empty(E, ly["d_in"], U, dtype=dt, device=dev)
                 _lib.tp_bwd(dt, self.lmax, N, E, U, ly["d_in"], ly["d_out"], ly["tab"], ly["cgw"], csr.row_ptr, csr.ctr,
                             sv.gamma[l], sv.V[l], None, None, gV_next, gV_in, None, None, ggamma)
-            gomega = torch.empty(E, self.nw, dtype=dt, device=dev)
-            _lib.env_bwd(dt, self.lmax, U, csr.ctr, sv.Y, sv.omega[l], ggamma, self.sf, gomega, gY, row_ptr=csr.row_ptr)
+            if self.env_seg and l > 0:
+                _lib.env_bwd(dt, self.lmax, U, csr.ctr, sv.Y, sv.omega[l], ggamma, self.sf, None, gY, row_ptr=csr.row_ptr)
+                gomega = _lib.EnvAdjSeg(sv.Y, csr.ctr, ggamma, self.sf)
+            else:
+                gomega = torch.empty(E, self.nw, dtype=dt, device=dev)
+                _lib.env_bwd(dt, self.lmax, U, csr.ctr, sv.Y, sv.omega[l], ggamma, self.sf, gomega, gY, row_ptr=csr.row_ptr)
             gV_next, gomega_next = gV_in, gomega
         _lib.set_tag("bwd.embed")
         gvec = _lib.sh_bwd(sv.vec, gY, self.lmax)
diff --git a/include/allegro_b200.h b/include/allegro_b200.h
--- a/include/allegro_b200.h
+++ b/include/allegro_b200.h
@@ -69,6 +69,29 @@
                 const void* w1_row , void* pre, int64_t pre_ld, int n_o,
                 void* const* o_ptr_host, const int64_t* o_ld_host, const int32_t* o_width_host,
                 const int32_t* o_accum_host, void* stream, int nonlin);
+
+typedef struct AB2EnvSeg {
+    int seg;
+    int lmax;
+    int U;
+    const void* Y;
+    const int32_t* ctr;
+    const void* ggamma;
+    double sf;
+} AB2EnvSeg;
+int ab2_env_seg_available(int dtype, int lmax, int U);
+int ab2_linear_env(int dtype, int64_t M, int K, int N, int n_a, const void* const* a_ptr_host,
+                   const int64_t* a_ld_host, const int32_t* a_width_host,
+                   const void* const* a_aux_ptr_host , const int64_t* a_aux_ld_host,
+                   int act, const void* W, const void* W_packed ,
+                   int n_o, void* const* o_ptr_host, const int64_t* o_ld_host,
+                   const int32_t* o_width_host, const int32_t* o_accum_host, int epi, const void* aux,
+                   int64_t aux_ld, void* stream, int nonlin, const AB2EnvSeg* env);
+int ab2_mlp2_env(int dtype, int backward, int64_t M, int K, int H, int N, int n_a, const void* const* a_ptr_host,
+                 const int64_t* a_ld_host, const int32_t* a_width_host, const void* W1_packed, const void* W2_packed,
+                 const void* w1_row , void* pre, int64_t pre_ld, int n_o,
+                 void* const* o_ptr_host, const int64_t* o_ld_host, const int32_t* o_width_host,
+                 const int32_t* o_accum_host, void* stream, int nonlin, const AB2EnvSeg* env);
 
 int ab2_mlp2_readout(int dtype, int backward, int64_t M, int P, int S, int U, int H, void* x, int64_t x_ld, void* s, int64_t s_ld,
                      void* xl, int64_t xl_ld, void* pre_l, int64_t pre_l_ld, void* pre_r, int64_t pre_r_ld, void* ez, int64_t ez_ld,
```

Measured after the change: 3.550 million, median of 6. 1.8% higher.
